# yozhijk/capsaicin

Measured on AMD Instinct MI355X. Metric: Mrays/sec (primary+secondary), cornell_box 1080p 64spp, higher is better.
Workload: dtype f32; 1 GPU; cornell_box.obj 1920x1080 64spp depth=8 (reference shading: Lambert + directional light + sky), tile-sharded over 1 GPU(s); triangles=32, bvh_depth=8, parallelism=tiles1, exchange=none

## Files before the change

### capsaicin_amd/capi.py

```python
import ctypes as C
import os
import subprocess

import numpy as np

_PKG = os.path.dirname(os.path.abspath(__file__))
_ROOT = os.path.dirname(_PKG)
LIB_PATH = os.path.join(_PKG, "libcapsaicin_hip.so")
if os.environ.get("CAP_LIB_VARIANT"):
    LIB_PATH = os.path.join(_PKG, "variants", "libcapsaicin_hip_%s.so" % os.environ["CAP_LIB_VARIANT"])

RENDER_AOV = 1
RENDER_EXT_MATERIALS = 2
RENDER_STAGE_TIMERS = 4
RENDER_GBUFFER_FEEDBACK = 8
RENDER_LOWRES_INDIRECT = 16

BUF_GBUFFER_GEO, BUF_DIRECT, BUF_ALBEDO, BUF_NORMAL_DEPTH, BUF_INDIRECT, BUF_COMBINED, BUF_ACCUM_SUM, BUF_ACCUM_MEAN, BUF_INDIRECT_LOWRES = range(9)


class CapError(RuntimeError):
    pass


# ... 472 lines not shown
        t = np.ascontiguousarray(rgba8, np.uint8)
        _check(lib().cap_texture_upload(self.ctx, index, _p(t), t.shape[1], t.shape[0]), "cap_texture_upload")

    def upload_bluenoise(self, rgba8):
        t = np.ascontiguousarray(rgba8, np.uint8)
        assert t.size == 256 * 256 * 4
        _check(lib().cap_bluenoise_upload(self.ctx, _p(t)), "cap_bluenoise_upload")

    def upload_materials(self, materials):
        m = np.ascontiguousarray(materials, np.float32).reshape(-1, 12)
        _check(lib().cap_materials_upload(self.ctx, _p(m), m.shape[0]), "cap_materials_upload")

    BVH_BUILD_AUTO, BVH_BUILD_LBVH, BVH_BUILD_SAH, BVH_BUILD_PLOC, BVH_BUILD_SAH_DEVICE = 0, 1, 2, 3, 4

    def set_bvh_build(self, mode):
        _check(lib().cap_set_bvh_build(self.ctx, mode), "cap_set_bvh_build")

    def build_bvh(self):
        _check(lib().cap_bvh_build(self.ctx), "cap_bvh_build")
        return self.bvh_info()

    def update_vertices(self, positions=None, normals=None, texcoords=None):
        ptrs, flags, keep = vertex_update_args(self._vertex_count, positions, normals, texcoords)
        if flags:
            import torch
            dev = torch.device("cuda", self.device)
            for a in keep:
                if a.device != dev:
                    raise CapError("update_vertices: tensors must be on %s, got %s" % (dev, a.device))
            torch.cuda.current_stream(dev).synchronize()
        _check(lib().cap_scene_update_vertices(self.ctx, ptrs[0], ptrs[1], ptrs[2], flags), "cap_scene_update_vertices")

    def refit_bvh(self):
        info = RefitInfo()
        _check(lib().cap_bvh_refit(self.ctx, C.byref(info)), "cap_bvh_refit")
        return info

    def bvh_info(self):
        bi = BvhInfo()
        _check(lib().cap_bvh_info(self.ctx, C.byref(bi)), "cap_bvh_info")
        return bi

    def bvh_readback(self):
        bi = self.bvh_info()
        nodes = np.zeros((bi.node_count, 16), np.float32)
        leaves = np.zeros(bi.triangle_count, np.uint32)
        _check(lib().cap_bvh_readback(self.ctx, _p(nodes), _p(leaves)), "cap_bvh_readback")
        return nodes, leaves

    def bvh_wide_readback(self):
        info = np.zeros(3, np.uint32)
        _check(lib().cap_bvh_wide_readback(self.ctx, None, None, _p(info)), "cap_bvh_wide_readback")
        nodes = np.zeros((int(info[0]), 20), np.uint32)
        src = np.zeros(max(1, self.bvh_info().triangle_count), np.uint32)
        _check(lib().cap_bvh_wide_readback(self.ctx, _p(nodes), _p(src), _p(info)), "cap_bvh_wide_readback")
        return nodes, src[:self.bvh_info().triangle_count], int(info[1]), int(info[2])

    def bvh_wide_info(self):
        info = np.zeros(3, np.uint32)
        _check(lib().cap_bvh_wide_readback(self.ctx, None, None, _p(info)), "cap_bvh_wide_readback")
        return int(info[0]), int(info[1]), int(info[2])

    def set_camera(self, cam):
        _check(lib().cap_camera_set(self.ctx, C.byref(cam)), "cap_camera_set")

    def set_prev_camera(self, cam):
        _check(lib().cap_prev_camera_set(self.ctx, C.byref(cam)), "cap_prev_camera_set")

    def set_resolution(self, width, height):
        _check(lib().cap_set_resolution(self.ctx, width, height), "cap_set_resolution")
        self.width, self.height = width, height

    def set_shard(self, index, count):
        _check(lib().cap_set_shard(self.ctx, index, count), "cap_set_shard")

    def set_traversal(self, mode):
        _check(lib().cap_set_traversal(self.ctx, mode), "cap_set_traversal")

    DEBUG_QUEUE_CAPACITY_DIV, DEBUG_WIDE_DEPTH_LIMIT, DEBUG_WIDE_IN_USE, DEBUG_FAIL_LANE1, DEBUG_LANES_USED = 1, 2, 3, 4, 5
    DEBUG_QUEUE_CANARY_FILL, DEBUG_QUEUE_CANARY_BEHIND, DEBUG_QUEUE_CANARY_USED, DEBUG_SELFTEST_DIV, DEBUG_NEE_PAIRS = 6, 7, 8, 9, 10
    DEBUG_SELFTEST_SHADE_UNARY, DEBUG_SELFTEST_SHADE_DIV2, DEBUG_SHADE_TAME = 11, 12, 13
    DEBUG_CAMERA_CULL = 14
    DEBUG_MARK_FORM = 15

    def debug_set(self, key, value):
        _check(lib().cap_debug_set(self.ctx, key, value), "cap_debug_set")

    DEBUG_SWITCH_BASE = 64

    def debug_switch(self, name, value):
        i = lib().cap_debug_switch_index(name.encode())
        if i < 0:
            raise CapError("unknown switch %s" % name)
        self.debug_set(self.DEBUG_SWITCH_BASE + i, 0xFFFFFFFFFFFFFFFF if value is None else int(value))

    def debug_get(self, key):
        v = _u64()
        _check(lib().cap_debug_get(self.ctx, key, C.byref(v)), "cap_debug_get")
        return int(v.value)

    def set_batch_paths(self, n):
        _check(lib().cap_set_batch_paths(self.ctx, n), "cap_set_batch_paths")

    def render(self, frame_begin, n_frames, num_bounces, flags=0):
        _check(lib().cap_render(self.ctx, frame_begin, n_frames, num_bounces, flags), "cap_render")

    def accum_reset(self):
        _check(lib().cap_accum_reset(self.ctx), "cap_accum_reset")

    def accum_import(self, sum_rgba, frames):
        a = np.ascontiguousarray(sum_rgba, np.float32)
        assert a.shape == (self.height, self.width, 4)
        _check(lib().cap_accum_import(self.ctx, _p(a), int(frames)), "cap_accum_import")

    def sync(self):
        _check(lib().cap_sync(self.ctx), "cap_sync")

    def readback(self, kind):
        if kind == BUF_INDIRECT_LOWRES:
            out = np.zeros((self.height // 2, self.width // 2, 4), np.float32)
        else:
            out = np.zeros((self.height, self.width, 4), np.float32)
        _check(lib().cap_readback(self.ctx, kind, _p(out)), "cap_readback")
        return out

    def stats(self):
        s = Stats()
        _check(lib().cap_stats_get(self.ctx, C.byref(s)), "cap_stats_get")
        return s

    def stats_reset(self):
        _check(lib().cap_stats_reset(self.ctx), "cap_stats_reset")

    RAY_FLAG_ACCEPT_FIRST_HIT, RAY_FLAG_CULL_BACK_FACING, RAY_FLAG_CULL_FRONT_FACING = 0x04, 0x10, 0x20

    def set_instance_masks(self, masks):
        if masks is None:
            _check(lib().cap_scene_set_instance_masks(self.ctx, None, len(self._tri_end)), "cap_scene_set_instance_masks")
            return
        m = np.ascontiguousarray(masks, np.uint8).reshape(-1)
        _check(lib().cap_scene_set_instance_masks(self.ctx, _p(m), m.size), "cap_scene_set_instance_masks")

    def trace_options(self, cull=None, mask=None, first_hit=False):
        if cull not in (None, "back", "front"):
            raise CapError('cull must be None, "back" or "front", got %r' % (cull,))
        if cull is None and mask is None and not first_hit:
            return None
        flags = {None: 0, "back": self.RAY_FLAG_CULL_BACK_FACING, "front": self.RAY_FLAG_CULL_FRONT_FACING}[cull]
        if first_hit:
            flags |= self.RAY_FLAG_ACCEPT_FIRST_HIT
        return TraceOptions(flags, 0 if mask is None else int(mask))

    def trace_rays(self, rays, out=None, sync=True, cull=None, mask=None, first_hit=False):
        return self._query(rays, out, sync, False, self.trace_options(cull, mask, first_hit))

    def trace_occlusion(self, rays, out=None, sync=True, cull=None, mask=None):
        return self._query(rays, out, sync, True, self.trace_options(cull, mask))

    def _query(self, rays, out, sync, any_hit, options=None):
        import torch
        dev = torch.device("cuda", self.device)
        host = isinstance(rays, np.ndarray)
        if host:
            rays = torch.from_numpy(np.ascontiguousarray(rays, np.float32).reshape(-1, 8)).to(dev)
            sync = True
        if rays.dtype != torch.float32 or rays.dim() != 2 or rays.shape[1] != 8 or not rays.is_contiguous() or rays.device != dev:
# ... 466 lines not shown
```

### capsaicin_amd/csrc/cap_context.h

```cpp
#pragma once

#include <array>
#include <string>
#include <utility>
#include <vector>

#include "../../include/capsaicin_hip.h"

#include "cap_kernels.h"

namespace cap
{
int fail(int code, const char* fmt, ...);

#define HIP_TRY(expr)                                                                                         \
    do                                                                                                        \
    {                                                                                                         \
        hipError_t e_ = (expr);                                                                               \
        if (e_ != hipSuccess) return fail(CAP_ERR_HIP, "%s failed: %s (%s:%d)", #expr, hipGetErrorString(e_), \
                                          __FILE__, __LINE__);                                                \
    } while (0)

template <typename T>
struct DevBuf
// ... 69 lines not shown
    uint32_t         vertex_count = 0, index_count = 0, mesh_count = 0, tri_count = 0;
    bool             scene_ready = false;

    std::vector<DevBuf<uint8_t>> texture_data;
    std::vector<TextureDev>      texture_host;
    DevBuf<TextureDev>           textures;
    bool                         textures_dirty = true;
    DevBuf<float2>               bluenoise;
    bool                         bluenoise_ready = false;
    std::vector<CapMaterial>     materials_host;
    DevBuf<CapMaterial>          materials;
    std::vector<float>           positions_host;
    std::vector<uint32_t>        indices_host;
    std::vector<CapMeshDesc>     meshes_host;
    DevBuf<uint32_t>             light_tris;
    DevBuf<float>                light_cdf;
    DevBuf<float2>               bluenoise_ba;
    uint32_t                     light_count = 0;
    float                        light_area  = 0.0f;
    bool                         materials_ready = false;

    DevBuf<float4>   shade_tris, tris_sorted, nodes, tri_raw, tri_box;
    DevBuf<float4>   nodes8, tris8;
    DevBuf<uint32_t> wide_src;
    DevBuf<uint32_t> wide_task, wide_alloc, wide_cnt;
    uint32_t         wide8_depth = 0, wide8_top = 0, wide8_nodes = 0;
    float            wide8_ms = 0.f;
    DevBuf<uint32_t> query_work, query_defer;
    DevBuf<uint8_t>  tri_mask;
    bool             tri_mask_on = false;
    DevBuf<float4>   inst_desc, inst_rec, inst_box, inst_tlas;
    DevBuf<uint32_t> inst_keys[2], inst_vals[2], inst_hist, inst_scan, inst_misc, inst_level_off;
    uint32_t         inst_count = 0, inst_top = 0, inst_nodes = 0;
    DevBuf<float2>   inst_near;
    DevBuf<uint32_t> inst_obj;
    bool             inst_obj_on = false;
    InstObject       scene_object_host{};
    DevBuf<InstObject> scene_object;
    std::vector<CapObjectInfo> obj_info;
    std::vector<uint32_t>      obj_node_base, obj_rec_base;
    uint32_t                   obj_count = 0, obj_max_depth = 0;
    DevBuf<float4>             forest_nodes, forest_tris;
    DevBuf<InstObject>         obj_table;
    DevBuf<float4>             obj_tri_raw, obj_tri_box;
    DevBuf<uint32_t>           obj_leaf_tri, obj_misc;
    DevBuf<float4>   fan_pairs, fan_singles;
    uint32_t         fan_pair_count = 0, fan_single_count = 0;
    DevBuf<float4>   fan_pairs_nee;
    uint32_t         fan_pair_nee_count = 0;
    std::vector<float>    fan_pairs_host;
    std::vector<uint32_t> light_tris_host;
    DevBuf<uint32_t> leaf_tri, keys0, keys1, vals0, vals1, hist, parent, flags, bvh_misc;
    DevBuf<float4>   ploc_boxes;
    DevBuf<uint32_t> ploc_ints;
    DevBuf<uint32_t> sahdev_words;
    CapBvhInfo       bvh_info{};
    bool             shade_tame = false;
    bool             bvh_ready = false;
    DevBuf<float>        pn_table;
    bool                 pn_ready = false;
    CapPseudonormalsInfo pn_info{};
    bool                  bvh_stale = false;
    bool                  positions_host_stale = false;
    bool                  visits_built_known = false;
    double                refit_visits_built = 0.0;
    std::vector<uint32_t> wide_levels;
    DevBuf<float>         wide_boxes;
    DevBuf<double>        refit_sums;

    CapCameraData camera{}, prev_camera{};
    bool          camera_ready = false, prev_camera_ready = false;
    ScreenDev     screen{};
    uint64_t      max_batch_paths = 0;
    SwitchTable   sw{};
    uint32_t      debug_capacity_div = 1;
    uint32_t      debug_wide_depth_limit = 0;
    bool          debug_fail_lane = false;
    uint64_t      lane1_failed_paths = 0;
    uint32_t      lane1_failed_bounces = 0, lane1_retry_tick = 0;
    uint32_t      lanes_last_render = 0;
    uint32_t      last_class_capacity = 0;
    uint32_t      tri_ids_dense = 0;
    uint32_t      last_mark_form = 0;
    uint32_t      last_cull_camera_pairs = 0;
    uint32_t      traversal_mode  = CAP_TRAVERSAL_AUTO;
    uint32_t      bvh_build_mode  = CAP_BVH_BUILD_AUTO;

    DevBuf<float4>     aov_geo, aov_nd, accum, image_tmp;
    DevBuf<uint64_t>   shaded_counter;
    struct Lane
    {
        hipStream_t      stream = nullptr;
        DevBuf<float4>   hits, q_org[2], q_dir[2], q_thr[2], s_org, s_dir, s_con, pl_color, pl_direct, pl_albedo;
        DevBuf<uint32_t> counters;
        DevBuf<uint32_t> stack_spill;
    } lane[2];
    hipStream_t stream2 = nullptr;
    hipEvent_t  lane_ev[2] = {nullptr, nullptr}, fork_ev = nullptr, join_ev = nullptr;
    static constexpr int kFrameRing = 4;
    DevBuf<FrameConst> frames_ring[kFrameRing];
    FrameConst*        frames_pinned[kFrameRing] = {nullptr, nullptr, nullptr, nullptr};
    size_t             frames_pinned_n[kFrameRing] = {0, 0, 0, 0};
    hipEvent_t         frames_event[kFrameRing] = {nullptr, nullptr, nullptr, nullptr};
    uint32_t           frames_next = 0;
    uint32_t           last_slots = 0;
    bool               aov_valid = false;
    bool               aov_lowres = false;
    uint32_t           aov_frame  = 0;
    uint64_t           frames_accumulated = 0;

    DevBuf<float4> post_in[4];
    DevBuf<float4> post_ihist[2], post_mhist[2], post_chist[2], post_prev_nd, post_itemp, post_temp[2], post_normals;
    uint32_t       post_w = 0, post_h = 0;
    int            post_last_dst = -1;

    void*           comm = nullptr;
    uint32_t        comm_rank = 0, comm_size = 0;
    bool            comm_local = false;
    DevBuf<float>   comm_send, comm_gathered, comm_image;
    hipEvent_t      comm_event = nullptr;

    CapStats               stats{};
    std::vector<TimedSpan> spans;
    std::vector<std::array<hipEvent_t, 6>> post_marks;
    std::vector<hipEvent_t> event_pool;
    std::vector<uint32_t*> pinned_pool;
    std::vector<std::pair<uint32_t*, uint32_t>> pending;
    uint64_t*              pinned_shaded = nullptr;
};

namespace cap
{
struct AovPlanes
{
    const float4 *color, *direct, *albedo;
};

int        sync_and_collect(CapContext* c);
hipEvent_t get_event(CapContext* c);
CameraDev  camera_dev(const CapCameraData& cd);
BvhDev     bvh_dev(const CapContext* c, const CapContext::Lane& lane);
AovPlanes  aov_planes(const CapContext* c);
int        trace_launch(const CapContext* c, const char* fmt, ...);
void       launch_texture_footprints(hipStream_t stream, const uint32_t* src, uint4* dst, uint32_t width, uint32_t height);
bool pair_ids_dense(const float* pairs, uint32_t pair_count, uint32_t single_count, uint32_t tri_count);
int  upload_fan_records(CapContext* c);
int  update_nee_pairs(CapContext* c);
int  ensure_positions_host(CapContext* c);
int  upload_light_table(CapContext* c);
int query_state(CapContext* c, const char* what);
}
```

### capsaicin_amd/csrc/cap_kernels.h

```cpp
#pragma once

#include "cap_device.h"

#include <cstdio>
#include <vector>

namespace cap
{
enum CapSwitch : uint32_t
{
    SW_NO_WIDE8 = 0,
    SW_LANE1_PRIORITY,
    SW_PLOC_RADIUS,
    SW_SAHDEV_LEAF,
    SW_WIDE_HOST_COLLAPSE,
    SW_TRACE_LAUNCHES,
    SW_NO_TWO_LANES,
    SW_LANE_SPLIT_MIN,
    SW_BLOCKS_PER_CU,
    SW_NO_CAMERA_CULL,
    SW_NO_ALBEDO_IN_W,
    SW_NO_INLINE_NEE,
    SW_NO_INLINE_PROBE,
    SW_NO_WAVE_RING,
    SW_ANY_REFILL,
    SW_PRIMARY_WIDE,
    SW_NO_PACKET,
    SW_NO_ANY_PROBE,
    SW_ANY_PROBE,
    SW_ANY_BLOCKS,
    SW_NO_PRIMARY_FUSE,
    SW_W8_REFILL,
    SW_W8_GRID,
    SW_AUTO_SAH_TRIANGLES,
    SW_NO_NEE_PAIR_CULL,
    SW_RAYGEN_KERNEL,
    SW_NO_PLANE_CODE,
    SW_COUNT
};
struct SwitchTable
{
    int64_t v[SW_COUNT];
    bool    on(CapSwitch k) const { return v[k] > 0; }
    int64_t get(CapSwitch k, int64_t dflt) const { return v[k] >= 0 ? v[k] : dflt; }
};

struct LaunchCfg
{
    hipStream_t stream;
    uint32_t    grid_blocks;
    uint32_t    stack_entries;
    uint32_t    cu_count = 0;
    uint32_t    any_no_probe = 0;
    const SwitchTable* sw = nullptr;
    bool    sw_on(CapSwitch k) const { return sw && sw->on(k); }
    int64_t sw_get(CapSwitch k, int64_t dflt) const { return sw ? sw->get(k, dflt) : dflt; }
};

template <auto K>
uint32_t resident_grid(const LaunchCfg& cfg, uint32_t want)
{
    static int per_cu = -1;
    if (per_cu < 0)
    {
        int n = 0;
        per_cu = (hipOccupancyMaxActiveBlocksPerMultiprocessor(&n, K, (int)kBlock, 0) == hipSuccess && n > 0) ? n : 0;
        if (cfg.sw_on(SW_TRACE_LAUNCHES)) fprintf(stderr, "[cap] resident workgroups per CU: %d\n", per_cu);
    }
    if (!cfg.cu_count || !per_cu) return want;
    const uint32_t cap = cfg.cu_count * (uint32_t)per_cu;
    return want < cap ? want : cap;
}
inline uint32_t queue_grid(const LaunchCfg& cfg, uint32_t max_count)
{
    uint32_t g = (max_count + kBlock - 1) / kBlock;
    if (g > cfg.grid_blocks) g = cfg.grid_blocks;
    return g ? g : 1;
}

void launch_trace_primary(const LaunchCfg& cfg, const BvhDev& bvh, const CameraDev& cam, const ScreenDev& screen,
                          const FrameConst* frames, uint32_t n_slots, float4* hits, uint32_t* work);
void launch_raygen_identity(const LaunchCfg& cfg, const CameraDev& cam, const ScreenDev& screen, const FrameConst* frames, uint32_t n_slots,
                            const RayQueue& q);
void launch_trace_closest(const LaunchCfg& cfg, const BvhDev& bvh, const RayQueue& q, uint32_t max_count, float4* hits);
void launch_trace_closest8(const LaunchCfg& cfg, const BvhDev& bvh, const RayQueue& q, uint32_t max_count, float4* hits, uint32_t* work);
void launch_trace_closest8_camera(const LaunchCfg& cfg, const BvhDev& bvh, const RayQueue& q, uint32_t max_count, float4* hits, uint32_t* work,
                                  const CameraDev& cam, const ScreenDev& screen, const FrameConst* frames, uint32_t n_slots);
void launch_trace_any(const LaunchCfg& cfg, const BvhDev& bvh, const ShadowQueue& q, uint32_t max_count, float4* target,
                      uint32_t pixels_padded, uint32_t n_slots, uint64_t* guard, uint32_t* work, bool mostly_unoccluded,
                      const FrameConst* frames, float4* code_plane = nullptr);

void launch_trace_any8_refill(const LaunchCfg& cfg, const BvhDev& bvh, const ShadowQueue& q, uint32_t max_count, float4* target, uint32_t pixels_padded,
                              uint32_t n_slots, uint64_t* guard, uint32_t* work, const FrameConst* frames);

struct QueryArgs
{
    const float4* rays;
    uint32_t      n;
    void*         out;
    uint32_t*     work;
    uint32_t*     defer;
    float         safe;
};
constexpr float kQuerySafeScale = 4.0f;
bool query8_stack_matches();
struct RayFilter;
void launch_query8(const LaunchCfg& cfg, const BvhDev& bvh, const QueryArgs& q, bool any, const RayFilter* f = nullptr, bool first_hit = false);
void launch_query_binary(const LaunchCfg& cfg, const BvhDev& bvh, const QueryArgs& q, bool any, bool deferred);
struct MultiArgs
{
    QueryArgs q;
    uint32_t  k;
    uint32_t* counts;
    uint32_t  resume;
};
constexpr uint32_t kMultiMaxK = 16;
uint32_t multi_bucket(uint32_t k);
void     launch_query8_multi(const LaunchCfg& cfg, const BvhDev& bvh, const MultiArgs& m, const RayFilter* f = nullptr);
void     launch_query_binary_multi(const LaunchCfg& cfg, const BvhDev& bvh, const MultiArgs& m, bool deferred, const RayFilter* f = nullptr);

// ... 19 lines not shown
    const float* normals;
    float*       signed_out;
};
void launch_signed_distance(const LaunchCfg& cfg, const BvhDev& bvh, const ClosestArgs& a, const SignedArgs& s, const RayFilter* f, uint32_t depth);
struct ClosestMultiArgs
{
    ClosestArgs a;
    uint32_t    k;
    uint32_t*   counts;
    uint32_t    resume;
};
void launch_closest_points_multi(const LaunchCfg& cfg, const BvhDev& bvh, const ClosestMultiArgs& m, const RayFilter* f, uint32_t depth);
struct TlasDev;
struct ClosestInstArgs
{
    ClosestArgs     a;
    uint32_t*       inst_out;
    const float4*   descs;
    const float2*   near;
    const uint32_t* xw_max;
};
void launch_closest_instances(const LaunchCfg& cfg, const BvhDev& bvh, const ClosestInstArgs& a, const TlasDev& tl, const RayFilter& f, uint32_t depth);
struct ClosestInstMultiArgs
{
    ClosestInstArgs ia;
    uint32_t        k;
    uint32_t*       counts;
    uint32_t        resume;
};
void launch_closest_instances_multi(const LaunchCfg& cfg, const BvhDev& bvh, const ClosestInstMultiArgs& m, const TlasDev& tl, const RayFilter& f,
                                    uint32_t depth);

struct InstObject
{
    double   blo[3], bhi[3];
    int32_t  root;
    uint32_t reserved;
};
struct InstanceBuildArgs
{
    const float*      descs;
    uint32_t          n;
    const InstObject* objects;
    uint32_t          n_objects;
    const uint32_t*   object_index;
    float4*      rec;
    float4*      box;
    float4*      tlas;
    float2*      near;
    uint32_t*    keys[2];
    uint32_t*    vals[2];
    uint32_t*    hist;
    uint32_t*    scan;
    uint32_t*    misc;
};
constexpr uint32_t kTlasMaxLevels = 25;
uint32_t tlas_layout(uint32_t n, uint32_t level_off[kTlasMaxLevels], uint32_t* total);
void     launch_instances_build(hipStream_t stream, const InstanceBuildArgs& a);
struct TlasDev
{
    const float4*   rec;
    const float4*   tlas;
    const uint32_t* level_off;
    uint32_t        top;
};
void launch_query_instances(const LaunchCfg& cfg, const BvhDev& bvh, const QueryArgs& q, const TlasDev& tl, const RayFilter& f, int mode, uint32_t* inst_out,
                            uint32_t depth);
void launch_query_instances_multi(const LaunchCfg& cfg, const BvhDev& bvh, const MultiArgs& m, const TlasDev& tl, const RayFilter& f, uint32_t* inst_out,
                                  uint32_t depth);
struct ForestRelocArgs
{
    float4*  nodes;
    float4*  tris;
    uint32_t n_tris, node_base, rec_base, first_triangle;
};
void launch_forest_relocate(hipStream_t stream, const ForestRelocArgs& a);

struct ShadeArgs
{
    SceneDev          scene;
    CameraDev         cam;
    ScreenDev         screen;
    const FrameConst* frames;
    const float4*     hits;
    RayQueue          in;
    RayQueue          out;
    ShadowQueue       shadow;
    Planes            planes;
    uint32_t          n_slots;
    uint32_t          bounce;
    uint32_t          num_bounces;
    uint32_t          max_count;
    uint32_t          aov_slot;
    uint64_t*         shaded_counter;
    uint32_t*         work;
    FeedbackDev       fb;
    uint32_t          albedo_in_w;
    uint32_t          inline_nee;
    uint32_t          inline_probe;
    uint32_t          wave_ring;
    uint32_t          cull_camera_pairs;
    uint32_t          code_in_color;
};
constexpr float kCodePadding = 0.f, kCodeSky = 1.f, kCodeKd = 2.f, kCodeBlack = 3.f;
constexpr float kCodeLit = 4.f;
constexpr float kCameraCullPad = 2.0f;
void launch_shade(const LaunchCfg& cfg, const ShadeArgs& args, bool ext, bool feedback = false);
bool launch_primary_shade(const LaunchCfg& cfg, const BvhDev& bvh, const ShadeArgs& args, float4* hits, bool ext);
uint32_t launch_trace_shade(const LaunchCfg& cfg, const BvhDev& bvh, const ShadeArgs& args, bool ext, bool feedback = false);
bool trace_shade_has_code_form(const BvhDev& bvh, const SceneDev& scene);

void launch_resolve(const LaunchCfg& cfg, const Planes& planes, uint32_t n_slots, uint32_t pixels_padded, float4* accum,
                    bool albedo_in_w = false, float kd_untextured = 0.0f, bool code_in_color = false);
void launch_untile(const LaunchCfg& cfg, const ScreenDev& screen, const float4* src, const float4* albedo, const float4* direct,
                   int plane_kind, float4* image);
void launch_tile(const LaunchCfg& cfg, const ScreenDev& screen, const float4* image, float4* dst);
void launch_untile4(const LaunchCfg& cfg, const ScreenDev& screen, const float4* s0, const float4* s1, const float4* s2, const float4* s3,
                    float4* d0, float4* d1, float4* d2, float4* d3);
void launch_tiles_mean(const LaunchCfg& cfg, const float4* accum, uint32_t pixels_padded, float4* dst);
void launch_assemble(const LaunchCfg& cfg, const ScreenDev& screen, const float4* gathered, uint32_t shard_count, float4* image,
                     size_t shard_stride = 0);
void launch_geo_aov(const LaunchCfg& cfg, const SceneDev& scene, const float4* hits_slot, uint32_t pixels_padded, float4* aov_geo);

struct BvhBuildArgs
{
    const float*    positions;
    const float*    normals;
    const float*    texcoords;
    const uint32_t* indices;
    const uint4*    tri_ids;
    const uint4*    mesh_offsets;
    uint32_t        tri_count;
    float4*         shade_tris;
    float4*         tris_sorted;
    float4*         nodes;
    uint32_t*       leaf_tri;
    float4*         tri_raw;
    float4*         tri_box;
    uint32_t*       keys[2];
    uint32_t*       vals[2];
    uint32_t*       hist;
    uint32_t*       parent;
    uint32_t*       flags;
    uint32_t*       bounds;
    uint32_t*       max_depth;
};
size_t bvh_radix_blocks(uint32_t n);
void   launch_bvh_build(hipStream_t stream, const BvhBuildArgs& a);
int    launch_bvh_sort(hipStream_t stream, const BvhBuildArgs& a);
size_t bvh_radix_scan_words(uint32_t n);
int    launch_radix_sort_pairs(hipStream_t stream, uint32_t* const keys[2], uint32_t* const vals[2], uint32_t n, uint32_t* hist, uint32_t* scan);
size_t bvh_scan_scratch_words(uint32_t total);
void   launch_exclusive_scan_u32(hipStream_t stream, uint32_t* v, uint32_t total, uint32_t* scratch);
struct PlocScratch
{
    float4*   boxes;
    uint32_t* ints;
};
int    launch_bvh_build_ploc(hipStream_t stream, const BvhBuildArgs& a, const PlocScratch& s, uint32_t radius);
size_t bvh_sah_device_scratch_words(uint32_t n);
int    launch_bvh_build_sah_device(hipStream_t stream, const BvhBuildArgs& a, const PlocScratch& s, uint32_t* scratch, uint32_t radius, uint32_t leaf);
void launch_bvh_setup(hipStream_t stream, const BvhBuildArgs& a);
void launch_bvh_finish_host(hipStream_t stream, const BvhBuildArgs& a);

void     launch_gather_wide(hipStream_t stream, const uint32_t* tri_src, const float4* tris_sorted, uint32_t n, float4* tris8);
struct WideCollapseArgs
{
    const float4*   bnodes;
    const uint32_t* count;
    uint32_t        n_tris, capacity;
    double          pad;
    uint32_t *      task, *alloc, *nodes8, *tri_src;
    uint32_t*       cnt;
    uint32_t        begin, end;
};
int      launch_wide_collapse(hipStream_t stream, WideCollapseArgs a, uint32_t* node_count, uint32_t* depth, uint32_t* top_nodes,
                          std::vector<uint32_t>* level_begin = nullptr);
struct PseudonormalArgs
{
    const float*    positions;
    const uint32_t* indices;
    const uint4*    tri_ids;
    const uint4*    mesh_offsets;
    uint32_t        tri_count;
    float*          table;
    uint32_t *      kx, *ky, *kz;
    uint32_t*       keys[2];
    uint32_t*       vals[2];
    uint32_t*       weld;
    uint32_t*       flag;
    uint32_t*       hist;
    uint32_t*       scan;
    double*         nf;
// ... 55 lines not shown
```

### capsaicin_amd/csrc/cap_shade.h

```cpp
#pragma once

#include "cap_exhaustive.h"
#include "cap_kernels.h"
#include "cap_reproject.h"
#include "cap_unscaled.h"

namespace cap
{
__device__ __forceinline__ void bluenoise4x4(const float2* tex, uint32_t x, uint32_t y, uint32_t count, float& s0, float& s1)
{
    const uint32_t px = (count % 16u) % 4u, py = (count % 16u) / 4u;
    const uint32_t sx = (x * 4u + px) % 256u, sy = (y * 4u + py) % 256u;
    const float2   t  = tex[sy * 256u + sx];
    const float    k  = 0.61803398875f * (float)(count / 16u);
    const float    a = t.x + k, b = t.y + k;
    s0 = a - floorf(a);
    s1 = b - floorf(b);
}

__device__ __forceinline__ v3 ortho_vector(v3 n)
{
    const bool  zn = fabsf(n.z) > 0.0f;
    const float a = zn ? n.z : n.y, b = zn ? n.y : n.x;
    const float k = sqrtf(fmaf(a, a, b * b));
    const float q1 = a / k, q2 = b / k;
    return zn ? mk3(0.0f, -q1, q2) : mk3(q1, -q2, 0.0f);
}

__device__ __forceinline__ v3 map_to_hemisphere(float r1, float r2, v3 n)
{
    v3       u = ortho_vector(n);
    const v3 v = cross3(u, n);
    u          = cross3(n, v);
    float sin_psi, cos_psi;
    sincos_c((2.0f * kPi) * r1, sin_psi, cos_psi);
    const float cos_theta = sqrtf(1.0f - r2);
    const float sin_theta = sqrtf(1.0f - cos_theta * cos_theta);
    const float a = sin_theta * cos_psi, b = sin_theta * sin_psi;
    return normalize3(mk3(fmaf(n.x, cos_theta, fmaf(v.x, b, u.x * a)), fmaf(n.y, cos_theta, fmaf(v.y, b, u.y * a)),
                          fmaf(n.z, cos_theta, fmaf(v.z, b, u.z * a))));
}

constexpr float kNormLo = 0.125f, kNormHi = 4.0f;
__device__ __forceinline__ v3 normalize3_tame(v3 v)
{
    return v * div_unscaled(1.0f, sqrt_pos(dot3(v, v)));
}
__device__ __forceinline__ bool ortho_in_range(float a, float b, float g)
{
    constexpr uint32_t kG0 = (127u - 78u) << 23, kG1 = (127u + 80u) << 23, kX0 = (127u - 80u) << 23;
    const uint32_t     xa = (f2u(a) & 0x7fffffffu) - 1u, xb = (f2u(b) & 0x7fffffffu) - 1u;
    return (f2u(g) - kG0 < kG1 - kG0) & ((xa < xb ? xa : xb) >= kX0 - 1u);
}
__device__ __forceinline__ v3 map_to_hemisphere_tame(float r1, float r2, v3 n)
{
    const bool  zn = fabsf(n.z) > 0.0f;
    const float a = zn ? n.z : n.y, b = zn ? n.y : n.x;
    const float g = fmaf(a, a, b * b);
#if defined(CAP_SHADE_ORTHO_PLAIN)
    const bool fast = false;
#else
    const bool  fast = __ballot(!ortho_in_range(a, b, g)) == 0ull;
#endif
    float       q1, q2;
    if (fast)
        div2_unscaled(a, b, sqrt_pos(g), q1, q2);
    else
    {
        const float k = sqrtf(g);
        q1 = a / k, q2 = b / k;
    }
    v3       u = zn ? mk3(0.0f, -q1, q2) : mk3(q1, -q2, 0.0f);
    const v3 v = cross3(u, n);
    u          = cross3(n, v);
    float sin_psi, cos_psi;
    sincos_c((2.0f * kPi) * r1, sin_psi, cos_psi);
    const float cos_theta = sqrt_pos(1.0f - r2);
    const float sin_theta = sqrt_unscaled(1.0f - cos_theta * cos_theta);
    const float ca = sin_theta * cos_psi, cb = sin_theta * sin_psi;
    const v3    d = mk3(fmaf(n.x, cos_theta, fmaf(v.x, cb, u.x * ca)), fmaf(n.y, cos_theta, fmaf(v.y, cb, u.y * ca)),
                        fmaf(n.z, cos_theta, fmaf(v.z, cb, u.z * ca)));
    return fast ? normalize3_tame(d) : normalize3(d);
}

__device__ __forceinline__ void oct_encode(v3 n, float& ox, float& oy)
{
    const float s = fabsf(n.x) + fabsf(n.y) + fabsf(n.z);
    n             = mk3(n.x / s, n.y / s, n.z / s);
    ox = n.x, oy = n.y;
    if (!(n.z >= 0.0f))
    {
        ox = (1.0f - fabsf(n.y)) * (n.x >= 0.0f ? 1.0f : -1.0f);
        oy = (1.0f - fabsf(n.x)) * (n.y >= 0.0f ? 1.0f : -1.0f);
    }
    ox = ox * 0.5f + 0.5f;
    oy = oy * 0.5f + 0.5f;
}

__device__ __forceinline__ uint32_t wrap_texel(float f, uint32_t n)
{
    const float m = f - floorf(f / (float)n) * (float)n;
    int         i = (int)m;
    if (i < 0) i = 0;
    if ((uint32_t)i >= n) i = 0;
    return (uint32_t)i;
}

__device__ __forceinline__ v3 sample_texture(const TextureDev& tex, float u, float v)
{
    const float    fx = fmaf(u, (float)tex.width, -0.5f), fy = fmaf(v, (float)tex.height, -0.5f);
    const float    x0f = floorf(fx), y0f = floorf(fy);
    const float    wx = fx - x0f, wy = fy - y0f;
    const uint32_t x0 = wrap_texel(x0f, tex.width), y0 = wrap_texel(y0f, tex.height);
    const uint4  fq   = reinterpret_cast<const uint4*>(tex.quads)[y0 * tex.width + x0];
    auto         rgba = [](uint32_t wd) { return make_uchar4((uint8_t)wd, (uint8_t)(wd >> 8), (uint8_t)(wd >> 16), (uint8_t)(wd >> 24)); };
    const uchar4 c00 = rgba(fq.x), c10 = rgba(fq.y), c01 = rgba(fq.z), c11 = rgba(fq.w);
    auto unorm8 = [](uint8_t b) {
        const float r = 1.0f / 255.0f, fb = (float)b, q = fb * r;
        return fmaf(fmaf(-q, 255.0f, fb), r, q);
    };
    auto           lerp2 = [&](uint8_t a00, uint8_t a10, uint8_t a01, uint8_t a11) {
        const float f00 = unorm8(a00), f10 = unorm8(a10), f01 = unorm8(a01), f11 = unorm8(a11);
        const float top = fmaf(f10 - f00, wx, f00);
        const float bot = fmaf(f11 - f01, wx, f01);
        return fmaf(bot - top, wy, top);
    };
    return mk3(lerp2(c00.x, c10.x, c01.x, c11.x), lerp2(c00.y, c10.y, c01.y, c11.y), lerp2(c00.z, c10.z, c01.z, c11.z));
}

__device__ __forceinline__ uint32_t wave_append(bool emit, uint32_t* counter)
{
    const unsigned long long mask = __ballot(emit);
    if (mask == 0ull) return 0;
    const uint32_t lane   = threadIdx.x & 63u;
    const uint32_t leader = (uint32_t)__ffsll((long long)mask) - 1u;
    uint32_t       base   = 0;
    if (lane == leader) base = atomicAdd(counter, (uint32_t)__popcll(mask));
    base = __shfl(base, (int)leader);
    return base + (uint32_t)__popcll(mask & ((1ull << lane) - 1ull));
}

struct ShadePre
{
    bool  valid;
    v3    L, I;
    float r1, r2;
    float r3, r4, r5, r6;
    float r1n, r2n;
    bool  indirect_on;
};

__device__ __forceinline__ void stage_frames(const ShadeArgs& a, FrameConst* lds_frames)
{
    const uint32_t  words = a.n_slots * (uint32_t)(sizeof(FrameConst) / 4);
    const uint32_t* src   = reinterpret_cast<const uint32_t*>(a.frames);
    uint32_t*       dst   = reinterpret_cast<uint32_t*>(lds_frames);
    for (uint32_t i = threadIdx.x; i < words; i += kBlock) dst[i] = src[i];
    __syncthreads();
}

#if defined(CAP_CHUNK_PLAIN)
constexpr bool kChunkLean = false;
#else
constexpr bool kChunkLean = true;
#endif

#pragma clang diagnostic push
#pragma clang diagnostic ignored "-Wuninitialized"
__device__ __forceinline__ float unread_f()
{
    float x;
    return x;
}
#pragma clang diagnostic pop
__device__ __forceinline__ v3 unread3() { return mk3(unread_f(), unread_f(), unread_f()); }

struct SlotSample
{
    uint32_t off;
    float    k;
};
__device__ __forceinline__ uint32_t bluenoise_offset(uint32_t count) { return (((count % 16u) / 4u) << 8) | ((count % 16u) % 4u); }
__device__ __forceinline__ float    bluenoise_shift(uint32_t count) { return 0.61803398875f * (float)(count / 16u); }
__device__ __forceinline__ uint32_t bluenoise_base(uint32_t x, uint32_t y) { return ((y & 63u) << 10) | ((x & 63u) << 2); }
__device__ __forceinline__ void     bluenoise_at(const float2* tex, uint32_t base, uint32_t off, float k, float& s0, float& s1)
{
    const float2 t = tex[base | off];
    const float  a = t.x + k, b = t.y + k;
    s0 = a - floorf(a);
    s1 = b - floorf(b);
}
template <bool FIRST>
__device__ __forceinline__ void stage_frames_samples(const ShadeArgs& a, FrameConst* lds_frames, SlotSample* lds_first)
{
    constexpr uint32_t kWords = (uint32_t)(sizeof(FrameConst) / 4);
    static_assert(kWords == 12 && offsetof(FrameConst, frame_count) == 8 && offsetof(FrameConst, pad1) == 28 && offsetof(FrameConst, pad2) == 44, "FrameConst layout");
    const uint32_t  words = (a.n_slots < kMaxFrameSlots ? a.n_slots : kMaxFrameSlots) * kWords;
    const uint32_t* src   = reinterpret_cast<const uint32_t*>(a.frames);
    uint32_t*       dst   = reinterpret_cast<uint32_t*>(lds_frames);
    for (uint32_t i = threadIdx.x; i < kMaxFrameSlots * kWords; i += kBlock)
    {
        uint32_t v = 0u;
        if (i < words)
        {
            const uint32_t sl = i / kWords, w = i - sl * kWords;
            v = src[i];
            if (w == 7u || w == 11u)
            {
                const uint32_t next = src[sl * kWords + 2u] * 25u + a.bounce + 1u;
                v = w == 7u ? bluenoise_offset(next) : f2u(bluenoise_shift(next));
            }
        }
        dst[i] = v;
    }
    if (FIRST)
        for (uint32_t sl = threadIdx.x; sl < kMaxFrameSlots; sl += kBlock)
        {
            SlotSample ss = {0u, 0.0f};
            if (sl < a.n_slots)
            {
                const uint32_t count = a.frames[sl].frame_count * 25u + a.bounce;
                ss.off = bluenoise_offset(count), ss.k = bluenoise_shift(count);
            }
            lds_first[sl] = ss;
        }
    __syncthreads();
}

template <class C>
__device__ __forceinline__ ShadePre shade_prefetch(const ShadeArgs& a, const FrameConst* lds_frames, bool active, uint32_t pid,
                                                   float carried_r1 = 0.f, float carried_r2 = 0.f, const SlotSample* lds_first = nullptr)
{
    ShadePre       s;
    const uint32_t slot = pid >> kPidShift, pl = pid & kPidMask;
    if constexpr (C::LEAN)
    {
        static_assert(C::CARRY && !C::EXT, "LEAN: the reference model's fused kernels");
        const uint32_t    sl = slot < kMaxFrameSlots ? slot : 0;
        const FrameConst& fc = lds_frames[sl];
        uint32_t          base;
        s.indirect_on = true;
        if (C::FIRST)
        {
            uint32_t x = 0, y = 0;
            s.valid = active && local_pixel_to_xy(a.screen, pl, x, y);
            if (fc.lowres_sel & 4u) s.indirect_on = (x & 1u) == ((fc.lowres_sel >> 1) & 1u) && (y & 1u) == (fc.lowres_sel & 1u);
            base = bluenoise_base(x, y);
        }
        else
        {
            s.valid = active;
            const uint32_t gt = __umul24(pl >> 6, a.screen.shard_count) + a.screen.shard_index;
            const uint32_t ty = tile_div(gt, a.screen.tiles_x_mul, a.screen.tiles_x_shift);
            const uint32_t tx = gt + (ty & 7u) * ((0u - a.screen.tiles_x) & 7u);
            base = ((ty & 7u) << 13) | ((pl & 0x38u) << 7) | ((tx & 7u) << 5) | ((pl & 7u) << 2);
        }
        s.L = unread3(), s.I = unread3(), s.r1 = s.r2 = s.r1n = s.r2n = unread_f();
        s.r3 = s.r4 = s.r5 = s.r6 = 0.f;
        if (s.valid)
        {
            s.L = mk3(fc.light_dir[0], fc.light_dir[1], fc.light_dir[2]);
            s.I = mk3(fc.light_intensity[0], fc.light_intensity[1], fc.light_intensity[2]);
            if (C::FIRST)
            {
                const SlotSample ss = lds_first[sl];
                bluenoise_at(a.scene.bluenoise, base, ss.off, ss.k, s.r1, s.r2);
            }
            else
                s.r1 = carried_r1, s.r2 = carried_r2;
            if (!C::TAME || a.bounce < a.num_bounces) bluenoise_at(a.scene.bluenoise, base, f2u(fc.pad1), fc.pad2, s.r1n, s.r2n);
        }
        return s;
    }
    uint32_t       x = 0, y = 0;
    s.valid = active && local_pixel_to_xy(a.screen, pl, x, y);
    s.L = mk3(0, 0, 0), s.I = mk3(0, 0, 0), s.r1 = 0.f, s.r2 = 0.f;
    s.r3 = s.r4 = s.r5 = s.r6 = 0.f;
    s.r1n = s.r2n = 0.f;
    s.indirect_on = true;
    if (s.valid)
    {
        const FrameConst fc = lds_frames[slot < kMaxFrameSlots ? slot : 0];
        if (fc.lowres_sel & 4u) s.indirect_on = (x & 1u) == ((fc.lowres_sel >> 1) & 1u) && (y & 1u) == (fc.lowres_sel & 1u);
        s.L = mk3(fc.light_dir[0], fc.light_dir[1], fc.light_dir[2]);
        s.I = mk3(fc.light_intensity[0], fc.light_intensity[1], fc.light_intensity[2]);
        const uint32_t count = fc.frame_count * 25u + a.bounce;
        if (C::CARRY && !C::FIRST)
            s.r1 = carried_r1, s.r2 = carried_r2;
        else
            bluenoise4x4(a.scene.bluenoise, x, y, count, s.r1, s.r2);
        if (C::CARRY && (!C::TAME || a.bounce < a.num_bounces)) bluenoise4x4(a.scene.bluenoise, x, y, count + 1u, s.r1n, s.r2n);
        if (C::EXT)
        {
            bluenoise4x4(a.scene.bluenoise_ba, x, y, count, s.r3, s.r4);
            bluenoise4x4(a.scene.bluenoise, x, y, count + 7u, s.r5, s.r6);
        }
    }
    return s;
}

__device__ __forceinline__ void wave_append2(bool& emit_ext, bool& emit_shadow, uint32_t* counter_pair, uint32_t& ext_slot,
                                             uint32_t& shadow_slot, uint32_t capacity, uint64_t* guard)
{
    const unsigned long long me = __ballot(emit_ext), ms = __ballot(emit_shadow);
    ext_slot = shadow_slot = 0;
    if ((me | ms) == 0ull) return;
    const uint32_t lane   = threadIdx.x & 63u;
    const uint32_t leader = (uint32_t)__ffsll((long long)(me | ms)) - 1u;
    uint32_t       lo = 0, hi = 0;
    if (lane == leader)
    {
        const unsigned long long add = ((unsigned long long)__popcll(ms) << 32) | (unsigned long long)__popcll(me);
        const unsigned long long old = atomicAdd(reinterpret_cast<unsigned long long*>(counter_pair), add);
        lo = (uint32_t)old, hi = (uint32_t)(old >> 32);
    }
    lo = __shfl(lo, (int)leader), hi = __shfl(hi, (int)leader);
    const unsigned long long below = (1ull << lane) - 1ull;
    ext_slot    = lo + (uint32_t)__popcll(me & below);
    shadow_slot = hi + (uint32_t)__popcll(ms & below);
    if (lo + (uint32_t)__popcll(me) > capacity || hi + (uint32_t)__popcll(ms) > capacity)
    {
        if (lane == leader)
        {
            atomicAdd((unsigned long long*)guard + 4, 1ull);
            guard[3] = ((uint64_t)lo << 32) | hi;
        }
        emit_ext    = emit_ext && ext_slot < capacity;
        emit_shadow = emit_shadow && shadow_slot < capacity;
    }
}

#ifdef CAP_STAMPS
static __device__ unsigned long long g_stamps[16];
struct Stamps
{
    unsigned long long last, acc[8], t_begin;
    __device__ void    start()
    {
        for (int i = 0; i < 8; ++i) acc[i] = 0;
        last    = __builtin_amdgcn_s_memtime();
        t_begin = __builtin_amdgcn_s_memrealtime();
    }
    __device__ void mark(int i, bool wait)
    {
#ifdef CAP_STAMPS_PHASES
// ... 81 lines not shown
                    atomicAdd(c + 2, thr.z * 0.85f);
                }
            }
        }
        else if (valid)
        {
            ++n_shaded;
            const float4* tab = shade_tab + kShadeRec * (size_t)gid;
            const float4  s0 = tab[0], s1 = tab[1], s2 = tab[2], s3 = tab[3], s4 = tab[4], s5 = tab[5];
            const float   u = hit.x, v = hit.y, w = (1.0f - u) - v;
            auto          mix = [&](float c0, float c1, float c2) { return fmaf(c2, v, fmaf(c1, u, c0 * w)); };
            const v3      nm = mk3(mix(s3.x, s4.x, s5.x), mix(s3.y, s4.y, s5.y), mix(s3.z, s4.z, s5.z));
            const v3      n  = C::TAME ? normalize3_tame(nm) : normalize3(nm);
            p = mk3(mix(s0.x, s1.x, s2.x), mix(s0.y, s1.y, s2.y), mix(s0.z, s1.z, s2.z));
            v3       kd   = mk3(a.scene.kd_untextured, a.scene.kd_untextured, a.scene.kd_untextured);
            uint32_t inst = 0;
            if (a.scene.texture_count != 0 || (C::FIRST && slot == a.aov_slot))
            {
                const float4 idf   = tab[6];
                inst               = f2u(idf.x);
                const uint32_t tex = f2u(idf.z);
                if (tex != kInvalidId && tex < a.scene.texture_count)
                {
                    const float tu = mix(s0.w, s2.w, s4.w), tv = mix(s1.w, s3.w, s5.w);
                    const v3    c  = sample_texture(a.scene.textures[tex], tu, 1.0f - tv);
                    kd             = mk3(pow22_c(c.x), pow22_c(c.y), pow22_c(c.z));
                }
            }
            const bool black = kd.x < 1e-5f && kd.y < 1e-5f && kd.z < 1e-5f;
            if (C::FIRST)
            {
                if (C::CODE)
                    a.planes.color[plane_idx] = make_float4(0.f, 0.f, 0.f, black ? kCodeBlack : kCodeKd);
                else
                {
                    a.planes.color[plane_idx]  = make_float4(0.f, 0.f, 0.f, 1.f);
                    a.planes.direct[plane_idx] = make_float4(0.f, 0.f, 0.f, a.albedo_in_w ? (black ? kCodeBlack : kCodeKd) : 1.f);
                }
                if (!C::CODE && !a.albedo_in_w) a.planes.albedo[plane_idx] = black ? make_float4(0.f, 0.f, 0.f, 0.f) : make_float4(kd.x, kd.y, kd.z, 1.f);
                if (slot == a.aov_slot)
                {
                    float4 nd = make_float4(0.f, 0.f, 0.f, 0.f);
                    if (!black)
                    {
                        oct_encode(n, nd.x, nd.y);
                        nd.z = (float)inst;
                        nd.w = length3(mk3(a.cam.position[0], a.cam.position[1], a.cam.position[2]) - p);
                    }
                    a.planes.aov_normal_depth[pl] = nd;
                }
            }
            bool reused = false;
            if (C::FB && !C::FIRST && !black)
            {
                const uint32_t W = a.screen.width, H = a.screen.height;
                const f2       puv = image_plane_uv(a.fb.prev_cam, p);
                if (puv.x >= 0.0f && puv.y >= 0.0f && puv.x <= 1.0f && puv.y <= 1.0f)
                {
                    const f2    pxy        = uv_to_xy(puv, W, H);
                    const float prev_depth = ldi(Img{a.fb.prev_normal_depth, W, H}, (int)pxy.x, (int)pxy.y).w;
                    const float cur_depth =
                        length3(p - mk3(a.fb.prev_cam.position[0], a.fb.prev_cam.position[1], a.fb.prev_cam.position[2]));
                    if (!(fabsf(prev_depth - cur_depth) / cur_depth > 0.05f))
                    {
                        reused        = true;
                        const v3 hc   = sample_bilinear(Img{a.fb.color_history, W, H}, puv);
                        const float4 cur = a.planes.color[plane_idx];
                        a.planes.color[plane_idx] = make_float4(cur.x + thr.x * hc.x, cur.y + thr.y * hc.y, cur.z + thr.z * hc.z, cur.w);
                    }
                }
            }
            if (!black && !reused)
            {
                const float ndl = fmaxf(0.0f, dot3(n, pre.L));
                v3          c   = mk3(((pre.I.x * kd.x) * kInvPi) * ndl, ((pre.I.y * kd.y) * kInvPi) * ndl, ((pre.I.z * kd.z) * kInvPi) * ndl);
                if (c.x != 0.0f || c.y != 0.0f || c.z != 0.0f)
                {
                    emit_shadow = true;
                    contrib     = C::FIRST ? c : thr * c;
                }
                const bool more = a.bounce < a.num_bounces;
                if (!C::TAME || more)
                {
                    dir             = C::TAME ? map_to_hemisphere_tame(pre.r1, pre.r2, n) : map_to_hemisphere(pre.r1, pre.r2, n);
                    const float ndd = dot3(n, dir);
                    const float pdf = C::TAME ? div_unscaled(fmaxf(0.0f, ndd), kPi) : fmaxf(0.0f, ndd) / kPi;
                    if (!(pdf < 1e-5f))
                    {
                        const float fn = kInvPi * fmaxf(ndd, 0.0f);
                        const float f  = C::TAME ? div_unscaled(fn, pdf) : fn / pdf;
                        thr            = thr * f;
                        if (!C::FIRST) thr = thr * kd;
                        emit_ext = more && (!C::FIRST || pre.indirect_on);
                    }
                }
            }
        }

        if (C::PROBE)
        {
            if (probe.rows != nullptr)
            {
                const Ray    sr  = make_ray(p, pre.L, kRayEps, kRayFar);
                const uint32_t ps = valid ? slot : 0u;
                const float4   pa = probe.rows[2u * ps], pb = probe.rows[2u * ps + 1u];
                const bool   occluded = pair_occludes_pre(sr, probe.pairs, probe.k, pa, pb);
                if (emit_shadow && occluded) emit_shadow = false, ++*n_probed;
            }
        }
        uint32_t ei, si;
        STAMP(st, 2, true);
        wave_append2(emit_ext, emit_shadow, a.out.count + klass * kCounterStride, ei, si, a.out.class_capacity, a.shaded_counter);
        STAMP(st, 3, true);
        ei += klass * a.out.class_capacity;
        si += klass * a.shadow.class_capacity;
        if (C::PROBE && probe.ring_org != nullptr)
        {
            const unsigned long long ms = __ballot(emit_shadow);
            if (emit_shadow)
            {
                const uint32_t lane_ = threadIdx.x & 63u;
                const uint32_t pos   = (ring_head + *ring_n + (uint32_t)__popcll(ms & ((1ull << lane_) - 1ull))) & (kWaveRing - 1u);
                probe.ring_org[pos]  = make_float4(p.x, p.y, p.z, u2f(pid));
                probe.ring_con[pos]  = make_float4(contrib.x, contrib.y, contrib.z, 0.0f);
            }
            *ring_n += (uint32_t)__popcll(ms);
            __builtin_amdgcn_fence(__ATOMIC_RELEASE, "wavefront");
        }
        else if (emit_shadow)
        {
            a.shadow.org_tmin[si]    = make_float4(p.x, p.y, p.z, u2f(pid));
            a.shadow.contrib_pid[si] = make_float4(contrib.x, contrib.y, contrib.z, C::CODE ? kCodeKd : 0.0f);
        }
        if (emit_ext)
        {
            a.out.org_tmin[ei] = make_float4(p.x, p.y, p.z, C::CARRY ? pre.r1n : kRayEps);
            a.out.dir_tmax[ei] = make_float4(dir.x, dir.y, dir.z, C::CARRY ? pre.r2n : kRayFar);
            a.out.thr_pid[ei]  = make_float4(thr.x, thr.y, thr.z, u2f(pid));
        }
    }
}

struct ExtBsdf
{
    v3    f;
    float pdf_spec, pdf_diff;
};

__device__ __forceinline__ float lum3(v3 c) { return fmaf(c.z, 0.114f, fmaf(c.y, 0.587f, c.x * 0.299f)); }

struct ExtView
{
    float cos_o, lam_o;
};
__device__ __forceinline__ ExtView ext_view(float a2, v3 nf, v3 wo)
{
    ExtView w;
    w.cos_o = dot3(nf, wo);
    w.lam_o = w.cos_o + sqrtf(fmaf(1.0f - a2, w.cos_o * w.cos_o, a2));
    return w;
}
__device__ __forceinline__ ExtBsdf ext_bsdf(v3 kd, v3 ks, float a2, v3 nf, v3 wo, v3 wi, const ExtView& vw)
{
    const float cos_i = dot3(nf, wi);
    const v3    h     = normalize3(wo + wi);
    const float cos_h = dot3(nf, h), woh = dot3(wo, h);
    const float dd    = fmaf(cos_h * cos_h, a2 - 1.0f, 1.0f);
// ... 232 lines not shown
```

### capsaicin_amd/csrc/context.hip

```cpp
#include <algorithm>
#include <cmath>
#include <cstdarg>
#include <cstdio>
#include <cstdlib>
#include <cstring>
#include <memory>

#include "cap_context.h"
#include "cap_near.h"
#include "cap_wide.h"
#include "query_ranges.h"

namespace
{
thread_local std::string g_error;

constexpr double kPrimaryWideTrianglesPerPixel = 2.0;
constexpr uint64_t kAnyRefillTreeBytes = ~0ull;

constexpr size_t kGuardWords = 8;
}

namespace cap
{
// ... 152 lines not shown

namespace
{
struct StageTimer
{
    CapContext* c;
    TimedSpan   sp;
    bool        on;
    StageTimer(CapContext* ctx, int stage, bool enabled = true, int also = ST_NONE) : c(ctx), on(enabled)
    {
        if (!on) return;
        sp.stage = stage;
        sp.also  = also;
        sp.a     = get_event(c);
        sp.b     = get_event(c);
        (void)hipEventRecord(sp.a, c->stream);
    }
    ~StageTimer()
    {
        if (!on) return;
        (void)hipEventRecord(sp.b, c->stream);
        c->spans.push_back(sp);
    }
};

void update_screen(CapContext* c, uint32_t w, uint32_t h, uint32_t shard_index, uint32_t shard_count)
{
    ScreenDev& s  = c->screen;
    s.width       = w;
    s.height      = h;
    s.tiles_x     = (w + kTileDim - 1) / kTileDim;
    s.tiles_y     = (h + kTileDim - 1) / kTileDim;
    s.tile_count  = s.tiles_x * s.tiles_y;
    s.shard_index = shard_index;
    s.shard_count = shard_count ? shard_count : 1;
    const uint32_t max_local = (s.tile_count + s.shard_count - 1) / s.shard_count;
    s.local_tiles   = s.tile_count > s.shard_index ? (s.tile_count - s.shard_index + s.shard_count - 1) / s.shard_count : 0;
    s.pixels_padded = max_local * kTilePixels;
    tile_div_setup(s.tiles_x, s.tiles_x_mul, s.tiles_x_shift);
    c->frames_accumulated = 0;
    c->aov_valid = false;
}

FrameConst frame_const(uint32_t frame_count, bool lowres_indirect)
{
    FrameConst f{};
    halton23(frame_count, f.jitter_x, f.jitter_y);
    f.frame_count = frame_count;
    f.lowres_sel = lowres_indirect ? (4u | (((frame_count % 4u) / 2u) << 1) | ((frame_count % 4u) % 2u)) : 0u;
    const float t = 2.0f * 3.14f * (float)(frame_count % 4096) / 4096.0f;
    float       st, ct;
    sincos_c(t, st, ct);
    const v3 dir = normalize3(mk3(40.0f * st, 100.0f, 40.0f * ct));
    f.light_dir[0] = dir.x, f.light_dir[1] = dir.y, f.light_dir[2] = dir.z;
    f.light_intensity[0] = 1.0f * (2.0f * 14.0f + 0.0f);
    f.light_intensity[1] = 1.0f * (2.0f * 12.0f + 0.0f);
    f.light_intensity[2] = 1.0f * (2.0f * 10.0f + (2.0f + 2.0f * ct));
    return f;
}

SceneDev scene_dev(const CapContext* c)
{
    SceneDev s{};
    s.shade_tris    = c->shade_tris.p;
    s.tri_ids       = c->tri_ids.p;
    s.mesh_texture  = c->mesh_texture.p;
    s.textures      = c->textures.p;
    s.texture_count = (uint32_t)c->texture_host.size();
    s.bluenoise     = c->bluenoise.p;
    s.kd_untextured = pow22_c(0.75f);
    s.shade_tame    = c->shade_tame ? 1u : 0u;
    s.bluenoise_ba  = c->bluenoise_ba.p;
    s.materials     = reinterpret_cast<const MaterialDev*>(c->materials.p);
    s.material_count = c->materials_ready ? c->mesh_count : 0u;
    s.light_tris    = c->light_tris.p;
    s.light_cdf     = c->light_cdf.p;
    s.light_count   = c->light_count;
    s.light_area    = c->light_area;
    return s;
}

struct LaneSizes
{
    size_t planes, queues, rings, counters;
};

LaneSizes lane_sizes(const CapContext* c, uint32_t slots, uint32_t bounces)
{
    LaneSizes z;
    z.planes = (size_t)slots * c->screen.pixels_padded;
    z.queues = z.planes + (size_t)kQueueClasses * 64;
    z.rings = std::max(z.queues, (size_t)std::max(c->cu_count, 1) * 8 * (kBlock / 64) * 128);
    z.counters = (3 * (size_t)(bounces + 1) + 1) * kQueueClasses * kCounterStride;
    return z;
}

bool lane_grows(const CapContext::Lane& L, const LaneSizes& z) { return L.pl_color.n < z.planes || L.counters.n < z.counters; }

int ensure_lane(CapContext* c, CapContext::Lane& L, uint32_t slots, uint32_t bounces)
{
    const LaneSizes z = lane_sizes(c, slots, bounces);
    for (DevBuf<float4>* b : {&L.hits, &L.q_org[0], &L.q_org[1], &L.q_dir[0], &L.q_dir[1], &L.q_thr[0], &L.q_thr[1], &L.s_dir})
        HIP_TRY(b->ensure(z.queues));
    for (DevBuf<float4>* b : {&L.s_org, &L.s_con}) HIP_TRY(b->ensure(z.rings));
    for (DevBuf<float4>* b : {&L.pl_color, &L.pl_direct, &L.pl_albedo}) HIP_TRY(b->ensure(z.planes));
    HIP_TRY(L.counters.ensure(z.counters));
    if (c->lane[0].stack_spill.n) HIP_TRY(L.stack_spill.ensure(c->lane[0].stack_spill.n));
    return CAP_OK;
}

int ensure_frame_buffers(CapContext* c)
{
    HIP_TRY(c->aov_geo.ensure(c->screen.pixels_padded));
    HIP_TRY(c->aov_nd.ensure(c->screen.pixels_padded));
    if (!c->shaded_counter.p)
    {
        HIP_TRY(c->shaded_counter.ensure(kGuardWords));
        HIP_TRY(hipMemsetAsync(c->shaded_counter.p, 0, kGuardWords * sizeof(uint64_t), c->stream));
    }
    if (!c->accum.p || c->accum.n < c->screen.pixels_padded)
    {
        HIP_TRY(c->accum.ensure(c->screen.pixels_padded));
        HIP_TRY(hipMemsetAsync(c->accum.p, 0, sizeof(float4) * c->screen.pixels_padded, c->stream));
        c->frames_accumulated = 0;
    }
    return CAP_OK;
}

int ensure_lane_streams(CapContext* c)
{
    if (!c->stream2)
    {
        if (c->sw.v[SW_LANE1_PRIORITY] >= 0)
            HIP_TRY(hipStreamCreateWithPriority(&c->stream2, hipStreamNonBlocking, (int)c->sw.v[SW_LANE1_PRIORITY]));
        else
            HIP_TRY(hipStreamCreateWithFlags(&c->stream2, hipStreamNonBlocking));
    }
    c->lane[1].stream = c->stream2;
    for (hipEvent_t* e : {&c->lane_ev[0], &c->lane_ev[1], &c->fork_ev, &c->join_ev})
        if (!*e) HIP_TRY(hipEventCreateWithFlags(e, hipEventDisableTiming));
    return CAP_OK;
}

struct BatchPolicy
{
    uint32_t slots;
    bool     two_lanes;
    bool     lane1_failed_before;
};

BatchPolicy batch_policy(const CapContext* c, uint32_t n_frames, uint32_t num_bounces, uint32_t flags, bool tree_path)
{
    const uint32_t Ppad = c->screen.pixels_padded;
    uint64_t       budget = c->max_batch_paths ? c->max_batch_paths : (uint64_t)64 << 20;
    if (!c->max_batch_paths && (uint64_t)n_frames * Ppad > budget)
    {
        const uint64_t big       = (uint64_t)128 << 20;
        const uint64_t big_slots = std::max<uint64_t>(1, std::min<uint64_t>(big / std::max(1u, Ppad), kMaxFrameSlots));
        bool           room      = c->lane[0].pl_color.n >= big_slots * Ppad && (!tree_path || c->lane[1].pl_color.n >= big_slots * Ppad);
        if (!room)
        {
            size_t free_b = 0, total_b = 0;
            room = hipMemGetInfo(&free_b, &total_b) == hipSuccess && free_b > 3u * big_slots * Ppad * 256u;
        }
        if (room) budget = big;
    }
    uint32_t       slots  = (uint32_t)std::max<uint64_t>(1, std::min<uint64_t>(budget / std::max(1u, Ppad), kMaxFrameSlots));
    slots                 = std::min(slots, n_frames);
    const bool no_two_lanes = c->sw.on(SW_NO_TWO_LANES);
    bool two_lanes = !no_two_lanes && tree_path && c->bvh_info.stack_entries != 0 && !(flags & CAP_RENDER_GBUFFER_FEEDBACK) &&
                     !(flags & CAP_RENDER_LOWRES_INDIRECT) && n_frames >= 2;
    if (two_lanes && slots >= n_frames)
    {
        const uint64_t split_min = (uint64_t)c->sw.get(SW_LANE_SPLIT_MIN, (int64_t)4 << 20);
        if ((uint64_t)n_frames * Ppad >= split_min)
            slots = (n_frames + 1) / 2;
        else
            two_lanes = false;
    }
    if ((flags & CAP_RENDER_STAGE_TIMERS) || c->sw.on(SW_TRACE_LAUNCHES)) two_lanes = false;
    const bool failed_before =
        two_lanes && c->lane1_failed_paths && (uint64_t)slots * Ppad >= c->lane1_failed_paths && num_bounces >= c->lane1_failed_bounces;
    return BatchPolicy{slots, two_lanes, failed_before};
}
}

__global__ __launch_bounds__(256) void k_texture_footprints(const uint32_t* src, uint4* dst, uint32_t width, uint32_t height)
{
    const size_t i = (size_t)blockIdx.x * 256 + threadIdx.x;
    if (i >= (size_t)width * height) return;
    const uint32_t y = (uint32_t)(i / width), x = (uint32_t)(i - (size_t)y * width);
    const uint32_t x1 = x + 1 == width ? 0 : x + 1, y1 = y + 1 == height ? 0 : y + 1;
    dst[i] = make_uint4(src[(size_t)y * width + x], src[(size_t)y * width + x1], src[(size_t)y1 * width + x], src[(size_t)y1 * width + x1]);
}

void cap::launch_texture_footprints(hipStream_t stream, const uint32_t* src, uint4* dst, uint32_t width, uint32_t height)
{
    const size_t texels = (size_t)width * height;
    hipLaunchKernelGGL(k_texture_footprints, dim3((unsigned)((texels + 255) / 256)), dim3(256), 0, stream, src, dst, width, height);
}

extern "C" {

const char* cap_last_error(void) { return g_error.c_str(); }
void cap_set_error_(const char* msg) { g_error = msg ? msg : ""; }

int cap_device_count(void)
{
    int n = 0;
    if (hipGetDeviceCount(&n) != hipSuccess) return 0;
    return n;
}

static const char* const kSwitchNames[SW_COUNT] = {
    "CAP_NO_WIDE8", "CAP_LANE1_PRIORITY", "CAP_PLOC_RADIUS", "CAP_SAHDEV_LEAF", "CAP_WIDE_HOST_COLLAPSE", "CAP_TRACE_LAUNCHES", "CAP_NO_TWO_LANES",
    "CAP_LANE_SPLIT_MIN", "CAP_BLOCKS_PER_CU", "CAP_NO_CAMERA_CULL", "CAP_NO_ALBEDO_IN_W", "CAP_NO_INLINE_NEE", "CAP_NO_INLINE_PROBE", "CAP_NO_WAVE_RING",
    "CAP_ANY_REFILL", "CAP_PRIMARY_WIDE", "CAP_NO_PACKET", "CAP_NO_ANY_PROBE", "CAP_ANY_PROBE", "CAP_ANY_BLOCKS", "CAP_NO_PRIMARY_FUSE", "CAP_W8_REFILL",
    "CAP_W8_GRID", "CAP_AUTO_SAH_TRIANGLES", "CAP_NO_NEE_PAIR_CULL", "CAP_RAYGEN_KERNEL", "CAP_NO_PLANE_CODE"};

static void switches_from_environment(SwitchTable& t)
{
    for (uint32_t k = 0; k < SW_COUNT; ++k)
    {
        const char* e = getenv(kSwitchNames[k]);
        t.v[k]        = -1;
        if (!e) continue;
        char*           end = nullptr;
        const long long v   = strtoll(e, &end, 10);
        t.v[k]              = (end != e && v >= 0) ? v : 1;
    }
    if (getenv("CAP_BVH_BINARY") && t.v[SW_NO_WIDE8] < 0) t.v[SW_NO_WIDE8] = 1;
}

int cap_debug_switch_index(const char* name)
{
    for (uint32_t k = 0; name && k < SW_COUNT; ++k)
        if (strcmp(name, kSwitchNames[k]) == 0) return (int)k;
    return -1;
}

extern "C" int cap_debug_tile_divmod(uint32_t tiles_x, const uint32_t* n, uint64_t count, uint32_t* quotient, uint32_t* remainder)
{
    if (!tiles_x || !n || !quotient || !remainder) return CAP_ERR_INVALID_ARG;
    uint32_t mul, shift;
    tile_div_setup(tiles_x, mul, shift);
    for (uint64_t k = 0; k < count; ++k)
    {
        quotient[k]  = tile_div(n[k], mul, shift);
        remainder[k] = n[k] - quotient[k] * tiles_x;
    }
    return CAP_OK;
}

int cap_debug_pair_ids_dense(const float* pair_records, uint32_t pair_count, uint32_t single_count, uint32_t tri_count)
{
    if (!pair_records && pair_count) return 0;
    return pair_ids_dense(pair_records, pair_count, single_count, tri_count) ? 1 : 0;
}

int cap_debug_query_ranges(uint64_t n, uint32_t count, const uint64_t* base, const uint64_t* stride, const uint32_t* align)
{
    static const char* const names[4] = {"range 0", "range 1", "range 2", "range 3"};
    if (count > 4 || (count && (!base || !stride || !align))) return fail(CAP_ERR_INVALID_ARG, "cap_debug_query_ranges: at most 4 ranges, no NULL array");
    QueryRange r[4];
    for (uint32_t i = 0; i < count; ++i)
    {
        if (!align[i] || (align[i] & (align[i] - 1u))) return fail(CAP_ERR_INVALID_ARG, "cap_debug_query_ranges: align[%u] is not a power of two", i);
        r[i] = QueryRange{names[i], (uintptr_t)base[i], stride[i], align[i], stride[i] != 0};
    }
    char msg[256];
    return query_ranges_ok("cap_debug_query_ranges", n, r, count, msg, sizeof(msg)) ? CAP_OK : fail(CAP_ERR_INVALID_ARG, "%s", msg);
}

int cap_debug_closest_instance_bound(const float* transform, const float* box_lo, const float* box_hi, const float* point, float best_dist2,
                                     float* world_to_object, float* g, float* xw, float* slack, uint32_t* skip)
{
    if (!transform || !box_lo || !box_hi || !point) return fail(CAP_ERR_INVALID_ARG, "cap_debug_closest_instance_bound: NULL input");
    double m[12], w[12], wd[12], A[12], nA, kappa, blo[3], bhi[3];
    float  wf[12];
    bool   live = true;
    for (int k = 0; k < 12; ++k) m[k] = (double)transform[k], live = live && finite_d(m[k]);
    for (int k = 0; k < 3; ++k) blo[k] = (double)box_lo[k], bhi[k] = (double)box_hi[k];
    live = instance_inverse(m, live, w, wf, wd, A, nA, kappa, (float)CAP_INSTANCE_MAX_CONDITION);
    const float gi = live ? near_sigma_min_bound(w) : 0.0f, xi = live ? near_world_extent(m, blo, bhi) : 0.0f;
    const float pmax = fmaxf(fabsf(point[0]), fmaxf(fabsf(point[1]), fabsf(point[2])));
    const float sl   = near_slack(pmax, xi);
    float       ox, oy, oz;
    near_to_object(wf, point[0], point[1], point[2], ox, oy, oz);
    const float bd2 = box_dist2(ox, oy, oz, box_lo[0], box_lo[1], box_lo[2], box_hi[0], box_hi[1], box_hi[2]);
    if (world_to_object)
        for (int k = 0; k < 12; ++k) world_to_object[k] = wf[k];
    if (g) *g = gi;
    if (xw) *xw = xi;
    if (slack) *slack = sl;
    if (skip) *skip = live && near_skip(bd2, near_bound2_object(sqrtf(best_dist2), sl, gi)) ? 1u : 0u;
    return CAP_OK;
}

int cap_ctx_create(int device_id, void* hip_stream, CapContext** out_ctx)
{
    if (!out_ctx) return fail(CAP_ERR_INVALID_ARG, "cap_ctx_create: out_ctx is NULL");
// ... 145 lines not shown
    if (!c) return fail(CAP_ERR_INVALID_ARG, "cap_debug_set: ctx is NULL");
    switch (key)
    {
    case CAP_DEBUG_QUEUE_CAPACITY_DIV:
        if (value < 1 || value > 1024) return fail(CAP_ERR_INVALID_ARG, "cap_debug_set: capacity divisor %llu not in 1..1024", (unsigned long long)value);
        c->debug_capacity_div = (uint32_t)value;
        return CAP_OK;
    case CAP_DEBUG_WIDE_DEPTH_LIMIT:
        c->debug_wide_depth_limit = (uint32_t)value;
        return CAP_OK;
    case CAP_DEBUG_QUEUE_CANARY_FILL:
        if (!c->lane[0].q_org[0].p) return fail(CAP_ERR_STATE, "cap_debug_set: the queues are allocated by the first cap_render");
        HIP_TRY(hipSetDevice(c->device));
        for (int k = 0; k < 2; ++k)
            for (DevBuf<float4>* b : {&c->lane[0].q_org[k], &c->lane[0].q_dir[k], &c->lane[0].q_thr[k]})
                HIP_TRY(hipMemsetD32Async((hipDeviceptr_t)b->p, (int)kCanaryWord, b->n * 4, c->stream));
        return CAP_OK;
    case CAP_DEBUG_FAIL_LANE1:
        c->debug_fail_lane = value != 0;
        if (!value) c->lane1_failed_paths = 0;
        return CAP_OK;
    default:
        if (key >= CAP_DEBUG_SWITCH_BASE && key < CAP_DEBUG_SWITCH_BASE + SW_COUNT)
        {
            c->sw.v[key - CAP_DEBUG_SWITCH_BASE] = value == ~0ull ? -1 : (int64_t)value;
            return CAP_OK;
        }
        return fail(CAP_ERR_INVALID_ARG, "cap_debug_set: unknown key %u", key);
    }
}

int cap_debug_get(CapContext* c, uint32_t key, uint64_t* value)
{
    if (!c || !value) return fail(CAP_ERR_INVALID_ARG, "cap_debug_get: NULL argument");
    switch (key)
    {
    case CAP_DEBUG_QUEUE_CAPACITY_DIV: *value = c->debug_capacity_div; return CAP_OK;
    case CAP_DEBUG_WIDE_DEPTH_LIMIT: *value = c->debug_wide_depth_limit; return CAP_OK;
    case CAP_DEBUG_FAIL_LANE1: *value = c->debug_fail_lane ? 1u : 0u; return CAP_OK;
    case CAP_DEBUG_LANES_USED: *value = c->lanes_last_render; return CAP_OK;
    case CAP_DEBUG_SELFTEST_DIV:
    {
        HIP_TRY(hipSetDevice(c->device));
        DevBuf<unsigned long long> d;
        unsigned long long         h[3] = {0, 0, 0};
        HIP_TRY(d.ensure(3));
        HIP_TRY(hipMemsetAsync(d.p, 0, sizeof(h), c->stream));
        launch_div_selftest(c->stream, d.p);
        HIP_TRY(hipGetLastError());
        HIP_TRY(hipMemcpyAsync(h, d.p, sizeof(h), hipMemcpyDeviceToHost, c->stream));
        HIP_TRY(hipStreamSynchronize(c->stream));
        const unsigned long long expected = (0x7f7fffffull - 0x00800000ull + 1ull) + (1ull << 30);
        if (h[2] != expected) return fail(CAP_ERR_HIP, "cap_debug_get: the division self-test compared %llu of %llu cases", h[2], expected);
        *value = h[0] + h[1];
        return CAP_OK;
    }
    case CAP_DEBUG_SELFTEST_SHADE_UNARY:
    case CAP_DEBUG_SELFTEST_SHADE_DIV2:
    {
        HIP_TRY(hipSetDevice(c->device));
        DevBuf<unsigned long long> d;
        unsigned long long         h[2] = {0, 0};
        HIP_TRY(d.ensure(2));
        HIP_TRY(hipMemsetAsync(d.p, 0, sizeof(h), c->stream));
        launch_shade_forms_selftest(c->stream, d.p, key == CAP_DEBUG_SELFTEST_SHADE_DIV2 ? 1u : 0u);
        HIP_TRY(hipGetLastError());
        HIP_TRY(hipMemcpyAsync(h, d.p, sizeof(h), hipMemcpyDeviceToHost, c->stream));
        HIP_TRY(hipStreamSynchronize(c->stream));
        const unsigned long long floats_sqrt = 0x7f7fffffull - ((127ull - 96ull) << 23) + 1ull;
        const unsigned long long least = key == CAP_DEBUG_SELFTEST_SHADE_DIV2 ? (1ull << 30) : 2ull * floats_sqrt + 3ull + (5ull << 23) + 1ull + 0x40000001ull + (8ull << 23);
        if (h[1] < least) return fail(CAP_ERR_HIP, "cap_debug_get: the shading self-test compared %llu of at least %llu cases", h[1], least);
        *value = h[0];
        return CAP_OK;
    }
    case CAP_DEBUG_SHADE_TAME:
        if (!c->bvh_ready || c->bvh_stale) return fail(CAP_ERR_STATE, "cap_debug_get: BVH not built or stale");
        *value = c->shade_tame ? 1u : 0u;
        return CAP_OK;
    case CAP_DEBUG_CAMERA_CULL: *value = c->last_cull_camera_pairs; return CAP_OK;
    case CAP_DEBUG_MARK_FORM:
        if (!c->bvh_ready) return fail(CAP_ERR_STATE, "cap_debug_get: BVH not built");
        *value = ((uint64_t)c->last_mark_form << 8) | c->tri_ids_dense;
        return CAP_OK;
    case CAP_DEBUG_NEE_PAIRS:
        if (!c->bvh_ready) return fail(CAP_ERR_STATE, "cap_debug_get: BVH not built");
        *value = ((uint64_t)(c->fan_pairs_nee.p ? c->fan_pair_nee_count : c->fan_pair_count) << 32) | c->fan_pair_count;
        return CAP_OK;
    case CAP_DEBUG_QUEUE_CANARY_BEHIND: return canary_count(c, true, value);
    case CAP_DEBUG_QUEUE_CANARY_USED: return canary_count(c, false, value);
    case CAP_DEBUG_WIDE_IN_USE:
        if (!c->bvh_ready) return fail(CAP_ERR_STATE, "cap_debug_get: BVH not built");
        *value = bvh_dev(c, c->lane[0]).wide8_ok;
        return CAP_OK;
    default:
        if (key >= CAP_DEBUG_SWITCH_BASE && key < CAP_DEBUG_SWITCH_BASE + SW_COUNT)
        {
            *value = (uint64_t)c->sw.v[key - CAP_DEBUG_SWITCH_BASE];
            return CAP_OK;
        }
        return fail(CAP_ERR_INVALID_ARG, "cap_debug_get: unknown key %u", key);
    }
}

int cap_set_bvh_build(CapContext* c, uint32_t mode)
{
    if (!c) return fail(CAP_ERR_INVALID_ARG, "cap_set_bvh_build: ctx is NULL");
    if (mode > CAP_BVH_BUILD_SAH_DEVICE) return fail(CAP_ERR_INVALID_ARG, "cap_set_bvh_build: unknown mode %u", mode);
    c->bvh_build_mode = mode;
    return CAP_OK;
}

int cap_set_traversal(CapContext* c, uint32_t mode)
{
    if (!c) return fail(CAP_ERR_INVALID_ARG, "cap_set_traversal: ctx is NULL");
    if (mode > CAP_TRAVERSAL_EXHAUSTIVE) return fail(CAP_ERR_INVALID_ARG, "cap_set_traversal: unknown mode %u", mode);
    c->traversal_mode = mode;
    return CAP_OK;
}

int cap_accum_reset(CapContext* c)
{
    if (!c) return fail(CAP_ERR_INVALID_ARG, "cap_accum_reset: ctx is NULL");
    HIP_TRY(hipSetDevice(c->device));
    if (c->accum.p) HIP_TRY(hipMemsetAsync(c->accum.p, 0, sizeof(float4) * c->accum.n, c->stream));
    c->frames_accumulated = 0;
    return CAP_OK;
}

int cap_accum_import(CapContext* c, const float* sum_rgba, uint64_t frames)
{
    if (!c || !sum_rgba) return fail(CAP_ERR_INVALID_ARG, "cap_accum_import: NULL argument");
    if (!c->screen.width) return fail(CAP_ERR_STATE, "cap_accum_import: resolution not set");
    HIP_TRY(hipSetDevice(c->device));
    if (sync_and_collect(c) != CAP_OK) return CAP_ERR_HIP;
    const size_t npix = (size_t)c->screen.width * c->screen.height;
    HIP_TRY(c->image_tmp.ensure(npix));
    HIP_TRY(c->accum.ensure(c->screen.pixels_padded));
    HIP_TRY(hipMemcpyAsync(c->image_tmp.p, sum_rgba, sizeof(float4) * npix, hipMemcpyHostToDevice, c->stream));
    LaunchCfg cfg{c->stream, (uint32_t)c->cu_count * 8u, 32};
    launch_tile(cfg, c->screen, c->image_tmp.p, c->accum.p);
    HIP_TRY(hipGetLastError());
    HIP_TRY(hipStreamSynchronize(c->stream));
    c->frames_accumulated = frames;
    return CAP_OK;
}

int cap_sync(CapContext* c)
{
    if (!c) return fail(CAP_ERR_INVALID_ARG, "cap_sync: ctx is NULL");
    HIP_TRY(hipSetDevice(c->device));
    return sync_and_collect(c);
}

int cap_render(CapContext* c, uint32_t frame_begin, uint32_t n_frames, uint32_t num_bounces, uint32_t flags)
{
    if (!c) return fail(CAP_ERR_INVALID_ARG, "cap_render: ctx is NULL");
    if (!c->bvh_ready) return fail(CAP_ERR_STATE, "cap_render: call cap_bvh_build first");
    if (c->bvh_stale) return fail(CAP_ERR_STATE, "cap_render: vertices changed; call cap_bvh_refit or cap_bvh_build");
    if (!c->camera_ready || !c->bluenoise_ready || !c->screen.width) return fail(CAP_ERR_STATE, "cap_render: camera, blue noise and resolution must be set");
    const bool ext = (flags & CAP_RENDER_EXT_MATERIALS) != 0;
    if (ext && !c->materials_ready) return fail(CAP_ERR_STATE, "cap_render: CAP_RENDER_EXT_MATERIALS needs cap_materials_upload (one material per mesh)");
    static_assert(sizeof(MaterialDev) == sizeof(CapMaterial), "material layouts must match");
    if (num_bounces > 255) return fail(CAP_ERR_INVALID_ARG, "cap_render: num_bounces %u exceeds 255", num_bounces);
    if (!n_frames) return CAP_OK;
    HIP_TRY(hipSetDevice(c->device));
    c->last_mark_form   = 0;
    const bool feedback = (flags & CAP_RENDER_GBUFFER_FEEDBACK) != 0;
    if (feedback)
    {
        if (ext) return fail(CAP_ERR_UNSUPPORTED, "cap_render: CAP_RENDER_GBUFFER_FEEDBACK is defined for the reference shading model only");
        if (n_frames != 1) return fail(CAP_ERR_INVALID_ARG, "cap_render: CAP_RENDER_GBUFFER_FEEDBACK renders one frame per call (n_frames is %u)", n_frames);
        if (!c->prev_camera_ready) return fail(CAP_ERR_STATE, "cap_render: CAP_RENDER_GBUFFER_FEEDBACK needs cap_prev_camera_set");
        if (c->post_w != c->screen.width || c->post_h != c->screen.height)
            if (int e = cap_post_reset(c)) return e;
    }

    const bool lowres = (flags & CAP_RENDER_LOWRES_INDIRECT) != 0;
    if (lowres)
    {
        if (ext) return fail(CAP_ERR_UNSUPPORTED, "cap_render: CAP_RENDER_LOWRES_INDIRECT is defined for the reference shading model only");
        if (n_frames != 1) return fail(CAP_ERR_INVALID_ARG, "cap_render: CAP_RENDER_LOWRES_INDIRECT renders one frame per call (n_frames is %u)", n_frames);
        if ((c->screen.width | c->screen.height) & 1u) return fail(CAP_ERR_INVALID_ARG, "cap_render: CAP_RENDER_LOWRES_INDIRECT needs even width and height (%ux%u)", c->screen.width, c->screen.height);
    }

    if (c->traversal_mode == CAP_TRAVERSAL_EXHAUSTIVE && c->tri_count > 4096)
        return fail(CAP_ERR_UNSUPPORTED, "cap_render: exhaustive traversal refused for %u triangles", c->tri_count);
    const bool     tree_path     = c->traversal_mode == CAP_TRAVERSAL_EXHAUSTIVE ? false
                                                                                 : !(c->traversal_mode == CAP_TRAVERSAL_AUTO && c->tri_count <= kExhaustiveMax);
    const uint32_t stack_entries = tree_path ? c->bvh_info.stack_entries : 0u;
    const bool     fused         = stack_entries == 0;

    const uint32_t    Ppad      = c->screen.pixels_padded;
    const BatchPolicy policy    = batch_policy(c, n_frames, num_bounces, flags, tree_path);
    const uint32_t    slots     = policy.slots;
    bool              two_lanes = policy.two_lanes;
    if (c->spans.size() > 2048 || c->pending.size() > 64 || c->post_marks.size() > 256)
        if (sync_and_collect(c) != CAP_OK) return CAP_ERR_HIP;
    const LaneSizes need = lane_sizes(c, slots, num_bounces);
    if (lane_grows(c->lane[0], need) || !c->accum.p || c->accum.n < Ppad) HIP_TRY(hipStreamSynchronize(c->stream));
    if (ensure_lane(c, c->lane[0], slots, num_bounces) != CAP_OK || ensure_frame_buffers(c) != CAP_OK) return CAP_ERR_HIP;
    if (policy.lane1_failed_before)
    {
        size_t free_b = 0, total_b = 0;
        const bool room = hipMemGetInfo(&free_b, &total_b) == hipSuccess && free_b > (size_t)slots * Ppad * 256u;
        if (!room && (++c->lane1_retry_tick % 32u) != 0u)
        {
            two_lanes = false;
            ++c->stats.lane1_dropped;
        }
    }
    if (two_lanes)
    {
        if (lane_grows(c->lane[1], need))
        {
            HIP_TRY(hipStreamSynchronize(c->stream));
            if (c->stream2) HIP_TRY(hipStreamSynchronize(c->stream2));
        }
        if (c->debug_fail_lane || ensure_lane(c, c->lane[1], slots, num_bounces) != CAP_OK || ensure_lane_streams(c) != CAP_OK)
        {
            (void)hipGetLastError();
            c->lane[1] = CapContext::Lane{};
            c->lane1_failed_paths = (uint64_t)slots * Ppad, c->lane1_failed_bounces = num_bounces;
            ++c->stats.lane1_dropped;
            two_lanes = false;
        }
    }
    c->lanes_last_render = two_lanes ? 2u : 1u;
    const uint32_t ring = c->frames_next;
    c->frames_next      = (c->frames_next + 1) % CapContext::kFrameRing;
    if (!c->frames_event[ring]) HIP_TRY(hipEventCreateWithFlags(&c->frames_event[ring], hipEventDisableTiming));
    HIP_TRY(hipEventSynchronize(c->frames_event[ring]));
    if (c->frames_ring[ring].n < n_frames)
    {
        HIP_TRY(c->frames_ring[ring].ensure(n_frames));
    }
    if (c->frames_pinned_n[ring] < n_frames)
    {
        if (c->frames_pinned[ring]) HIP_TRY(hipHostFree(c->frames_pinned[ring]));
        c->frames_pinned[ring] = nullptr;
        HIP_TRY(hipHostMalloc((void**)&c->frames_pinned[ring], sizeof(FrameConst) * n_frames, hipHostMallocDefault));
        c->frames_pinned_n[ring] = n_frames;
    }
    for (uint32_t f = 0; f < n_frames; ++f) c->frames_pinned[ring][f] = frame_const(frame_begin + f, lowres);
    HIP_TRY(hipMemcpyAsync(c->frames_ring[ring].p, c->frames_pinned[ring], sizeof(FrameConst) * n_frames, hipMemcpyHostToDevice, c->stream));
    const bool st = (flags & CAP_RENDER_STAGE_TIMERS) != 0;
    if (c->textures_dirty)
    {
        HIP_TRY(hipStreamSynchronize(c->stream));
        HIP_TRY(c->textures.ensure(std::max<size_t>(1, c->texture_host.size())));
        if (!c->texture_host.empty())
            HIP_TRY(hipMemcpy(c->textures.p, c->texture_host.data(), sizeof(TextureDev) * c->texture_host.size(), hipMemcpyHostToDevice));
        c->textures_dirty = false;
    }

    uint32_t blocks_per_cu = fused ? 6u : (stack_entries <= 32 ? 5u : 2u);
    if (c->sw.v[SW_BLOCKS_PER_CU] >= 0) blocks_per_cu = (uint32_t)std::max<int64_t>(1, c->sw.v[SW_BLOCKS_PER_CU]);
    const SceneDev  scene = scene_dev(c);
    const CameraDev cam   = camera_dev(c->camera);
    const uint32_t  D     = num_bounces;
    std::unique_ptr<StageTimer> total(new StageTimer(c, ST_COUNT));

    const uint32_t n_batches = (n_frames + slots - 1) / slots;
    struct LaneJoin
    {
        CapContext* c;
        bool        armed = false;
        ~LaneJoin()
        {
            if (!armed) return;
            if (hipEventRecord(c->join_ev, c->stream2) != hipSuccess || hipStreamWaitEvent(c->stream, c->join_ev, 0) != hipSuccess)
                (void)hipStreamSynchronize(c->stream2);
        }
    } lane_join{c};
    if (two_lanes)
    {
        HIP_TRY(hipEventRecord(c->fork_ev, c->stream));
        HIP_TRY(hipStreamWaitEvent(c->stream2, c->fork_ev, 0));
        lane_join.armed = true;
    }
    hipEvent_t last_resolve = nullptr;
    uint32_t   batch        = 0;

    for (uint32_t done = 0; done < n_frames; done += slots, ++batch)
    {
        const uint32_t    lane = two_lanes ? ((n_batches - 1u - batch) & 1u) : 0u;
        CapContext::Lane& L    = c->lane[lane];
        const BvhDev      bvh  = bvh_dev(c, L);
        LaunchCfg         cfg{L.stream, (uint32_t)c->cu_count * blocks_per_cu, stack_entries, (uint32_t)c->cu_count};
        cfg.sw = &c->sw;
        const uint32_t ns = std::min(slots, n_frames - done);
        const FrameConst* frames = c->frames_ring[ring].p + done;
        const size_t   per_queue     = (size_t)kQueueClasses * kCounterStride;
        const size_t   counter_words = (size_t)(D + 1) * per_queue;
        HIP_TRY(hipMemsetAsync(L.counters.p, 0, sizeof(uint32_t) * 3 * counter_words, L.stream));
        uint32_t*      ext_count = L.counters.p;
        uint32_t*      sh_count  = L.counters.p + 1;
        uint32_t*      work_shade = L.counters.p + counter_words;
        uint32_t*      work_any   = L.counters.p + 2 * counter_words;
        const uint32_t total_chunks   = ns * (Ppad >> 6);
        uint32_t       class_capacity = ((total_chunks + kQueueClasses - 1) / kQueueClasses) * 64u;
        if (c->debug_capacity_div > 1) class_capacity = std::max(64u, (class_capacity / c->debug_capacity_div) & ~63u);
        c->last_class_capacity = class_capacity;
        const bool     last_batch = done + ns >= n_frames;
        const uint32_t aov_slot   = ((flags & CAP_RENDER_AOV) && last_batch) ? ns - 1 : ~0u;
        const uint32_t max_count  = ns * Ppad;

        ShadeArgs sa{};
        sa.scene = scene, sa.cam = cam, sa.screen = c->screen, sa.frames = frames, sa.hits = L.hits.p;
        sa.planes = Planes{L.pl_color.p, L.pl_direct.p, L.pl_albedo.p, c->aov_geo.p, c->aov_nd.p};
        sa.n_slots = ns, sa.num_bounces = D, sa.max_count = max_count, sa.aov_slot = aov_slot, sa.shaded_counter = c->shaded_counter.p;
        {
            const bool no_cull = c->sw.on(SW_NO_CAMERA_CULL);
            auto dotf = [](const float* x, const float* y) { return x[0] * y[0] + x[1] * y[1] + x[2] * y[2]; };
            const CapCameraData& cd = c->camera;
            const float skew = std::max({std::fabs(dotf(cd.right, cd.up)), std::fabs(dotf(cd.right, cd.forward)), std::fabs(dotf(cd.up, cd.forward)),
                                         std::fabs(dotf(cd.right, cd.right) - 1.f), std::fabs(dotf(cd.up, cd.up) - 1.f),
                                         std::fabs(dotf(cd.forward, cd.forward) - 1.f)});
            const double f = cd.focal_length, sx = cd.sensor_size[0], sy = cd.sensor_size[1];
            const double shift_x = (double)skew * c->screen.width * (f / sx + 1.0 + sy / (2.0 * sx) + (sx + sy) / (4.0 * f));
            const double shift_y = (double)skew * c->screen.height * (f / sy + 1.0 + sx / (2.0 * sy) + (sx + sy) / (4.0 * f));
            const bool   ortho   = skew < 1e-4f && shift_x <= 0.125 * (double)kCameraCullPad && shift_y <= 0.125 * (double)kCameraCullPad;
            sa.cull_camera_pairs = (ortho && !no_cull) ? 1u : 0u;
            c->last_cull_camera_pairs = sa.cull_camera_pairs;
        }
        const bool no_albedo_w = c->sw.on(SW_NO_ALBEDO_IN_W);
        sa.albedo_in_w = (!no_albedo_w && !feedback && !lowres && !(flags & CAP_RENDER_AOV) && (ext || scene.texture_count == 0)) ? 1u : 0u;
        const bool no_plane_code = c->sw.on(SW_NO_PLANE_CODE);
        sa.code_in_color = (sa.albedo_in_w && fused && !ext && !no_plane_code && trace_shade_has_code_form(bvh, scene)) ? 1u : 0u;
        if (feedback)
            sa.fb = FeedbackDev{camera_dev(c->prev_camera), c->post_prev_nd.p, c->post_chist[(frame_begin + 1) % 2].p};
        const bool no_inline_nee = c->sw.on(SW_NO_INLINE_NEE);
        sa.inline_nee = (ext && fused && !no_inline_nee) ? 1u : 0u;
        const bool no_inline_probe = c->sw.on(SW_NO_INLINE_PROBE);
        sa.inline_probe = (!ext && !feedback && fused && !no_inline_probe && c->tri_count <= kExhaustiveMax && bvh.fan_pair_count >= 1 &&
                           bvh.fan_pair_count <= kExhaustiveMax / 2)
                              ? 1u
                              : 0u;
        const bool no_wave_ring = c->sw.on(SW_NO_WAVE_RING);
        sa.wave_ring = (sa.inline_probe && !no_wave_ring && (size_t)cfg.grid_blocks * (kBlock / 64) * 128 <= std::min(L.s_org.n, L.s_con.n)) ? 1u : 0u;
        LaunchCfg cfg_any    = cfg;
        cfg_any.any_no_probe = sa.inline_probe;
        bool primary_shaded = false;
        bool any_refill = false;
        if (!fused && !ext && bvh.wide8_ok && c->tri_count > kExhaustiveMax)
        {
            const int force = (int)c->sw.v[SW_ANY_REFILL];
            const uint64_t tree_bytes = (uint64_t)c->wide8_nodes * kWideNodeStride * 4u + (uint64_t)c->tri_count * 64u;
            any_refill = force >= 0 ? force != 0 : tree_bytes >= kAnyRefillTreeBytes;
        }
        bool primary_wide = false;
        if (!fused && bvh.wide8_ok && c->tri_count > kExhaustiveMax)
        {
            const int force = (int)c->sw.v[SW_PRIMARY_WIDE];
            bool inside = true;
            for (int k = 0; k < 3; ++k)
                inside = inside && c->camera.position[k] >= c->bvh_info.bounds_lo[k] && c->camera.position[k] <= c->bvh_info.bounds_hi[k];
            const double per_pixel = (double)c->tri_count / std::max(1.0, (double)c->screen.width * c->screen.height);
            primary_wide = inside && (force >= 0 ? force != 0 : per_pixel >= kPrimaryWideTrianglesPerPixel);
        }
        for (uint32_t b = 0; b <= D; ++b)
        {
            const int pi = (int)(b & 1u), po = pi ^ 1;
            sa.bounce    = b;
            sa.in        = RayQueue{L.q_org[pi].p, L.q_dir[pi].p, L.q_thr[pi].p, b ? ext_count + (b - 1) * per_queue : nullptr, class_capacity,
                                    pi ? L.s_dir.p : L.s_org.p};
            sa.out       = RayQueue{L.q_org[po].p, L.q_dir[po].p, L.q_thr[po].p, ext_count + b * per_queue, class_capacity,
                                    po ? L.s_dir.p : L.s_org.p};
            sa.shadow    = ShadowQueue{L.s_org.p, L.s_dir.p, L.s_con.p, sh_count + b * per_queue, class_capacity};
            sa.work      = work_shade + b * per_queue;
            if (fused)
            {
                StageTimer t(c, b == 0 ? ST_PRIMARY : ST_CLOSEST, st);
                const uint32_t form = launch_trace_shade(cfg, bvh, sa, ext, feedback);
                if (b) ++c->stats.launches_trace_closest, c->last_mark_form = form;
                if (trace_launch(c, "trace_shade bounce %u batch %u", b, batch)) return fail(CAP_ERR_HIP, "trace_shade failed");
            }
            else
            {
                if (b == 0)
                {
                    {
                        StageTimer t(c, ST_PRIMARY, st);
                        if (primary_wide)
                        {
                            const uint32_t id_cap = (((max_count + kQueueClasses - 1) / kQueueClasses) + 63u) & ~63u;
                            const RayQueue idq{L.q_org[0].p, L.q_dir[0].p, nullptr, L.counters.p + 3 * counter_words, id_cap, nullptr};
                            if (c->sw.on(SW_RAYGEN_KERNEL) || bvh.tri_count == 0)
                            {
                                launch_raygen_identity(cfg, cam, c->screen, frames, ns, idq);
                                launch_trace_closest8(cfg, bvh, idq, max_count, L.hits.p, sa.work);
                            }
                            else
                                launch_trace_closest8_camera(cfg, bvh, idq, max_count, L.hits.p, sa.work, cam, c->screen, frames, ns);
                        }
                        else
                        {
                            primary_shaded = launch_primary_shade(cfg, bvh, sa, L.hits.p, ext);
                            if (!primary_shaded) launch_trace_primary(cfg, bvh, cam, c->screen, frames, ns, L.hits.p, sa.work);
                        }
                    }
                    if (aov_slot != ~0u) launch_geo_aov(cfg, scene, L.hits.p + (size_t)aov_slot * Ppad, Ppad, c->aov_geo.p);
                }
                if (b != 0 || !primary_shaded)
                {
                    StageTimer t(c, ST_SHADE, st, b == 0 ? ST_DIRECT : ST_NONE);
                    launch_shade(cfg, sa, ext, feedback);
                    ++c->stats.launches_shade;
                }
            }
            if (!sa.inline_nee && !(fused && sa.wave_ring && b != 0))
            {
                StageTimer t(c, ST_ANY, st, b == 0 ? ST_DIRECT : ST_NONE);
                if (any_refill)
                    launch_trace_any8_refill(cfg_any, bvh, sa.shadow, max_count, b == 0 ? L.pl_direct.p : L.pl_color.p, Ppad, ns, c->shaded_counter.p,
                                             work_any + b * per_queue, frames);
                else
                    launch_trace_any(cfg_any, bvh, sa.shadow, max_count, b == 0 ? L.pl_direct.p : L.pl_color.p, Ppad, ns, c->shaded_counter.p,
                                     work_any + b * per_queue,  ext, frames,
                                     (b == 0 && sa.code_in_color) ? L.pl_color.p : nullptr);
                ++c->stats.launches_trace_any;
                if (trace_launch(c, "trace_any bounce %u batch %u", b, batch)) return fail(CAP_ERR_HIP, "trace_any failed");
            }
            if (!fused && b < D)
            {
                StageTimer t(c, ST_CLOSEST, st);
                if (bvh.wide8_ok)
                    launch_trace_closest8(cfg, bvh, sa.out, max_count, L.hits.p, work_shade + (b + 1) * per_queue);
                else
                    launch_trace_closest(cfg, bvh, sa.out, max_count, L.hits.p);
                ++c->stats.launches_trace_closest;
            }
        }
        if (!lowres)
        {
            StageTimer t(c, ST_RESOLVE, st);
            if (two_lanes && last_resolve) HIP_TRY(hipStreamWaitEvent(L.stream, last_resolve, 0));
            launch_resolve(cfg, sa.planes, ns, Ppad, c->accum.p, sa.albedo_in_w != 0u, scene.kd_untextured, sa.code_in_color != 0u);
            if (two_lanes)
            {
                HIP_TRY(hipEventRecord(c->lane_ev[lane], L.stream));
                last_resolve = c->lane_ev[lane];
            }
        }
        uint32_t* pinned = nullptr;
        if (!c->pinned_pool.empty())
        {
// ... 139 lines not shown
```

### capsaicin_amd/csrc/kernels.hip

```cpp
#include "cap_exhaustive.h"
#include "cap_kernels.h"
#include "cap_reproject.h"
#include "cap_shade.h"
#include "cap_trace.h"
#include "cap_unscaled.h"
#include "cap_wide_trace.h"

#include <cassert>

namespace cap
{
template <int STACK>
__device__ __forceinline__ void traverse_closest(const BvhDev& bvh, const Ray& r, uint32_t* stack, float& best_t, float& best_u,
                                                 float& best_v, uint32_t& best_gid)
{
    best_t = r.tmax, best_u = 0.0f, best_v = 0.0f, best_gid = kInvalidId;
    if (bvh.tri_count == 0) return;
    int node = bvh.root;
    int sp   = 0;
    while (true)
    {
        if (node >= 0)
        {
            const float4 q0 = bvh.nodes[4 * node + 0], q1 = bvh.nodes[4 * node + 1], q2 = bvh.nodes[4 * node + 2],
// ... 807 lines not shown
    }
    uint32_t       gx     = (chunks + 3) / 4;
    if (gx > cfg.grid_blocks) gx = cfg.grid_blocks;
    if (gx == 0) gx = 1;
    const dim3 grid(gx, n_slots);
    BvhDev     b = bvh;
    b.wide8_ok   = 0;
    if (cfg.stack_entries == 0)
        hipLaunchKernelGGL(k_trace_primary<0>, grid, dim3(kBlock), 0, cfg.stream, b, cam, screen, frames, hits);
    else if (cfg.stack_entries <= 32)
        hipLaunchKernelGGL(k_trace_primary<32>, grid, dim3(kBlock), 0, cfg.stream, b, cam, screen, frames, hits);
    else
        hipLaunchKernelGGL(k_trace_primary<64>, grid, dim3(kBlock), 0, cfg.stream, b, cam, screen, frames, hits);
}

void launch_trace_closest(const LaunchCfg& cfg, const BvhDev& bvh, const RayQueue& q, uint32_t max_count, float4* hits)
{
    dim3 grid(queue_grid(cfg, max_count));
    if (cfg.stack_entries == 0)
        hipLaunchKernelGGL(k_trace_closest<0>, grid, dim3(kBlock), 0, cfg.stream, bvh, q, hits);
    else if (cfg.stack_entries <= 32)
    {
        grid.x = resident_grid<k_trace_closest_refill<32>>(cfg, grid.x);
        hipLaunchKernelGGL(k_trace_closest_refill<32>, grid, dim3(kBlock), 0, cfg.stream, bvh, q, hits);
    }
    else
    {
        grid.x = resident_grid<k_trace_closest_refill<64>>(cfg, grid.x);
        hipLaunchKernelGGL(k_trace_closest_refill<64>, grid, dim3(kBlock), 0, cfg.stream, bvh, q, hits);
    }
}

void launch_trace_any(const LaunchCfg& cfg, const BvhDev& bvh, const ShadowQueue& q, uint32_t max_count, float4* target,
                      uint32_t pixels_padded, uint32_t n_slots, uint64_t* guard, uint32_t* work, bool mostly_unoccluded,
                      const FrameConst* frames, float4* code_plane)
{
    assert(!code_plane || (cfg.stack_entries == 0 && !mostly_unoccluded));
    dim3         grid(queue_grid(cfg, max_count));
    const BvhDev bw = for_grid(bvh, grid.x);
    const uint32_t pre = (cfg.stack_entries == 0 && !mostly_unoccluded) ? pre_table_bytes(n_slots, bvh.fan_pair_count) : 0u;
    const bool     no_probe = cfg.sw_on(SW_NO_ANY_PROBE);
    const uint32_t probe    = (uint32_t)cfg.sw_get(SW_ANY_PROBE, CAP_ANY_PROBE);
    if (pre != 0u && work && !no_probe && !cfg.any_no_probe && bvh.fan_pair_count <= kExhaustiveMax / 2)
    {
        const uint32_t per_cu = (uint32_t)cfg.sw_get(SW_ANY_BLOCKS, 6);
        uint32_t g = (max_count + kBlock - 1) / kBlock;
        const uint32_t cap = cfg.cu_count ? cfg.cu_count * per_cu : cfg.grid_blocks;
        g = g > cap ? cap : (g ? g : 1u);
        grid = dim3(g);
        const auto kernel = code_plane ? k_trace_any_small<true> : k_trace_any_small<false>;
        hipLaunchKernelGGL(kernel, grid, dim3(kBlock), pre, cfg.stream, bw, q, target, pixels_padded, n_slots, guard, work, frames, probe, code_plane);
        return;
    }
#define CAP_LAUNCH_ANY(S, R, ...) \
    hipLaunchKernelGGL((k_trace_any<S, R, ##__VA_ARGS__>), grid, dim3(kBlock), pre, cfg.stream, bw, q, target, pixels_padded, n_slots, guard, work, frames, pre, code_plane)
    if (cfg.stack_entries == 0)
    {
        if (mostly_unoccluded)
            CAP_LAUNCH_ANY(0, true);
        else if (code_plane)
            CAP_LAUNCH_ANY(0, false, true);
        else
            CAP_LAUNCH_ANY(0, false);
    }
    else if (bw.wide8_ok)
    {
        if (mostly_unoccluded) CAP_LAUNCH_ANY((int)kWideLdsEntries, true); else CAP_LAUNCH_ANY((int)kWideLdsEntries, false);
    }
    else if (cfg.stack_entries <= 32)
    {
        if (mostly_unoccluded) CAP_LAUNCH_ANY(32, true); else CAP_LAUNCH_ANY(32, false);
    }
    else
    {
        if (mostly_unoccluded) CAP_LAUNCH_ANY(64, true); else CAP_LAUNCH_ANY(64, false);
    }
#undef CAP_LAUNCH_ANY
}

template <bool FIRST_, bool EXT_, bool FB_ = false>
struct ShadeStageCfg
{
    static constexpr bool FIRST = FIRST_, EXT = EXT_, FB = FB_;
    static constexpr bool CARRY = false, SKY_RMW = true, PROBE = false, TAME = false, LEAN = false, CODE = false;
};

template <bool FIRST, bool EXT, bool FB = false>
__global__ __launch_bounds__(kBlock) void k_shade(ShadeArgs a)
{
    using C = ShadeStageCfg<FIRST, EXT, FB>;
    const uint32_t Ppad = a.screen.pixels_padded;
    const uint32_t chunks   = FIRST ? (Ppad >> 6) : (a.in.class_capacity >> 6) * kQueueClasses;
    uint32_t       n_shaded = 0;
    __shared__ FrameConst lds_frames[kMaxFrameSlots];
    stage_frames(a, lds_frames);
    Stamps st;
    st.start();
    for (uint32_t chunk = wave_global_id(); chunk < chunks; chunk += wave_total())
    {
        uint32_t i, klass;
        bool     active;
        if (FIRST)
        {
            i      = chunk * 64 + (threadIdx.x & 63u);
            active = true;
            klass  = chunk_class(blockIdx.y * (Ppad >> 6) + chunk);
        }
        else
            active = queue_chunk(a.in.count, a.in.class_capacity, chunk, threadIdx.x & 63u, i, klass);
        uint32_t pid = 0;
        float4   hit = make_float4(0.f, 0.f, u2f(kInvalidId), 0.f);
        v3       thr = mk3(1.0f, 1.0f, 1.0f);
        if (active)
        {
            if (FIRST)
            {
                pid = (blockIdx.y << kPidShift) | i;
                hit = a.hits[(size_t)blockIdx.y * Ppad + i];
            }
            else
            {
                const float4 tp = a.in.thr_pid[i];
                thr = mk3(tp.x, tp.y, tp.z), pid = f2u(tp.w);
                hit = a.hits[i];
            }
        }
        const ShadePre pre = shade_prefetch<C>(a, lds_frames, active, pid);
        if constexpr (EXT)
        {
            v3 d = mk3(0.f, 0.f, 1.f);
            if (active)
            {
                if (FIRST)
                {
                    uint32_t x, y;
                    if (local_pixel_to_xy(a.screen, i, x, y)) d = primary_dir(a.cam, a.screen, a.frames[blockIdx.y], x, y);
                }
                else
                {
                    const float4 dq = a.in.dir_tmax[i];
                    d               = mk3(dq.x, dq.y, dq.z);
                }
            }
            shade_vertex_ext<FIRST>(a, a.scene.shade_tris, pre, klass, pid, hit, thr, d, n_shaded);
        }
        else
            shade_vertex<C>(a, a.scene.shade_tris, pre, klass, pid, hit, thr, n_shaded, st);
    }
    flush_stats(a.out.count + (size_t)(wave_global_id() % kQueueClasses) * kCounterStride, n_shaded);
}

#ifndef CAP_PS_BLOCKS
#define CAP_PS_BLOCKS 8
#endif
template <bool EXT>
__global__ __launch_bounds__(kBlock, CAP_PS_BLOCKS) void k_primary_shade(BvhDev bvh, ShadeArgs a, float4* hits_out)
{
    using C = ShadeStageCfg<true, EXT>;
    __shared__ uint32_t   lds_wstack[(kBlock / 64) * kPacketStack];
    __shared__ FrameConst lds_frames[kMaxFrameSlots];
    stage_frames(a, lds_frames);
    uint32_t*      wstack   = lds_wstack + (threadIdx.x >> 6) * kPacketStack;
    const uint32_t Ppad     = a.screen.pixels_padded;
    const uint32_t cps      = Ppad >> 6;
    const uint32_t chunks   = cps * a.n_slots;
    const uint32_t my_class = wave_global_id() % kQueueClasses;
    uint32_t       n_shaded = 0;
// ... 118 lines not shown
```

### capsaicin_amd/csrc/small_scene.hip

```cpp
#include "cap_shade.h"

#include <cassert>

namespace cap
{
#ifndef CAP_TS_FIRST
#define CAP_TS_FIRST 5
#endif
#ifndef CAP_TS_EXT
#define CAP_TS_EXT 6
#endif
#ifndef CAP_TS_NEXT
#define CAP_TS_NEXT 6
#endif
#ifdef CAP_STAMPS
__device__ unsigned long long g_wave_times[2 * 16384];
#endif
template <bool FIRST_, bool EXT_, bool FB_, bool LDS_, bool TAME_, bool CODE_ = false>
struct TraceShadeCfg
{
    static_assert(!TAME_ || (!EXT_ && !FB_ && LDS_), "TAME: reference model, scene in LDS");
    static_assert(!CODE_ || (FIRST_ && TAME_), "CODE: bounce 0 of the reference model, scene in LDS, tame records");
    static constexpr bool FIRST = FIRST_, EXT = EXT_, FB = FB_, LDS = LDS_, TAME = TAME_, CODE = CODE_;
    static constexpr bool CARRY = !EXT, SKY_RMW = false;
    static constexpr bool PROBE = !EXT && !FB && LDS;
    static constexpr bool LEAN = PROBE && TAME && kChunkLean;
    static constexpr bool ORG  = FIRST && LDS;
    static constexpr bool XT   = EXT && LDS;
    static constexpr int  kBlocksPerCu = FB ? 4 : (EXT ? (FIRST ? 5 : CAP_TS_EXT) : (FIRST ? CAP_TS_FIRST : CAP_TS_NEXT));
};

__device__ __forceinline__ void stage_scene_records(const BvhDev& bvh, const ShadeArgs& a, float4* lds_shade, float4* lds_rec)
{
    const uint32_t n = bvh.tri_count <= kExhaustiveMax ? bvh.tri_count : kExhaustiveMax;
    for (uint32_t k = threadIdx.x; k < kShadeRec * n; k += kBlock) lds_shade[k] = a.scene.shade_tris[k];
    for (uint32_t k = threadIdx.x; k < 4 * n; k += kBlock) lds_rec[k] = bvh.tris_by_id[k];
}
__device__ __forceinline__ void stage_ext_tables(const ShadeArgs& a, float* lds_mat, float* lds_lcdf, float4* lds_lrec)
{
    const float* ms = reinterpret_cast<const float*>(a.scene.materials);
    for (uint32_t k = threadIdx.x; k < 12u * a.scene.material_count; k += kBlock) lds_mat[k] = ms[k];
    for (uint32_t k = threadIdx.x; k < a.scene.light_count; k += kBlock)
    {
        lds_lcdf[k] = a.scene.light_cdf[k];
        const float4* lt = a.scene.shade_tris + kShadeRec * (size_t)a.scene.light_tris[k];
        const float4  l0 = lt[0], l1 = lt[1], l2 = lt[2];
        const v3      q0 = mk3(l0.x, l0.y, l0.z), q1 = mk3(l1.x, l1.y, l1.z), q2 = mk3(l2.x, l2.y, l2.z);
        const v3      nl = normalize3(cross3(q1 - q0, q2 - q0));
        const MaterialDev lm = a.scene.materials[f2u(lt[6].x)];
        lds_lrec[4 * k]     = make_float4(q0.x, q0.y, q0.z, lm.ke[0]);
        lds_lrec[4 * k + 1] = make_float4(q1.x, q1.y, q1.z, lm.ke[1]);
        lds_lrec[4 * k + 2] = make_float4(q2.x, q2.y, q2.z, lm.ke[2]);
        lds_lrec[4 * k + 3] = make_float4(nl.x, nl.y, nl.z, 0.f);
    }
}
__device__ __forceinline__ void stage_camera_pairs(const BvhDev& bvh, const ShadeArgs& a, float4* lds_org, float4* lds_bounds)
{
    const v3     o  = mk3(a.cam.position[0], a.cam.position[1], a.cam.position[2]);
    const float* fp = reinterpret_cast<const float*>(bvh.fan_pairs);
    for (uint32_t k = threadIdx.x; k < bvh.fan_pair_count && 2 * k + 1 < kExhaustiveMax; k += kBlock)
    {
        const float* rec  = fp + 20 * (size_t)k;
        const v3     tvec = o - mk3(rec[0], rec[1], rec[2]);
        lds_org[2 * k]     = make_float4(tvec.x, tvec.y, tvec.z, dot3(tvec, mk3(rec[12], rec[13], rec[14])));
        lds_org[2 * k + 1] = make_float4(dot3(tvec, mk3(rec[15], rec[16], rec[17])), 0.f, 0.f, 0.f);
        const v3 R = mk3(a.cam.right[0], a.cam.right[1], a.cam.right[2]), U = mk3(a.cam.up[0], a.cam.up[1], a.cam.up[2]),
                 F = mk3(a.cam.forward[0], a.cam.forward[1], a.cam.forward[2]);
        float x0 = 3.0e38f, y0 = 3.0e38f, x1 = -3.0e38f, y1 = -3.0e38f;
        bool  behind = false;
        for (int e = 0; e < 4; ++e)
        {
            const v3    d = e == 0 ? tvec * -1.0f : (mk3(rec[3 * e], rec[3 * e + 1], rec[3 * e + 2]) - tvec);
            const float z = dot3(d, F);
            behind |= !(z > 1e-4f);
            const float px = ((a.cam.focal_length * dot3(d, R) / z) / a.cam.sensor_x + 0.5f) * (float)a.screen.width;
            const float py = ((a.cam.focal_length * dot3(d, U) / z) / a.cam.sensor_y + 0.5f) * (float)a.screen.height;
            x0 = fminf(x0, px), x1 = fmaxf(x1, px), y0 = fminf(y0, py), y1 = fmaxf(y1, py);
        }
        const bool usable = a.cull_camera_pairs != 0u && !behind && x0 == x0 && y0 == y0 && x1 == x1 && y1 == y1;
        lds_bounds[k] = usable ? make_float4(x0 - kCameraCullPad, y0 - kCameraCullPad, x1 + kCameraCullPad, y1 + kCameraCullPad) : make_float4(-3.0e38f, -3.0e38f, 3.0e38f, 3.0e38f);
    }
}
__device__ __forceinline__ void stage_probe_rows(const BvhDev& bvh, const ShadeArgs& a, float* lds_pscore, uint32_t& probe_k, float4* lds_probe)
{
    const uint32_t np = bvh.fan_pair_count;
    const float*   fp = reinterpret_cast<const float*>(bvh.fan_pairs);
    if (threadIdx.x < np)
    {
        const float* rec = fp + 20 * (size_t)threadIdx.x;
        const v3     L   = mk3(a.frames[0].light_dir[0], a.frames[0].light_dir[1], a.frames[0].light_dir[2]);
        const v3     v0  = mk3(rec[0], rec[1], rec[2]);
        float        sc  = dot3(v0, L);
        for (int e = 0; e < 3; ++e) sc += dot3(v0 + mk3(rec[3 + 3 * e], rec[4 + 3 * e], rec[5 + 3 * e]), L);
        lds_pscore[threadIdx.x] = sc;
    }
    __syncthreads();
    if (threadIdx.x < np)
    {
        const float sc   = lds_pscore[threadIdx.x];
        uint32_t    rank = 0;
        for (uint32_t j = 0; j < np; ++j)
        {
            const float o = lds_pscore[j];
            rank += (o > sc || (o == sc && j < threadIdx.x)) ? 1u : 0u;
        }
        if (rank == 0) probe_k = threadIdx.x;
    }
    __syncthreads();
    const float* rec = fp + 20 * (size_t)probe_k;
    for (uint32_t sl = threadIdx.x; sl < a.n_slots && sl < kMaxFrameSlots; sl += kBlock)
    {
        const v3 d = mk3(a.frames[sl].light_dir[0], a.frames[sl].light_dir[1], a.frames[sl].light_dir[2]);
        lds_probe[2 * sl]     = tri_pre(d, mk3(rec[12], rec[13], rec[14]), kRayEps, kRayFar);
        lds_probe[2 * sl + 1] = tri_pre(d, mk3(rec[15], rec[16], rec[17]), kRayEps, kRayFar);
    }
}

template <bool FIRST, bool EXT, bool FB = false, bool LDS = false, bool TAME = false, bool CODE = false>
__global__ __launch_bounds__(kBlock, (TraceShadeCfg<FIRST, EXT, FB, LDS, TAME, CODE>::kBlocksPerCu)) void k_trace_shade(BvhDev bvh, ShadeArgs a)
{
    using C = TraceShadeCfg<FIRST, EXT, FB, LDS, TAME, CODE>;
    const uint32_t Ppad     = a.screen.pixels_padded;
    const uint32_t cps      = Ppad >> 6;
    const uint32_t chunks   = FIRST ? cps * a.n_slots : (a.in.class_capacity >> 6) * kQueueClasses;
    uint32_t       n_shaded = 0, n_probed = 0;
    __shared__ FrameConst lds_frames[kMaxFrameSlots];
    __shared__ float4     lds_shade[LDS ? kShadeRec * kExhaustiveMax : 1];
    __shared__ float4     lds_rec[LDS ? 4 * kExhaustiveMax : 1];
    __shared__ float4     lds_probe[C::PROBE ? 2 * kMaxFrameSlots : 1];
    __shared__ float      lds_pscore[C::PROBE ? kExhaustiveMax / 2 : 1];
    __shared__ SlotSample lds_first[(C::LEAN && FIRST) ? kMaxFrameSlots : 1];
    __shared__ uint32_t   lds_probe_k;
    __shared__ float4     lds_ring[(C::PROBE && !FIRST) ? (kBlock / 64) * kWaveRing : 1];
    __shared__ float4     lds_org[C::ORG ? kExhaustiveMax : 1];
    __shared__ float4     lds_bounds[C::ORG ? kExhaustiveMax / 2 : 1];
    __shared__ float      lds_mat[C::XT ? 12 * kExhaustiveMax : 1];
    __shared__ float      lds_lcdf[C::XT ? kExtLightsMax : 1];
    __shared__ float4     lds_lrec[C::XT ? 4 * kExtLightsMax : 1];
    const bool            ext_tabs = C::XT && a.scene.material_count <= kExhaustiveMax && a.scene.light_count <= kExtLightsMax;
    if (LDS)
    {
        stage_scene_records(bvh, a, lds_shade, lds_rec);
        if (C::XT && ext_tabs) stage_ext_tables(a, lds_mat, lds_lcdf, lds_lrec);
        if (C::ORG) stage_camera_pairs(bvh, a, lds_org, lds_bounds);
    }
    if (C::PROBE && a.inline_probe) stage_probe_rows(bvh, a, lds_pscore, lds_probe_k, lds_probe);
    if constexpr (C::LEAN)
        stage_frames_samples<FIRST>(a, lds_frames, lds_first);
    else
        stage_frames(a, lds_frames);
    ProbeArgs probe;
    if (C::PROBE && a.inline_probe) probe.rows = lds_probe, probe.pairs = bvh.fan_pairs, probe.k = lds_probe_k;
    uint32_t ring_head = 0, ring_n = 0;
    if (C::PROBE && !FIRST && a.inline_probe && a.wave_ring)
    {
        probe.ring_org = lds_ring + (threadIdx.x >> 6) * kWaveRing;
        probe.ring_con = a.shadow.contrib_pid + (size_t)wave_global_id() * kWaveRing;
    }
    auto trace_ring = [&](uint32_t count) {
        wave_handoff();
        const uint32_t lane_ = threadIdx.x & 63u;
        const bool     on    = lane_ < count;
        const uint32_t pos   = (ring_head + lane_) & (kWaveRing - 1u);
        float4         o     = make_float4(0.f, 0.f, 0.f, 0.f);
        if (on) o = probe.ring_org[pos];
        const uint32_t spid = f2u(o.w);
        const bool     good = on && (spid >> kPidShift) < a.n_slots && (spid & kPidMask) < Ppad;
        const FrameConst& fc = lds_frames[good ? (spid >> kPidShift) : 0u];
        const Ray  sr = make_ray(mk3(o.x, o.y, o.z), mk3(fc.light_dir[0], fc.light_dir[1], fc.light_dir[2]), kRayEps, good ? kRayFar : kRayEps);
        float4* const target = a.bounce == 0 ? a.planes.direct : a.planes.color;
        const size_t  idx    = good ? (size_t)(spid >> kPidShift) * Ppad + (spid & kPidMask) : 0;
        float4        c = make_float4(0.f, 0.f, 0.f, 0.f), cur = c;
        if (good) c = probe.ring_con[pos], cur = target[idx];
        const bool occluded = exhaustive_any<false>(bvh, sr);
        if (good && !occluded) target[idx] = make_float4(cur.x + c.x, cur.y + c.y, cur.z + c.z, cur.w);
        ring_head = (ring_head + count) & (kWaveRing - 1u);
        ring_n -= count;
    };
    const float4* shade_tab = LDS ? lds_shade : a.scene.shade_tris;
    const float4* rec_tab   = LDS ? lds_rec : bvh.tris_by_id;
    ExtTables     xtabs;
    if (C::XT && ext_tabs) xtabs.materials = reinterpret_cast<const MaterialDev*>(lds_mat), xtabs.light_cdf = lds_lcdf, xtabs.light_rec = lds_lrec;
    Stamps st;
    st.start();
    const uint32_t my_class = wave_global_id() % kQueueClasses;
    const uint32_t lane     = threadIdx.x & 63u;
    uint32_t       n_class  = 0;
    if (!FIRST)
    {
        n_class = a.in.count[my_class * kCounterStride];
        n_class = n_class < a.in.class_capacity ? n_class : a.in.class_capacity;
    }
    uint32_t grab = grab_issue(a.work, my_class);
    while (true)
    {
        const uint32_t j = grab_value(grab);
        uint32_t       i, pid = 0, slot = 0;
        const uint32_t klass = my_class;
        bool           active;
        v3             thr = mk3(1.0f, 1.0f, 1.0f);
        Ray            r   = make_ray(mk3(0.f, 0.f, 0.f), mk3(0.f, 0.f, 1.f), 0.0f, 0.0f);
        float          carried_r1 = 0.f, carried_r2 = 0.f;
        if (FIRST)
        {
            const uint32_t chunk = class_chunk(j, my_class);
            if (chunk >= chunks) break;
            grab   = grab_issue(a.work, my_class);
            slot   = chunk / cps;
            i      = (chunk - slot * cps) * 64 + lane;
            active = true;
            pid    = (slot << kPidShift) | i;
            uint32_t x, y;
            if (local_pixel_to_xy(a.screen, i, x, y))
                r = make_ray(mk3(a.cam.position[0], a.cam.position[1], a.cam.position[2]),
                             primary_dir(a.cam, a.screen, lds_frames[slot], x, y), 0.0f, kPrimaryFar);
        }
        else
        {
            if (j * 64u >= n_class) break;
            active = j * 64u + lane < n_class;
            if constexpr (C::LEAN)
            {
                const uint32_t local = j * 64u + lane;
                i                    = my_class * a.in.class_capacity + (local < n_class ? local : n_class - 1u);
                const float4 o = a.in.org_tmin[i], d = a.in.dir_tmax[i], tp = a.in.thr_pid[i];
                grab = grab_issue(a.work, my_class);
                r    = make_ray(mk3(o.x, o.y, o.z), mk3(d.x, d.y, d.z), kRayEps, kRayFar);
                thr  = mk3(tp.x, tp.y, tp.z), pid = f2u(tp.w);
                carried_r1 = o.w, carried_r2 = d.w;
            }
            else
            {
                i      = my_class * a.in.class_capacity + j * 64u + lane;
                float4 o = make_float4(0.f, 0.f, 0.f, 0.f), d = make_float4(0.f, 0.f, 1.f, 0.f), tp = make_float4(1.f, 1.f, 1.f, 0.f);
                if (active) o = a.in.org_tmin[i], d = a.in.dir_tmax[i], tp = a.in.thr_pid[i];
                grab = grab_issue(a.work, my_class);
                if (active)
                {
                    r   = make_ray(mk3(o.x, o.y, o.z), mk3(d.x, d.y, d.z), kRayEps, kRayFar);
                    thr = mk3(tp.x, tp.y, tp.z), pid = f2u(tp.w);
                    carried_r1 = o.w, carried_r2 = d.w;
                }
            }
        }
        float    t, u, v;
        uint32_t gid;
        STAMP(st, 0, true);
        uint32_t pair_mask = ~0u;
        if (C::ORG)
        {
            uint32_t tx = 0, ty = 0;
            (void)local_pixel_to_xy(a.screen, i & ~63u, tx, ty);
            const float4 b    = lds_bounds[lane < kExhaustiveMax / 2 ? lane : 0u];
            const bool   over = lane < bvh.fan_pair_count && b.x < (float)(tx + 8u) && b.z >= (float)tx && b.y < (float)(ty + 8u) && b.w >= (float)ty;
            pair_mask         = (uint32_t)__ballot(over);
        }
        __builtin_amdgcn_s_setprio(0);
#if !defined(CAP_CLOSEST_V1)
        if constexpr (LDS && !C::ORG)
        {
            if (bvh.tri_count > 32u)
                exhaustive_closest_marked<true>(bvh, rec_tab, r, active, t, u, v, gid);
            else
                exhaustive_closest_marked<false>(bvh, rec_tab, r, active, t, u, v, gid);
        }
        else
#endif
            exhaustive_closest<C::ORG, !LDS>(bvh, rec_tab, r, t, u, v, gid, lds_org, pair_mask);
        __builtin_amdgcn_s_setprio(3);
        STAMP(st, 1, true);
        const ShadePre pre = shade_prefetch<C>(a, lds_frames, active, pid, carried_r1, carried_r2, lds_first);
        if (FIRST && slot == a.aov_slot)
        {
            float4 g = make_float4(0.f, 0.f, u2f(kInvalidId), u2f(kInvalidId));
            if (gid != kInvalidId)
            {
                const uint4 id = a.scene.tri_ids[gid];
                g              = make_float4(u, v, u2f(id.x), u2f(id.y));
            }
            a.planes.aov_geo[i] = g;
        }
        if constexpr (EXT)
        {
            if (a.inline_nee)
            {
                v3 acc = mk3(0.f, 0.f, 0.f);
                if (!FIRST && active)
                {
                    const float4 q = a.in.acc[i];
                    acc            = mk3(q.x, q.y, q.z);
                }
                shade_vertex_ext<FIRST, true>(a, shade_tab, pre, klass, pid, make_float4(u, v, u2f(gid), t), thr, r.d, n_shaded, &bvh, acc, xtabs);
            }
            else
                shade_vertex_ext<FIRST>(a, shade_tab, pre, klass, pid, make_float4(u, v, u2f(gid), t), thr, r.d, n_shaded, nullptr, mk3(0.f, 0.f, 0.f), xtabs);
        }
        else
        {
            shade_vertex<C>(a, shade_tab, pre, klass, pid, make_float4(u, v, u2f(gid), t), thr, n_shaded, st, probe, &n_probed, ring_head, &ring_n);
            if (C::PROBE && ring_n >= 64u) trace_ring(64u);
        }
        STAMP(st, 4, false);
    }
    if (!FIRST && !EXT && !FB) st.flush();
#ifdef CAP_STAMPS
    if (!FIRST && !EXT && !FB && (threadIdx.x & 63u) == 0 && wave_global_id() < 16384)
    {
        g_wave_times[2 * wave_global_id() + 0] = st.t_begin;
        g_wave_times[2 * wave_global_id() + 1] = __builtin_amdgcn_s_memrealtime();
    }
#endif
    if (C::PROBE && ring_n != 0u) trace_ring(ring_n);
    flush_stats(a.out.count + (size_t)my_class * kCounterStride, n_shaded, n_probed);
}

#ifdef CAP_STAMPS
extern "C" int cap_debug_stamps(unsigned long long* out, int reset)
{
    if (reset == 2) return (int)hipMemcpyFromSymbol(out, HIP_SYMBOL(g_wave_times), 2 * 16384 * sizeof(unsigned long long));
    hipError_t e = hipMemcpyFromSymbol(out, HIP_SYMBOL(g_stamps), 8 * sizeof(unsigned long long));
    if (e == hipSuccess && reset)
    {
        unsigned long long z[16] = {};
        e = hipMemcpyToSymbol(HIP_SYMBOL(g_stamps), z, sizeof(z));
    }
    return (int)e;
}
#endif

__device__ __forceinline__ uint32_t selftest_hash32(uint32_t x)
{
    x ^= x >> 16, x *= 0x7feb352du, x ^= x >> 15, x *= 0x846ca68bu, x ^= x >> 16;
    return x;
}
__global__ __launch_bounds__(kBlock) void k_shade_forms_selftest(unsigned long long* out, uint32_t which)
{
    const uint32_t     tid = blockIdx.x * kBlock + threadIdx.x, total = gridDim.x * kBlock;
    unsigned long long bad = 0, n = 0;
    auto               differ = [](float x, float y) { return f2u(x) != f2u(y) ? 1u : 0u; };
    if (which == 0)
    {
        for (uint64_t b = ((127ull - 96ull) << 23) + tid; b <= 0x7f7fffffull; b += total)
        {
            const float x = u2f((uint32_t)b), s = sqrtf(x);
            bad += differ(sqrt_pos(x), s) + differ(sqrt_unscaled(x), s), n += 2;
        }
        if (tid < 3)
        {
            const float x = tid == 0 ? 0.0f : (tid == 1 ? -0.0f : __builtin_inff());
            bad += differ(sqrt_unscaled(x), sqrtf(x)), ++n;
        }
        for (uint64_t b = (uint64_t)f2u(kNormLo) + tid; b <= f2u(kNormHi); b += total)
        {
            const float x = u2f((uint32_t)b);
            bad += differ(div_unscaled(1.0f, sqrt_pos(x)), 1.0f / sqrtf(x)), ++n;
        }
        for (uint64_t b = tid; b <= f2u(2.0f); b += total)
        {
            const float x = u2f((uint32_t)b), pdf = x / kPi, fast = div_unscaled(x, kPi);
            if (b == 0 || b >= ((127ull - 80ull) << 23))
                bad += differ(fast, pdf);
            else
                bad += (fast < 1e-5f && fast > -1e-5f) ? 0u : 1u;
            ++n;
            if (!(pdf < 1e-5f)) bad += differ(div_unscaled(kInvPi * fmaxf(x, 0.0f), pdf), (kInvPi * fmaxf(x, 0.0f)) / pdf), ++n;
        }
    }
    else
    {
        for (uint64_t i = tid; i < (1ull << 31); i += total)
        {
            const uint32_t h0 = selftest_hash32((uint32_t)i), h1 = selftest_hash32((uint32_t)i ^ 0x9e3779b9u), h2 = selftest_hash32(h0 + h1);
            const uint32_t e1 = 82u + h2 % 90u, d = (h2 >> 8) % 96u, e0 = e1 > d ? e1 - d : 1u;
            float          p = u2f((e1 << 23) | (h0 & 0x007fffffu) | ((h2 << 3) & 0x80000000u));
            float          q = u2f((e0 << 23) | (h1 & 0x007fffffu) | ((h2 << 2) & 0x80000000u));
            if ((h2 >> 24 & 7u) == 0u) q = (h2 & 0x08000000u) ? 0.0f : -0.0f;
            const bool  sw = (h2 >> 27 & 1u) != 0u;
            const float a = sw ? q : p, b = sw ? p : q, g = fmaf(a, a, b * b);
            if (!ortho_in_range(a, b, g)) continue;
            const float k = sqrtf(g), kf = sqrt_pos(g);
            float       qa, qb;
            div2_unscaled(a, b, kf, qa, qb);
            bad += differ(kf, k) + differ(qa, a / k) + differ(qb, b / k), ++n;
        }
    }
    if (bad) atomicAdd(&out[0], bad);
    atomicAdd(&out[1], n);
}

void launch_shade_forms_selftest(hipStream_t stream, unsigned long long* out_device, uint32_t which)
{
    hipLaunchKernelGGL(k_shade_forms_selftest, dim3(4096), dim3(kBlock), 0, stream, out_device, which);
}

enum : uint32_t { TS_FIRST = 1, TS_EXT = 2, TS_FB = 4, TS_LDS = 8, TS_TAME = 16, TS_CODE = 32 };
struct TraceShadeKernel
{
    uint32_t is;
    void (*kernel)(BvhDev, ShadeArgs);
};
template <uint32_t IS>
constexpr TraceShadeKernel trace_shade_kernel()
{
    return {IS, k_trace_shade<(IS & TS_FIRST) != 0, (IS & TS_EXT) != 0, (IS & TS_FB) != 0, (IS & TS_LDS) != 0, (IS & TS_TAME) != 0, (IS & TS_CODE) != 0>};
}
constexpr TraceShadeKernel kTraceShadeKernels[13] = {
    trace_shade_kernel<TS_FIRST | TS_LDS | TS_TAME | TS_CODE>(),
    trace_shade_kernel<TS_FIRST | TS_EXT | TS_LDS>(), trace_shade_kernel<TS_FIRST | TS_EXT>(),
    trace_shade_kernel<TS_FIRST | TS_LDS | TS_TAME>(), trace_shade_kernel<TS_FIRST | TS_LDS>(), trace_shade_kernel<TS_FIRST>(),
    trace_shade_kernel<TS_EXT | TS_LDS>(), trace_shade_kernel<TS_EXT>(),
    trace_shade_kernel<TS_FB | TS_LDS>(), trace_shade_kernel<TS_FB>(),
    trace_shade_kernel<TS_LDS | TS_TAME>(), trace_shade_kernel<TS_LDS>(), trace_shade_kernel<0>(),
};

static bool tame_kernels(const BvhDev& bvh, const SceneDev& scene)
{
#if defined(CAP_SHADE_IEEE)
    return false;
#else
    return bvh.tri_count <= kExhaustiveMax && scene.shade_tame != 0;
#endif
}
bool trace_shade_has_code_form(const BvhDev& bvh, const SceneDev& scene) { return tame_kernels(bvh, scene); }

uint32_t launch_trace_shade(const LaunchCfg& cfg, const BvhDev& bvh, const ShadeArgs& args, bool ext, bool feedback)
{
    const bool first = args.bounce == 0;
    const bool fb    = feedback && !ext && !first;
    const bool lds   = bvh.tri_count <= kExhaustiveMax;
    const bool tame  = !ext && !fb && tame_kernels(bvh, args.scene);
    const bool code  = first && args.code_in_color != 0u;
    assert(!code || tame);
    const uint32_t is = (first ? TS_FIRST : 0u) | (ext ? TS_EXT : 0u) | (fb ? TS_FB : 0u) | (lds ? TS_LDS : 0u) | (tame ? TS_TAME : 0u) | (code ? TS_CODE : 0u);
    const uint32_t gx = queue_grid(cfg, first ? args.screen.pixels_padded * args.n_slots : args.max_count);
    const TraceShadeKernel* k = kTraceShadeKernels;
    while (k->is != is && k + 1 < kTraceShadeKernels + 13) ++k;
    assert(k->is == is);
    hipLaunchKernelGGL(k->kernel, dim3(gx), dim3(kBlock), 0, cfg.stream, bvh, args);
#if defined(CAP_CLOSEST_V1)
    return 0u;
#else
    if (!lds || first) return 0u;
    return (kMarkCarry && bvh.tri_ids_dense) ? (bvh.tri_count > 32u ? 3u : 2u) : 1u;
#endif
}
}
```

### include/capsaicin_hip.h

```cpp
#ifndef CAPSAICIN_HIP_H
#define CAPSAICIN_HIP_H

#include <stddef.h>
#include <stdint.h>

#ifdef __cplusplus
extern "C" {
#endif

typedef struct CapContext CapContext;

typedef enum CapStatus
{
    CAP_OK                = 0,
    CAP_ERR_INVALID_ARG   = 1,
    CAP_ERR_HIP           = 2,
    CAP_ERR_STATE         = 3,
    CAP_ERR_UNSUPPORTED   = 4,
    CAP_ERR_IO            = 5
} CapStatus;

typedef struct CapCameraData
{
    float position[3];
// ... 74 lines not shown
    double   ms_post;
    uint64_t post_frames;
    double   ms_direct;
    double   ms_post_pass[5];
    uint64_t shadow_entries;
    uint64_t shadow_entries_bounce0;
    uint64_t guard_append;
    uint64_t lane1_dropped;
} CapStats;

typedef struct CapBvhInfo
{
    uint32_t triangle_count;
    uint32_t node_count;
    uint32_t max_depth;
    uint32_t stack_entries;
    float    bounds_lo[3];
    float    bounds_hi[3];
    double   build_ms;
} CapBvhInfo;

const char* cap_last_error(void);
int cap_device_count(void);

int  cap_ctx_create(int device_id, void* hip_stream, CapContext** out_ctx);
void cap_ctx_destroy(CapContext* ctx);

int cap_scene_upload(CapContext* ctx, const float* positions, const float* normals, const float* texcoords,
                     const uint32_t* indices, const CapMeshDesc* meshes, uint32_t vertex_count, uint32_t index_count,
                     uint32_t mesh_count);
int cap_texture_upload(CapContext* ctx, uint32_t index, const uint8_t* rgba8, uint32_t width, uint32_t height);
int cap_bluenoise_upload(CapContext* ctx, const uint8_t* rgba8_256x256);
int cap_materials_upload(CapContext* ctx, const CapMaterial* materials, uint32_t mesh_count);

int cap_bvh_build(CapContext* ctx);
typedef enum CapBvhBuild
{
    CAP_BVH_BUILD_AUTO = 0,
    CAP_BVH_BUILD_LBVH = 1,
    CAP_BVH_BUILD_SAH  = 2,
    CAP_BVH_BUILD_PLOC = 3,
    CAP_BVH_BUILD_SAH_DEVICE = 4
} CapBvhBuild;
int cap_set_bvh_build(CapContext* ctx, uint32_t mode);
int cap_bvh_info(CapContext* ctx, CapBvhInfo* out);
int cap_bvh_readback(CapContext* ctx, float* nodes, uint32_t* leaf_triangles);
int cap_bvh_wide_readback(CapContext* ctx, uint32_t* nodes, uint32_t* tri_src, uint32_t* info);

enum
{
    CAP_VERTICES_DEVICE = 1u << 0
};
int cap_scene_update_vertices(CapContext* ctx, const float* positions, const float* normals, const float* texcoords, uint32_t flags);
typedef struct CapRefitInfo
{
    double ms;
    double expected_node_visits;
    double expected_node_visits_built;
} CapRefitInfo;
int cap_bvh_refit(CapContext* ctx, CapRefitInfo* out);

int cap_camera_set(CapContext* ctx, const CapCameraData* camera);
int cap_prev_camera_set(CapContext* ctx, const CapCameraData* camera);
int cap_set_resolution(CapContext* ctx, uint32_t width, uint32_t height);
int cap_set_shard(CapContext* ctx, uint32_t shard_index, uint32_t shard_count);
int cap_set_batch_paths(CapContext* ctx, uint64_t max_paths);
enum
{
    CAP_DEBUG_QUEUE_CAPACITY_DIV = 1,
    CAP_DEBUG_WIDE_DEPTH_LIMIT   = 2,
    CAP_DEBUG_WIDE_IN_USE        = 3,
    CAP_DEBUG_FAIL_LANE1         = 4,
    CAP_DEBUG_LANES_USED         = 5,
    CAP_DEBUG_QUEUE_CANARY_FILL   = 6,
    CAP_DEBUG_QUEUE_CANARY_BEHIND = 7,
    CAP_DEBUG_QUEUE_CANARY_USED   = 8,
    CAP_DEBUG_SELFTEST_DIV        = 9,
    CAP_DEBUG_NEE_PAIRS           = 10,
    CAP_DEBUG_SELFTEST_SHADE_UNARY = 11,
    CAP_DEBUG_SELFTEST_SHADE_DIV2  = 12,
    CAP_DEBUG_SHADE_TAME           = 13,
    CAP_DEBUG_CAMERA_CULL          = 14,
    CAP_DEBUG_MARK_FORM            = 15,
    CAP_DEBUG_SWITCH_BASE         = 64
};
int cap_debug_set(CapContext* ctx, uint32_t key, uint64_t value);
int cap_debug_get(CapContext* ctx, uint32_t key, uint64_t* value);
int cap_debug_switch_index(const char* name);
int cap_debug_pair_ids_dense(const float* pair_records, uint32_t pair_count, uint32_t single_count, uint32_t tri_count);
int cap_debug_query_ranges(uint64_t n, uint32_t count, const uint64_t* base, const uint64_t* stride, const uint32_t* align);
int cap_debug_closest_instance_bound(const float* transform, const float* box_lo, const float* box_hi, const float* point, float best_dist2,
                                     float* world_to_object, float* g, float* xw, float* slack, uint32_t* skip);
typedef enum CapTraversal
{
    CAP_TRAVERSAL_AUTO       = 0,
    CAP_TRAVERSAL_STACK      = 1,
    CAP_TRAVERSAL_EXHAUSTIVE = 2
} CapTraversal;
int cap_set_traversal(CapContext* ctx, uint32_t mode);

int cap_render(CapContext* ctx, uint32_t frame_begin, uint32_t n_frames, uint32_t num_bounces, uint32_t flags);
int cap_accum_reset(CapContext* ctx);
int cap_accum_import(CapContext* ctx, const float* sum_rgba, uint64_t frames);
int cap_sync(CapContext* ctx);

int cap_readback(CapContext* ctx, CapBufferKind kind, float* dst);

int cap_stats_get(CapContext* ctx, CapStats* out);
int cap_stats_reset(CapContext* ctx);

typedef struct CapRayDesc
{
    float origin[3];
    float tmin;
    float direction[3];
    float tmax;
} CapRayDesc;
typedef struct CapHit
{
    float    t;
    float    u;
    float    v;
    uint32_t triangle;
} CapHit;
int cap_trace_rays(CapContext* ctx, const CapRayDesc* device_rays, uint64_t n, CapHit* device_hits, uint32_t flags);
int cap_trace_occlusion(CapContext* ctx, const CapRayDesc* device_rays, uint64_t n, uint32_t* device_occluded, uint32_t flags);

#define CAP_MULTI_MAX_K 16
enum
{
    CAP_MULTI_CONTINUE = 1u << 0
};
int cap_trace_rays_multi(CapContext* ctx, const CapRayDesc* device_rays, uint64_t n, uint32_t k, CapHit* device_hits, uint32_t* device_counts,
                         uint32_t flags);

enum
{
    CAP_RAY_FLAG_ACCEPT_FIRST_HIT  = 0x04,
    CAP_RAY_FLAG_CULL_BACK_FACING  = 0x10,
    CAP_RAY_FLAG_CULL_FRONT_FACING = 0x20
};
typedef struct CapTraceOptions
{
    uint32_t ray_flags;
    uint32_t instance_mask;
    uint32_t reserved[2];
} CapTraceOptions;
int cap_scene_set_instance_masks(CapContext* ctx, const uint8_t* masks, uint32_t mesh_count);
int cap_trace_rays_ex(CapContext* ctx, const CapRayDesc* device_rays, uint64_t n, CapHit* device_hits, const CapTraceOptions* options);
int cap_trace_occlusion_ex(CapContext* ctx, const CapRayDesc* device_rays, uint64_t n, uint32_t* device_occluded,
                           const CapTraceOptions* options);
int cap_trace_rays_multi_ex(CapContext* ctx, const CapRayDesc* device_rays, uint64_t n, uint32_t k, CapHit* device_hits,
                            uint32_t* device_counts, uint32_t multi_flags, const CapTraceOptions* options);

typedef struct CapPointDesc
{
    float point[3];
    float radius;
} CapPointDesc;
typedef struct CapClosest
{
    float    point[3];
    float    dist2;
    float    u, v;
    uint32_t triangle;
    uint32_t feature;
// ... 149 lines not shown
```

Before: 56320 Mrays/s.

## Precompute per-slot bluenoise hemisphere sample terms into a table before bounces

Adds a pre-pass kernel that computes, for every slot, bounce and 64x64 bluenoise cell, the hemisphere sampling terms (sin/cos products and cos_theta). The fused lean trace-shade kernels then read these terms from the table instead of carrying r1/r2 in the ray queue and recomputing sincos and square roots per ray. The aim is to cut transcendental ALU work and the bluenoise staging in the shading path. The cost is an extra launch per batch, a table buffer, and a global memory gather per shaded ray. A switch controls it, a self-test verifies the table, and it is on by default.

```diff
diff --git a/capsaicin_amd/capi.py b/capsaicin_amd/capi.py
--- a/capsaicin_amd/capi.py
+++ b/capsaicin_amd/capi.py
@@ -578,6 +578,8 @@
     DEBUG_SELFTEST_SHADE_UNARY, DEBUG_SELFTEST_SHADE_DIV2, DEBUG_SHADE_TAME = 11, 12, 13
     DEBUG_CAMERA_CULL = 14
     DEBUG_MARK_FORM = 15
+    DEBUG_SAMPLE_TABLE = 16
+    DEBUG_SELFTEST_SAMPLE_TABLE = 17
 
     def debug_set(self, key, value):
         _check(lib().cap_debug_set(self.ctx, key, value), "cap_debug_set")
diff --git a/capsaicin_amd/csrc/cap_context.h b/capsaicin_amd/csrc/cap_context.h
--- a/capsaicin_amd/csrc/cap_context.h
+++ b/capsaicin_amd/csrc/cap_context.h
@@ -175,6 +175,12 @@
     uint32_t      last_class_capacity = 0;
     uint32_t      tri_ids_dense = 0;
     uint32_t      last_mark_form = 0;
+    uint32_t      last_sample_table = 0;
+    struct LastTerms
+    {
+        const FrameConst* frames = nullptr;
+        uint32_t          n_slots = 0, num_bounces = 0, lane = 0;
+    } last_terms;
     uint32_t      last_cull_camera_pairs = 0;
     uint32_t      traversal_mode  = CAP_TRAVERSAL_AUTO;
     uint32_t      bvh_build_mode  = CAP_BVH_BUILD_AUTO;
@@ -185,6 +191,7 @@
     {
         hipStream_t      stream = nullptr;
         DevBuf<float4>   hits, q_org[2], q_dir[2], q_thr[2], s_org, s_dir, s_con, pl_color, pl_direct, pl_albedo;
+        DevBuf<float4>   terms;
         DevBuf<uint32_t> counters;
         DevBuf<uint32_t> stack_spill;
     } lane[2];
diff --git a/capsaicin_amd/csrc/cap_kernels.h b/capsaicin_amd/csrc/cap_kernels.h
--- a/capsaicin_amd/csrc/cap_kernels.h
+++ b/capsaicin_amd/csrc/cap_kernels.h
@@ -36,6 +36,7 @@
     SW_NO_NEE_PAIR_CULL,
     SW_RAYGEN_KERNEL,
     SW_NO_PLANE_CODE,
+    SW_SAMPLE_TABLE,
     SW_COUNT
 };
 struct SwitchTable
@@ -221,7 +222,11 @@
     CameraDev         cam;
     ScreenDev         screen;
     const FrameConst* frames;
-    const float4*     hits;
+    union
+    {
+        const float4* hits;
+        const float4* sample_terms;
+    };
     RayQueue          in;
     RayQueue          out;
     ShadowQueue       shadow;
@@ -248,6 +253,10 @@
 bool launch_primary_shade(const LaunchCfg& cfg, const BvhDev& bvh, const ShadeArgs& args, float4* hits, bool ext);
 uint32_t launch_trace_shade(const LaunchCfg& cfg, const BvhDev& bvh, const ShadeArgs& args, bool ext, bool feedback = false);
 bool trace_shade_has_code_form(const BvhDev& bvh, const SceneDev& scene);
+bool trace_shade_has_table_form(const BvhDev& bvh, const SceneDev& scene);
+void launch_sample_terms(hipStream_t stream, const float2* bluenoise, const FrameConst* frames, uint32_t n_slots, uint32_t num_bounces, float4* table);
+void launch_sample_terms_selftest(hipStream_t stream, const float2* bluenoise, const FrameConst* frames, uint32_t n_slots, uint32_t num_bounces,
+                                  const float4* table, unsigned long long* out_device);
 
 void launch_resolve(const LaunchCfg& cfg, const Planes& planes, uint32_t n_slots, uint32_t pixels_padded, float4* accum,
                     bool albedo_in_w = false, float kd_untextured = 0.0f, bool code_in_color = false);
diff --git a/capsaicin_amd/csrc/cap_shade.h b/capsaicin_amd/csrc/cap_shade.h
--- a/capsaicin_amd/csrc/cap_shade.h
+++ b/capsaicin_amd/csrc/cap_shade.h
@@ -52,7 +52,20 @@
     const uint32_t     xa = (f2u(a) & 0x7fffffffu) - 1u, xb = (f2u(b) & 0x7fffffffu) - 1u;
     return (f2u(g) - kG0 < kG1 - kG0) & ((xa < xb ? xa : xb) >= kX0 - 1u);
 }
-__device__ __forceinline__ v3 map_to_hemisphere_tame(float r1, float r2, v3 n)
+struct HemiTerms
+{
+    float ca, cb, cos_theta;
+};
+__device__ __forceinline__ HemiTerms hemisphere_terms(float r1, float r2)
+{
+    float sin_psi, cos_psi;
+    sincos_c((2.0f * kPi) * r1, sin_psi, cos_psi);
+    const float cos_theta = sqrt_pos(1.0f - r2);
+    const float sin_theta = sqrt_unscaled(1.0f - cos_theta * cos_theta);
+    return HemiTerms{sin_theta * cos_psi, sin_theta * sin_psi, cos_theta};
+}
+template <class Terms>
+__device__ __forceinline__ v3 hemisphere_dir_tame(v3 n, Terms terms)
 {
     const bool  zn = fabsf(n.z) > 0.0f;
     const float a = zn ? n.z : n.y, b = zn ? n.y : n.x;
@@ -73,14 +86,15 @@
     v3       u = zn ? mk3(0.0f, -q1, q2) : mk3(q1, -q2, 0.0f);
     const v3 v = cross3(u, n);
     u          = cross3(n, v);
-    float sin_psi, cos_psi;
-    sincos_c((2.0f * kPi) * r1, sin_psi, cos_psi);
-    const float cos_theta = sqrt_pos(1.0f - r2);
-    const float sin_theta = sqrt_unscaled(1.0f - cos_theta * cos_theta);
-    const float ca = sin_theta * cos_psi, cb = sin_theta * sin_psi;
+    const HemiTerms h = terms();
+    const float     cos_theta = h.cos_theta, ca = h.ca, cb = h.cb;
     const v3    d = mk3(fmaf(n.x, cos_theta, fmaf(v.x, cb, u.x * ca)), fmaf(n.y, cos_theta, fmaf(v.y, cb, u.y * ca)),
                         fmaf(n.z, cos_theta, fmaf(v.z, cb, u.z * ca)));
     return fast ? normalize3_tame(d) : normalize3(d);
+}
+__device__ __forceinline__ v3 map_to_hemisphere_tame(float r1, float r2, v3 n)
+{
+    return hemisphere_dir_tame(n, [=] { return hemisphere_terms(r1, r2); });
 }
 
 __device__ __forceinline__ void oct_encode(v3 n, float& ox, float& oy)
@@ -190,7 +204,7 @@
     s0 = a - floorf(a);
     s1 = b - floorf(b);
 }
-template <bool FIRST>
+template <bool FIRST, bool TAB = false>
 __device__ __forceinline__ void stage_frames_samples(const ShadeArgs& a, FrameConst* lds_frames, SlotSample* lds_first)
 {
     constexpr uint32_t kWords = (uint32_t)(sizeof(FrameConst) / 4);
@@ -205,7 +219,7 @@
         {
             const uint32_t sl = i / kWords, w = i - sl * kWords;
             v = src[i];
-            if (w == 7u || w == 11u)
+            if (!TAB && (w == 7u || w == 11u))
             {
                 const uint32_t next = src[sl * kWords + 2u] * 25u + a.bounce + 1u;
                 v = w == 7u ? bluenoise_offset(next) : f2u(bluenoise_shift(next));
@@ -213,7 +227,7 @@
         }
         dst[i] = v;
     }
-    if (FIRST)
+    if (FIRST && !TAB)
         for (uint32_t sl = threadIdx.x; sl < kMaxFrameSlots; sl += kBlock)
         {
             SlotSample ss = {0u, 0.0f};
@@ -235,7 +249,7 @@
     const uint32_t slot = pid >> kPidShift, pl = pid & kPidMask;
     if constexpr (C::LEAN)
     {
-        static_assert(C::CARRY && !C::EXT, "LEAN: the reference model's fused kernels");
+        static_assert((C::CARRY != C::TAB) && !C::EXT, "LEAN: the reference model's fused kernels, the sample carried or from the table");
         const uint32_t    sl = slot < kMaxFrameSlots ? slot : 0;
         const FrameConst& fc = lds_frames[sl];
         uint32_t          base;
@@ -245,7 +259,7 @@
             uint32_t x = 0, y = 0;
             s.valid = active && local_pixel_to_xy(a.screen, pl, x, y);
             if (fc.lowres_sel & 4u) s.indirect_on = (x & 1u) == ((fc.lowres_sel >> 1) & 1u) && (y & 1u) == (fc.lowres_sel & 1u);
-            base = bluenoise_base(x, y);
+            base = C::TAB ? ((y & 63u) << 6) | (x & 63u) : bluenoise_base(x, y);
         }
         else
         {
@@ -253,7 +267,8 @@
             const uint32_t gt = __umul24(pl >> 6, a.screen.shard_count) + a.screen.shard_index;
             const uint32_t ty = tile_div(gt, a.screen.tiles_x_mul, a.screen.tiles_x_shift);
             const uint32_t tx = gt + (ty & 7u) * ((0u - a.screen.tiles_x) & 7u);
-            base = ((ty & 7u) << 13) | ((pl & 0x38u) << 7) | ((tx & 7u) << 5) | ((pl & 7u) << 2);
+            base = C::TAB ? ((ty & 7u) << 9) | ((pl & 0x38u) << 3) | ((tx & 7u) << 3) | (pl & 7u)
+                          : ((ty & 7u) << 13) | ((pl & 0x38u) << 7) | ((tx & 7u) << 5) | ((pl & 7u) << 2);
         }
         s.L = unread3(), s.I = unread3(), s.r1 = s.r2 = s.r1n = s.r2n = unread_f();
         s.r3 = s.r4 = s.r5 = s.r6 = 0.f;
@@ -261,6 +276,15 @@
         {
             s.L = mk3(fc.light_dir[0], fc.light_dir[1], fc.light_dir[2]);
             s.I = mk3(fc.light_intensity[0], fc.light_intensity[1], fc.light_intensity[2]);
+            if constexpr (C::TAB)
+            {
+                if (a.bounce < a.num_bounces)
+                {
+                    const float4 q = a.sample_terms[((slot < a.n_slots ? slot : 0u) << 12) | base];
+                    s.r1 = q.x, s.r2 = q.y, s.r1n = q.z;
+                }
+                return s;
+            }
             if (C::FIRST)
             {
                 const SlotSample ss = lds_first[sl];
@@ -508,7 +532,10 @@
                 const bool more = a.bounce < a.num_bounces;
                 if (!C::TAME || more)
                 {
-                    dir             = C::TAME ? map_to_hemisphere_tame(pre.r1, pre.r2, n) : map_to_hemisphere(pre.r1, pre.r2, n);
+                    if constexpr (C::TAB)
+                        dir = hemisphere_dir_tame(n, [&] { return HemiTerms{pre.r1, pre.r2, pre.r1n}; });
+                    else
+                        dir = C::TAME ? map_to_hemisphere_tame(pre.r1, pre.r2, n) : map_to_hemisphere(pre.r1, pre.r2, n);
                     const float ndd = dot3(n, dir);
                     const float pdf = C::TAME ? div_unscaled(fmaxf(0.0f, ndd), kPi) : fmaxf(0.0f, ndd) / kPi;
                     if (!(pdf < 1e-5f))
diff --git a/capsaicin_amd/csrc/context.hip b/capsaicin_amd/csrc/context.hip
--- a/capsaicin_amd/csrc/context.hip
+++ b/capsaicin_amd/csrc/context.hip
@@ -258,29 +258,31 @@
 
 struct LaneSizes
 {
-    size_t planes, queues, rings, counters;
+    size_t planes, queues, rings, counters, terms;
 };
 
-LaneSizes lane_sizes(const CapContext* c, uint32_t slots, uint32_t bounces)
+LaneSizes lane_sizes(const CapContext* c, uint32_t slots, uint32_t bounces, bool sample_table)
 {
     LaneSizes z;
     z.planes = (size_t)slots * c->screen.pixels_padded;
     z.queues = z.planes + (size_t)kQueueClasses * 64;
     z.rings = std::max(z.queues, (size_t)std::max(c->cu_count, 1) * 8 * (kBlock / 64) * 128);
     z.counters = (3 * (size_t)(bounces + 1) + 1) * kQueueClasses * kCounterStride;
+    z.terms = sample_table ? (size_t)slots * bounces * 4096 : 0;
     return z;
 }
 
-bool lane_grows(const CapContext::Lane& L, const LaneSizes& z) { return L.pl_color.n < z.planes || L.counters.n < z.counters; }
-
-int ensure_lane(CapContext* c, CapContext::Lane& L, uint32_t slots, uint32_t bounces)
-{
-    const LaneSizes z = lane_sizes(c, slots, bounces);
+bool lane_grows(const CapContext::Lane& L, const LaneSizes& z) { return L.pl_color.n < z.planes || L.counters.n < z.counters || L.terms.n < z.terms; }
+
+int ensure_lane(CapContext* c, CapContext::Lane& L, uint32_t slots, uint32_t bounces, bool sample_table)
+{
+    const LaneSizes z = lane_sizes(c, slots, bounces, sample_table);
     for (DevBuf<float4>* b : {&L.hits, &L.q_org[0], &L.q_org[1], &L.q_dir[0], &L.q_dir[1], &L.q_thr[0], &L.q_thr[1], &L.s_dir})
         HIP_TRY(b->ensure(z.queues));
     for (DevBuf<float4>* b : {&L.s_org, &L.s_con}) HIP_TRY(b->ensure(z.rings));
     for (DevBuf<float4>* b : {&L.pl_color, &L.pl_direct, &L.pl_albedo}) HIP_TRY(b->ensure(z.planes));
     HIP_TRY(L.counters.ensure(z.counters));
+    if (z.terms) HIP_TRY(L.terms.ensure(z.terms));
     if (c->lane[0].stack_spill.n) HIP_TRY(L.stack_spill.ensure(c->lane[0].stack_spill.n));
     return CAP_OK;
 }
@@ -392,7 +394,7 @@
     "CAP_NO_WIDE8", "CAP_LANE1_PRIORITY", "CAP_PLOC_RADIUS", "CAP_SAHDEV_LEAF", "CAP_WIDE_HOST_COLLAPSE", "CAP_TRACE_LAUNCHES", "CAP_NO_TWO_LANES",
     "CAP_LANE_SPLIT_MIN", "CAP_BLOCKS_PER_CU", "CAP_NO_CAMERA_CULL", "CAP_NO_ALBEDO_IN_W", "CAP_NO_INLINE_NEE", "CAP_NO_INLINE_PROBE", "CAP_NO_WAVE_RING",
     "CAP_ANY_REFILL", "CAP_PRIMARY_WIDE", "CAP_NO_PACKET", "CAP_NO_ANY_PROBE", "CAP_ANY_PROBE", "CAP_ANY_BLOCKS", "CAP_NO_PRIMARY_FUSE", "CAP_W8_REFILL",
-    "CAP_W8_GRID", "CAP_AUTO_SAH_TRIANGLES", "CAP_NO_NEE_PAIR_CULL", "CAP_RAYGEN_KERNEL", "CAP_NO_PLANE_CODE"};
+    "CAP_W8_GRID", "CAP_AUTO_SAH_TRIANGLES", "CAP_NO_NEE_PAIR_CULL", "CAP_RAYGEN_KERNEL", "CAP_NO_PLANE_CODE", "CAP_SAMPLE_TABLE"};
 
 static void switches_from_environment(SwitchTable& t)
 {
@@ -704,6 +706,26 @@
         if (!c->bvh_ready) return fail(CAP_ERR_STATE, "cap_debug_get: BVH not built");
         *value = ((uint64_t)c->last_mark_form << 8) | c->tri_ids_dense;
         return CAP_OK;
+    case CAP_DEBUG_SAMPLE_TABLE: *value = c->last_sample_table; return CAP_OK;
+    case CAP_DEBUG_SELFTEST_SAMPLE_TABLE:
+    {
+        const CapContext::LastTerms& lt = c->last_terms;
+        if (!c->last_sample_table || !lt.frames) return fail(CAP_ERR_STATE, "cap_debug_get: the last cap_render built no sample table");
+        HIP_TRY(hipSetDevice(c->device));
+        if (sync_and_collect(c) != CAP_OK) return CAP_ERR_HIP;
+        DevBuf<unsigned long long> d;
+        unsigned long long         h[2] = {0, 0};
+        HIP_TRY(d.ensure(2));
+        HIP_TRY(hipMemsetAsync(d.p, 0, sizeof(h), c->stream));
+        launch_sample_terms_selftest(c->stream, c->bluenoise.p, lt.frames, lt.n_slots, lt.num_bounces, c->lane[lt.lane].terms.p, d.p);
+        HIP_TRY(hipGetLastError());
+        HIP_TRY(hipMemcpyAsync(h, d.p, sizeof(h), hipMemcpyDeviceToHost, c->stream));
+        HIP_TRY(hipStreamSynchronize(c->stream));
+        const unsigned long long expected = (unsigned long long)lt.n_slots * lt.num_bounces * 4096ull;
+        if (h[1] != expected) return fail(CAP_ERR_HIP, "cap_debug_get: the sample table self-test compared %llu of %llu entries", h[1], expected);
+        *value = (h[0] << 32) | (expected >> 12);
+        return CAP_OK;
+    }
     case CAP_DEBUG_NEE_PAIRS:
         if (!c->bvh_ready) return fail(CAP_ERR_STATE, "cap_debug_get: BVH not built");
         *value = ((uint64_t)(c->fan_pairs_nee.p ? c->fan_pair_nee_count : c->fan_pair_count) << 32) | c->fan_pair_count;
@@ -787,6 +809,8 @@
     if (!n_frames) return CAP_OK;
     HIP_TRY(hipSetDevice(c->device));
     c->last_mark_form   = 0;
+    c->last_sample_table = 0;
+    c->last_terms        = CapContext::LastTerms{};
     const bool feedback = (flags & CAP_RENDER_GBUFFER_FEEDBACK) != 0;
     if (feedback)
     {
@@ -818,9 +842,12 @@
     bool              two_lanes = policy.two_lanes;
     if (c->spans.size() > 2048 || c->pending.size() > 64 || c->post_marks.size() > 256)
         if (sync_and_collect(c) != CAP_OK) return CAP_ERR_HIP;
-    const LaneSizes need = lane_sizes(c, slots, num_bounces);
+    const bool sample_table = fused && !ext && !feedback && num_bounces >= 1 && c->sw.get(SW_SAMPLE_TABLE, 1) != 0 &&
+                              trace_shade_has_table_form(bvh_dev(c, c->lane[0]), scene_dev(c));
+    c->last_sample_table = sample_table ? 1u : 0u;
+    const LaneSizes need = lane_sizes(c, slots, num_bounces, sample_table);
     if (lane_grows(c->lane[0], need) || !c->accum.p || c->accum.n < Ppad) HIP_TRY(hipStreamSynchronize(c->stream));
-    if (ensure_lane(c, c->lane[0], slots, num_bounces) != CAP_OK || ensure_frame_buffers(c) != CAP_OK) return CAP_ERR_HIP;
+    if (ensure_lane(c, c->lane[0], slots, num_bounces, sample_table) != CAP_OK || ensure_frame_buffers(c) != CAP_OK) return CAP_ERR_HIP;
     if (policy.lane1_failed_before)
     {
         size_t free_b = 0, total_b = 0;
@@ -838,7 +865,7 @@
             HIP_TRY(hipStreamSynchronize(c->stream));
             if (c->stream2) HIP_TRY(hipStreamSynchronize(c->stream2));
         }
-        if (c->debug_fail_lane || ensure_lane(c, c->lane[1], slots, num_bounces) != CAP_OK || ensure_lane_streams(c) != CAP_OK)
+        if (c->debug_fail_lane || ensure_lane(c, c->lane[1], slots, num_bounces, sample_table) != CAP_OK || ensure_lane_streams(c) != CAP_OK)
         {
             (void)hipGetLastError();
             c->lane[1] = CapContext::Lane{};
@@ -928,7 +955,8 @@
         const uint32_t max_count  = ns * Ppad;
 
         ShadeArgs sa{};
-        sa.scene = scene, sa.cam = cam, sa.screen = c->screen, sa.frames = frames, sa.hits = L.hits.p;
+        sa.scene = scene, sa.cam = cam, sa.screen = c->screen, sa.frames = frames;
+        if (!fused) sa.hits = L.hits.p;
         sa.planes = Planes{L.pl_color.p, L.pl_direct.p, L.pl_albedo.p, c->aov_geo.p, c->aov_nd.p};
         sa.n_slots = ns, sa.num_bounces = D, sa.max_count = max_count, sa.aov_slot = aov_slot, sa.shaded_counter = c->shaded_counter.p;
         {
@@ -980,10 +1008,17 @@
             const double per_pixel = (double)c->tri_count / std::max(1.0, (double)c->screen.width * c->screen.height);
             primary_wide = inside && (force >= 0 ? force != 0 : per_pixel >= kPrimaryWideTrianglesPerPixel);
         }
+        if (sample_table)
+        {
+            launch_sample_terms(L.stream, scene.bluenoise, frames, ns, D, L.terms.p);
+            c->last_terms = CapContext::LastTerms{frames, ns, D, lane};
+            if (trace_launch(c, "sample_terms batch %u", batch)) return fail(CAP_ERR_HIP, "sample_terms failed");
+        }
         for (uint32_t b = 0; b <= D; ++b)
         {
             const int pi = (int)(b & 1u), po = pi ^ 1;
             sa.bounce    = b;
+            if (fused) sa.sample_terms = sample_table ? L.terms.p + (size_t)(b < D ? b : 0u) * ns * 4096 : nullptr;
             sa.in        = RayQueue{L.q_org[pi].p, L.q_dir[pi].p, L.q_thr[pi].p, b ? ext_count + (b - 1) * per_queue : nullptr, class_capacity,
                                     pi ? L.s_dir.p : L.s_org.p};
             sa.out       = RayQueue{L.q_org[po].p, L.q_dir[po].p, L.q_thr[po].p, ext_count + b * per_queue, class_capacity,
diff --git a/capsaicin_amd/csrc/kernels.hip b/capsaicin_amd/csrc/kernels.hip
--- a/capsaicin_amd/csrc/kernels.hip
+++ b/capsaicin_amd/csrc/kernels.hip
@@ -913,7 +913,7 @@
 struct ShadeStageCfg
 {
     static constexpr bool FIRST = FIRST_, EXT = EXT_, FB = FB_;
-    static constexpr bool CARRY = false, SKY_RMW = true, PROBE = false, TAME = false, LEAN = false, CODE = false;
+    static constexpr bool CARRY = false, SKY_RMW = true, PROBE = false, TAME = false, LEAN = false, CODE = false, TAB = false;
 };
 
 template <bool FIRST, bool EXT, bool FB = false>
diff --git a/capsaicin_amd/csrc/small_scene.hip b/capsaicin_amd/csrc/small_scene.hip
--- a/capsaicin_amd/csrc/small_scene.hip
+++ b/capsaicin_amd/csrc/small_scene.hip
@@ -16,13 +16,14 @@
 #ifdef CAP_STAMPS
 __device__ unsigned long long g_wave_times[2 * 16384];
 #endif
-template <bool FIRST_, bool EXT_, bool FB_, bool LDS_, bool TAME_, bool CODE_ = false>
+template <bool FIRST_, bool EXT_, bool FB_, bool LDS_, bool TAME_, bool CODE_ = false, bool TAB_ = false>
 struct TraceShadeCfg
 {
     static_assert(!TAME_ || (!EXT_ && !FB_ && LDS_), "TAME: reference model, scene in LDS");
     static_assert(!CODE_ || (FIRST_ && TAME_), "CODE: bounce 0 of the reference model, scene in LDS, tame records");
-    static constexpr bool FIRST = FIRST_, EXT = EXT_, FB = FB_, LDS = LDS_, TAME = TAME_, CODE = CODE_;
-    static constexpr bool CARRY = !EXT, SKY_RMW = false;
+    static_assert(!TAB_ || (TAME_ && kChunkLean), "TAB: the lean kernels (reference model, scene in LDS, tame records)");
+    static constexpr bool FIRST = FIRST_, EXT = EXT_, FB = FB_, LDS = LDS_, TAME = TAME_, CODE = CODE_, TAB = TAB_;
+    static constexpr bool CARRY = !EXT && !TAB, SKY_RMW = false;
     static constexpr bool PROBE = !EXT && !FB && LDS;
     static constexpr bool LEAN = PROBE && TAME && kChunkLean;
     static constexpr bool ORG  = FIRST && LDS;
@@ -119,199 +120,16 @@
 template <bool FIRST, bool EXT, bool FB = false, bool LDS = false, bool TAME = false, bool CODE = false>
 __global__ __launch_bounds__(kBlock, (TraceShadeCfg<FIRST, EXT, FB, LDS, TAME, CODE>::kBlocksPerCu)) void k_trace_shade(BvhDev bvh, ShadeArgs a)
 {
-    using C = TraceShadeCfg<FIRST, EXT, FB, LDS, TAME, CODE>;
-    const uint32_t Ppad     = a.screen.pixels_padded;
-    const uint32_t cps      = Ppad >> 6;
-    const uint32_t chunks   = FIRST ? cps * a.n_slots : (a.in.class_capacity >> 6) * kQueueClasses;
-    uint32_t       n_shaded = 0, n_probed = 0;
-    __shared__ FrameConst lds_frames[kMaxFrameSlots];
-    __shared__ float4     lds_shade[LDS ? kShadeRec * kExhaustiveMax : 1];
-    __shared__ float4     lds_rec[LDS ? 4 * kExhaustiveMax : 1];
-    __shared__ float4     lds_probe[C::PROBE ? 2 * kMaxFrameSlots : 1];
-    __shared__ float      lds_pscore[C::PROBE ? kExhaustiveMax / 2 : 1];
-    __shared__ SlotSample lds_first[(C::LEAN && FIRST) ? kMaxFrameSlots : 1];
-    __shared__ uint32_t   lds_probe_k;
-    __shared__ float4     lds_ring[(C::PROBE && !FIRST) ? (kBlock / 64) * kWaveRing : 1];
-    __shared__ float4     lds_org[C::ORG ? kExhaustiveMax : 1];
-    __shared__ float4     lds_bounds[C::ORG ? kExhaustiveMax / 2 : 1];
-    __shared__ float      lds_mat[C::XT ? 12 * kExhaustiveMax : 1];
-    __shared__ float      lds_lcdf[C::XT ? kExtLightsMax : 1];
-    __shared__ float4     lds_lrec[C::XT ? 4 * kExtLightsMax : 1];
-    const bool            ext_tabs = C::XT && a.scene.material_count <= kExhaustiveMax && a.scene.light_count <= kExtLightsMax;
-    if (LDS)
-    {
-        stage_scene_records(bvh, a, lds_shade, lds_rec);
-        if (C::XT && ext_tabs) stage_ext_tables(a, lds_mat, lds_lcdf, lds_lrec);
-        if (C::ORG) stage_camera_pairs(bvh, a, lds_org, lds_bounds);
-    }
-    if (C::PROBE && a.inline_probe) stage_probe_rows(bvh, a, lds_pscore, lds_probe_k, lds_probe);
-    if constexpr (C::LEAN)
-        stage_frames_samples<FIRST>(a, lds_frames, lds_first);
-    else
-        stage_frames(a, lds_frames);
-    ProbeArgs probe;
-    if (C::PROBE && a.inline_probe) probe.rows = lds_probe, probe.pairs = bvh.fan_pairs, probe.k = lds_probe_k;
-    uint32_t ring_head = 0, ring_n = 0;
-    if (C::PROBE && !FIRST && a.inline_probe && a.wave_ring)
-    {
-        probe.ring_org = lds_ring + (threadIdx.x >> 6) * kWaveRing;
-        probe.ring_con = a.shadow.contrib_pid + (size_t)wave_global_id() * kWaveRing;
-    }
-    auto trace_ring = [&](uint32_t count) {
-        wave_handoff();
-        const uint32_t lane_ = threadIdx.x & 63u;
-        const bool     on    = lane_ < count;
-        const uint32_t pos   = (ring_head + lane_) & (kWaveRing - 1u);
-        float4         o     = make_float4(0.f, 0.f, 0.f, 0.f);
-        if (on) o = probe.ring_org[pos];
-        const uint32_t spid = f2u(o.w);
-        const bool     good = on && (spid >> kPidShift) < a.n_slots && (spid & kPidMask) < Ppad;
-        const FrameConst& fc = lds_frames[good ? (spid >> kPidShift) : 0u];
-        const Ray  sr = make_ray(mk3(o.x, o.y, o.z), mk3(fc.light_dir[0], fc.light_dir[1], fc.light_dir[2]), kRayEps, good ? kRayFar : kRayEps);
-        float4* const target = a.bounce == 0 ? a.planes.direct : a.planes.color;
-        const size_t  idx    = good ? (size_t)(spid >> kPidShift) * Ppad + (spid & kPidMask) : 0;
-        float4        c = make_float4(0.f, 0.f, 0.f, 0.f), cur = c;
-        if (good) c = probe.ring_con[pos], cur = target[idx];
-        const bool occluded = exhaustive_any<false>(bvh, sr);
-        if (good && !occluded) target[idx] = make_float4(cur.x + c.x, cur.y + c.y, cur.z + c.z, cur.w);
-        ring_head = (ring_head + count) & (kWaveRing - 1u);
-        ring_n -= count;
-    };
-    const float4* shade_tab = LDS ? lds_shade : a.scene.shade_tris;
-    const float4* rec_tab   = LDS ? lds_rec : bvh.tris_by_id;
-    ExtTables     xtabs;
-    if (C::XT && ext_tabs) xtabs.materials = reinterpret_cast<const MaterialDev*>(lds_mat), xtabs.light_cdf = lds_lcdf, xtabs.light_rec = lds_lrec;
-    Stamps st;
-    st.start();
-    const uint32_t my_class = wave_global_id() % kQueueClasses;
-    const uint32_t lane     = threadIdx.x & 63u;
-    uint32_t       n_class  = 0;
-    if (!FIRST)
-    {
-        n_class = a.in.count[my_class * kCounterStride];
-        n_class = n_class < a.in.class_capacity ? n_class : a.in.class_capacity;
-    }
-    uint32_t grab = grab_issue(a.work, my_class);
-    while (true)
-    {
-        const uint32_t j = grab_value(grab);
-        uint32_t       i, pid = 0, slot = 0;
-        const uint32_t klass = my_class;
-        bool           active;
-        v3             thr = mk3(1.0f, 1.0f, 1.0f);
-        Ray            r   = make_ray(mk3(0.f, 0.f, 0.f), mk3(0.f, 0.f, 1.f), 0.0f, 0.0f);
-        float          carried_r1 = 0.f, carried_r2 = 0.f;
-        if (FIRST)
-        {
-            const uint32_t chunk = class_chunk(j, my_class);
-            if (chunk >= chunks) break;
-            grab   = grab_issue(a.work, my_class);
-            slot   = chunk / cps;
-            i      = (chunk - slot * cps) * 64 + lane;
-            active = true;
-            pid    = (slot << kPidShift) | i;
-            uint32_t x, y;
-            if (local_pixel_to_xy(a.screen, i, x, y))
-                r = make_ray(mk3(a.cam.position[0], a.cam.position[1], a.cam.position[2]),
-                             primary_dir(a.cam, a.screen, lds_frames[slot], x, y), 0.0f, kPrimaryFar);
-        }
-        else
-        {
-            if (j * 64u >= n_class) break;
-            active = j * 64u + lane < n_class;
-            if constexpr (C::LEAN)
-            {
-                const uint32_t local = j * 64u + lane;
-                i                    = my_class * a.in.class_capacity + (local < n_class ? local : n_class - 1u);
-                const float4 o = a.in.org_tmin[i], d = a.in.dir_tmax[i], tp = a.in.thr_pid[i];
-                grab = grab_issue(a.work, my_class);
-                r    = make_ray(mk3(o.x, o.y, o.z), mk3(d.x, d.y, d.z), kRayEps, kRayFar);
-                thr  = mk3(tp.x, tp.y, tp.z), pid = f2u(tp.w);
-                carried_r1 = o.w, carried_r2 = d.w;
-            }
-            else
-            {
-                i      = my_class * a.in.class_capacity + j * 64u + lane;
-                float4 o = make_float4(0.f, 0.f, 0.f, 0.f), d = make_float4(0.f, 0.f, 1.f, 0.f), tp = make_float4(1.f, 1.f, 1.f, 0.f);
-                if (active) o = a.in.org_tmin[i], d = a.in.dir_tmax[i], tp = a.in.thr_pid[i];
-                grab = grab_issue(a.work, my_class);
-                if (active)
-                {
-                    r   = make_ray(mk3(o.x, o.y, o.z), mk3(d.x, d.y, d.z), kRayEps, kRayFar);
-                    thr = mk3(tp.x, tp.y, tp.z), pid = f2u(tp.w);
-                    carried_r1 = o.w, carried_r2 = d.w;
-                }
-            }
-        }
-        float    t, u, v;
-        uint32_t gid;
-        STAMP(st, 0, true);
-        uint32_t pair_mask = ~0u;
-        if (C::ORG)
-        {
-            uint32_t tx = 0, ty = 0;
-            (void)local_pixel_to_xy(a.screen, i & ~63u, tx, ty);
-            const float4 b    = lds_bounds[lane < kExhaustiveMax / 2 ? lane : 0u];
-            const bool   over = lane < bvh.fan_pair_count && b.x < (float)(tx + 8u) && b.z >= (float)tx && b.y < (float)(ty + 8u) && b.w >= (float)ty;
-            pair_mask         = (uint32_t)__ballot(over);
-        }
-        __builtin_amdgcn_s_setprio(0);
-#if !defined(CAP_CLOSEST_V1)
-        if constexpr (LDS && !C::ORG)
-        {
-            if (bvh.tri_count > 32u)
-                exhaustive_closest_marked<true>(bvh, rec_tab, r, active, t, u, v, gid);
-            else
-                exhaustive_closest_marked<false>(bvh, rec_tab, r, active, t, u, v, gid);
-        }
-        else
-#endif
-            exhaustive_closest<C::ORG, !LDS>(bvh, rec_tab, r, t, u, v, gid, lds_org, pair_mask);
-        __builtin_amdgcn_s_setprio(3);
-        STAMP(st, 1, true);
-        const ShadePre pre = shade_prefetch<C>(a, lds_frames, active, pid, carried_r1, carried_r2, lds_first);
-        if (FIRST && slot == a.aov_slot)
-        {
-            float4 g = make_float4(0.f, 0.f, u2f(kInvalidId), u2f(kInvalidId));
-            if (gid != kInvalidId)
-            {
-                const uint4 id = a.scene.tri_ids[gid];
-                g              = make_float4(u, v, u2f(id.x), u2f(id.y));
-            }
-            a.planes.aov_geo[i] = g;
-        }
-        if constexpr (EXT)
-        {
-            if (a.inline_nee)
-            {
-                v3 acc = mk3(0.f, 0.f, 0.f);
-                if (!FIRST && active)
-                {
-                    const float4 q = a.in.acc[i];
-                    acc            = mk3(q.x, q.y, q.z);
-                }
-                shade_vertex_ext<FIRST, true>(a, shade_tab, pre, klass, pid, make_float4(u, v, u2f(gid), t), thr, r.d, n_shaded, &bvh, acc, xtabs);
-            }
-            else
-                shade_vertex_ext<FIRST>(a, shade_tab, pre, klass, pid, make_float4(u, v, u2f(gid), t), thr, r.d, n_shaded, nullptr, mk3(0.f, 0.f, 0.f), xtabs);
-        }
-        else
-        {
-            shade_vertex<C>(a, shade_tab, pre, klass, pid, make_float4(u, v, u2f(gid), t), thr, n_shaded, st, probe, &n_probed, ring_head, &ring_n);
-            if (C::PROBE && ring_n >= 64u) trace_ring(64u);
-        }
-        STAMP(st, 4, false);
-    }
-    if (!FIRST && !EXT && !FB) st.flush();
-#ifdef CAP_STAMPS
-    if (!FIRST && !EXT && !FB && (threadIdx.x & 63u) == 0 && wave_global_id() < 16384)
-    {
-        g_wave_times[2 * wave_global_id() + 0] = st.t_begin;
-        g_wave_times[2 * wave_global_id() + 1] = __builtin_amdgcn_s_memrealtime();
-    }
-#endif
-    if (C::PROBE && ring_n != 0u) trace_ring(ring_n);
-    flush_stats(a.out.count + (size_t)my_class * kCounterStride, n_shaded, n_probed);
+    using C            = TraceShadeCfg<FIRST, EXT, FB, LDS, TAME, CODE>;
+    constexpr bool TAB = false;
+#include "small_scene_body.h"
+}
+template <bool FIRST, bool CODE>
+__global__ __launch_bounds__(kBlock, (TraceShadeCfg<FIRST, false, false, true, true, CODE, kChunkLean>::kBlocksPerCu)) void k_trace_shade_tab(BvhDev bvh, ShadeArgs a)
+{
+    using C            = TraceShadeCfg<FIRST, false, false, true, true, CODE, kChunkLean>;
+    constexpr bool EXT = false, FB = false, LDS = true, TAB = kChunkLean;
+#include "small_scene_body.h"
 }
 
 #ifdef CAP_STAMPS
@@ -393,7 +211,53 @@
     hipLaunchKernelGGL(k_shade_forms_selftest, dim3(4096), dim3(kBlock), 0, stream, out_device, which);
 }
 
-enum : uint32_t { TS_FIRST = 1, TS_EXT = 2, TS_FB = 4, TS_LDS = 8, TS_TAME = 16, TS_CODE = 32 };
+__global__ __launch_bounds__(kBlock) void k_sample_terms(const float2* bluenoise, const FrameConst* frames, uint32_t n_slots, uint32_t num_bounces, float4* table)
+{
+    const uint32_t tid = blockIdx.x * kBlock + threadIdx.x, row = tid >> 12, at = tid & 4095u;
+    if (row >= n_slots * num_bounces) return;
+    const uint32_t b = row / n_slots, sl = row - b * n_slots;
+    const uint32_t count = frames[sl].frame_count * 25u + b;
+    float          r1, r2;
+    bluenoise_at(bluenoise, bluenoise_base(at & 63u, at >> 6), bluenoise_offset(count), bluenoise_shift(count), r1, r2);
+    const HemiTerms h = hemisphere_terms(r1, r2);
+    table[tid]        = make_float4(h.ca, h.cb, h.cos_theta, 0.0f);
+}
+
+void launch_sample_terms(hipStream_t stream, const float2* bluenoise, const FrameConst* frames, uint32_t n_slots, uint32_t num_bounces, float4* table)
+{
+    const uint32_t rows = n_slots * num_bounces;
+    if (!rows) return;
+    hipLaunchKernelGGL(k_sample_terms, dim3(rows * (4096u / kBlock)), dim3(kBlock), 0, stream, bluenoise, frames, n_slots, num_bounces, table);
+}
+
+__global__ __launch_bounds__(kBlock) void k_sample_terms_selftest(const float2* bluenoise, const FrameConst* frames, uint32_t n_slots, uint32_t num_bounces,
+                                                                  const float4* table, unsigned long long* out)
+{
+    const uint32_t tid = blockIdx.x * kBlock + threadIdx.x, row = tid >> 12, at = tid & 4095u;
+    if (row >= n_slots * num_bounces) return;
+    const uint32_t b = row / n_slots, sl = row - b * n_slots;
+    float          r1, r2;
+    bluenoise4x4(bluenoise, at & 63u, at >> 6, frames[sl].frame_count * 25u + b, r1, r2);
+    const HemiTerms h = hemisphere_terms(r1, r2);
+    const float4    q = table[tid];
+    const bool      bad = f2u(q.x) != f2u(h.ca) || f2u(q.y) != f2u(h.cb) || f2u(q.z) != f2u(h.cos_theta) || f2u(q.w) != 0u;
+    const unsigned long long mb = __ballot(bad), mn = __ballot(true);
+    if ((threadIdx.x & 63u) == 0u)
+    {
+        if (mb) atomicAdd(&out[0], (unsigned long long)__popcll(mb));
+        atomicAdd(&out[1], (unsigned long long)__popcll(mn));
+    }
+}
+
+void launch_sample_terms_selftest(hipStream_t stream, const float2* bluenoise, const FrameConst* frames, uint32_t n_slots, uint32_t num_bounces,
+                                  const float4* table, unsigned long long* out_device)
+{
+    const uint32_t rows = n_slots * num_bounces;
+    if (!rows) return;
+    hipLaunchKernelGGL(k_sample_terms_selftest, dim3(rows * (4096u / kBlock)), dim3(kBlock), 0, stream, bluenoise, frames, n_slots, num_bounces, table, out_device);
+}
+
+enum : uint32_t { TS_FIRST = 1, TS_EXT = 2, TS_FB = 4, TS_LDS = 8, TS_TAME = 16, TS_CODE = 32, TS_TAB = 64 };
 struct TraceShadeKernel
 {
     uint32_t is;
@@ -402,15 +266,22 @@
 template <uint32_t IS>
 constexpr TraceShadeKernel trace_shade_kernel()
 {
-    return {IS, k_trace_shade<(IS & TS_FIRST) != 0, (IS & TS_EXT) != 0, (IS & TS_FB) != 0, (IS & TS_LDS) != 0, (IS & TS_TAME) != 0, (IS & TS_CODE) != 0>};
-}
-constexpr TraceShadeKernel kTraceShadeKernels[13] = {
+    if constexpr ((IS & TS_TAB) != 0)
+    {
+        static_assert((IS & ~(TS_FIRST | TS_CODE)) == (TS_LDS | TS_TAME | TS_TAB), "TAB: the lean kernels");
+        return {IS, k_trace_shade_tab<(IS & TS_FIRST) != 0, (IS & TS_CODE) != 0>};
+    }
+    else
+        return {IS, k_trace_shade<(IS & TS_FIRST) != 0, (IS & TS_EXT) != 0, (IS & TS_FB) != 0, (IS & TS_LDS) != 0, (IS & TS_TAME) != 0, (IS & TS_CODE) != 0>};
+}
+constexpr TraceShadeKernel kTraceShadeKernels[16] = {
     trace_shade_kernel<TS_FIRST | TS_LDS | TS_TAME | TS_CODE>(),
     trace_shade_kernel<TS_FIRST | TS_EXT | TS_LDS>(), trace_shade_kernel<TS_FIRST | TS_EXT>(),
     trace_shade_kernel<TS_FIRST | TS_LDS | TS_TAME>(), trace_shade_kernel<TS_FIRST | TS_LDS>(), trace_shade_kernel<TS_FIRST>(),
     trace_shade_kernel<TS_EXT | TS_LDS>(), trace_shade_kernel<TS_EXT>(),
     trace_shade_kernel<TS_FB | TS_LDS>(), trace_shade_kernel<TS_FB>(),
     trace_shade_kernel<TS_LDS | TS_TAME>(), trace_shade_kernel<TS_LDS>(), trace_shade_kernel<0>(),
+    trace_shade_kernel<TS_FIRST | TS_LDS | TS_TAME | TS_CODE | TS_TAB>(), trace_shade_kernel<TS_FIRST | TS_LDS | TS_TAME | TS_TAB>(), trace_shade_kernel<TS_LDS | TS_TAME | TS_TAB>(),
 };
 
 static bool tame_kernels(const BvhDev& bvh, const SceneDev& scene)
@@ -422,6 +293,7 @@
 #endif
 }
 bool trace_shade_has_code_form(const BvhDev& bvh, const SceneDev& scene) { return tame_kernels(bvh, scene); }
+bool trace_shade_has_table_form(const BvhDev& bvh, const SceneDev& scene) { return kChunkLean && tame_kernels(bvh, scene); }
 
 uint32_t launch_trace_shade(const LaunchCfg& cfg, const BvhDev& bvh, const ShadeArgs& args, bool ext, bool feedback)
 {
@@ -431,10 +303,12 @@
     const bool tame  = !ext && !fb && tame_kernels(bvh, args.scene);
     const bool code  = first && args.code_in_color != 0u;
     assert(!code || tame);
-    const uint32_t is = (first ? TS_FIRST : 0u) | (ext ? TS_EXT : 0u) | (fb ? TS_FB : 0u) | (lds ? TS_LDS : 0u) | (tame ? TS_TAME : 0u) | (code ? TS_CODE : 0u);
+    const bool tab = args.sample_terms != nullptr;
+    assert(!tab || (tame && kChunkLean));
+    const uint32_t is = (first ? TS_FIRST : 0u) | (ext ? TS_EXT : 0u) | (fb ? TS_FB : 0u) | (lds ? TS_LDS : 0u) | (tame ? TS_TAME : 0u) | (code ? TS_CODE : 0u) | (tab ? TS_TAB : 0u);
     const uint32_t gx = queue_grid(cfg, first ? args.screen.pixels_padded * args.n_slots : args.max_count);
     const TraceShadeKernel* k = kTraceShadeKernels;
-    while (k->is != is && k + 1 < kTraceShadeKernels + 13) ++k;
+    while (k->is != is && k + 1 < kTraceShadeKernels + 16) ++k;
     assert(k->is == is);
     hipLaunchKernelGGL(k->kernel, dim3(gx), dim3(kBlock), 0, cfg.stream, bvh, args);
 #if defined(CAP_CLOSEST_V1)
diff --git a/capsaicin_amd/csrc/small_scene_body.h b/capsaicin_amd/csrc/small_scene_body.h
--- /dev/null
+++ b/capsaicin_amd/csrc/small_scene_body.h
@@ -0,0 +1,192 @@
+    const uint32_t Ppad     = a.screen.pixels_padded;
+    const uint32_t cps      = Ppad >> 6;
+    const uint32_t chunks   = FIRST ? cps * a.n_slots : (a.in.class_capacity >> 6) * kQueueClasses;
+    uint32_t       n_shaded = 0, n_probed = 0;
+    __shared__ FrameConst lds_frames[kMaxFrameSlots];
+    __shared__ float4     lds_shade[LDS ? kShadeRec * kExhaustiveMax : 1];
+    __shared__ float4     lds_rec[LDS ? 4 * kExhaustiveMax : 1];
+    __shared__ float4     lds_probe[C::PROBE ? 2 * kMaxFrameSlots : 1];
+    __shared__ float      lds_pscore[C::PROBE ? kExhaustiveMax / 2 : 1];
+    __shared__ SlotSample lds_first[(C::LEAN && FIRST && !TAB) ? kMaxFrameSlots : 1];
+    __shared__ uint32_t   lds_probe_k;
+    __shared__ float4     lds_ring[(C::PROBE && !FIRST) ? (kBlock / 64) * kWaveRing : 1];
+    __shared__ float4     lds_org[C::ORG ? kExhaustiveMax : 1];
+    __shared__ float4     lds_bounds[C::ORG ? kExhaustiveMax / 2 : 1];
+    __shared__ float      lds_mat[C::XT ? 12 * kExhaustiveMax : 1];
+    __shared__ float      lds_lcdf[C::XT ? kExtLightsMax : 1];
+    __shared__ float4     lds_lrec[C::XT ? 4 * kExtLightsMax : 1];
+    const bool            ext_tabs = C::XT && a.scene.material_count <= kExhaustiveMax && a.scene.light_count <= kExtLightsMax;
+    if (LDS)
+    {
+        stage_scene_records(bvh, a, lds_shade, lds_rec);
+        if (C::XT && ext_tabs) stage_ext_tables(a, lds_mat, lds_lcdf, lds_lrec);
+        if (C::ORG) stage_camera_pairs(bvh, a, lds_org, lds_bounds);
+    }
+    if (C::PROBE && a.inline_probe) stage_probe_rows(bvh, a, lds_pscore, lds_probe_k, lds_probe);
+    if constexpr (C::LEAN)
+        stage_frames_samples<FIRST, TAB>(a, lds_frames, lds_first);
+    else
+        stage_frames(a, lds_frames);
+    ProbeArgs probe;
+    if (C::PROBE && a.inline_probe) probe.rows = lds_probe, probe.pairs = bvh.fan_pairs, probe.k = lds_probe_k;
+    uint32_t ring_head = 0, ring_n = 0;
+    if (C::PROBE && !FIRST && a.inline_probe && a.wave_ring)
+    {
+        probe.ring_org = lds_ring + (threadIdx.x >> 6) * kWaveRing;
+        probe.ring_con = a.shadow.contrib_pid + (size_t)wave_global_id() * kWaveRing;
+    }
+    auto trace_ring = [&](uint32_t count) {
+        wave_handoff();
+        const uint32_t lane_ = threadIdx.x & 63u;
+        const bool     on    = lane_ < count;
+        const uint32_t pos   = (ring_head + lane_) & (kWaveRing - 1u);
+        float4         o     = make_float4(0.f, 0.f, 0.f, 0.f);
+        if (on) o = probe.ring_org[pos];
+        const uint32_t spid = f2u(o.w);
+        const bool     good = on && (spid >> kPidShift) < a.n_slots && (spid & kPidMask) < Ppad;
+        const FrameConst& fc = lds_frames[good ? (spid >> kPidShift) : 0u];
+        const Ray  sr = make_ray(mk3(o.x, o.y, o.z), mk3(fc.light_dir[0], fc.light_dir[1], fc.light_dir[2]), kRayEps, good ? kRayFar : kRayEps);
+        float4* const target = a.bounce == 0 ? a.planes.direct : a.planes.color;
+        const size_t  idx    = good ? (size_t)(spid >> kPidShift) * Ppad + (spid & kPidMask) : 0;
+        float4        c = make_float4(0.f, 0.f, 0.f, 0.f), cur = c;
+        if (good) c = probe.ring_con[pos], cur = target[idx];
+        const bool occluded = exhaustive_any<false>(bvh, sr);
+        if (good && !occluded) target[idx] = make_float4(cur.x + c.x, cur.y + c.y, cur.z + c.z, cur.w);
+        ring_head = (ring_head + count) & (kWaveRing - 1u);
+        ring_n -= count;
+    };
+    const float4* shade_tab = LDS ? lds_shade : a.scene.shade_tris;
+    const float4* rec_tab   = LDS ? lds_rec : bvh.tris_by_id;
+    ExtTables     xtabs;
+    if (C::XT && ext_tabs) xtabs.materials = reinterpret_cast<const MaterialDev*>(lds_mat), xtabs.light_cdf = lds_lcdf, xtabs.light_rec = lds_lrec;
+    Stamps st;
+    st.start();
+    const uint32_t my_class = wave_global_id() % kQueueClasses;
+    const uint32_t lane     = threadIdx.x & 63u;
+    uint32_t       n_class  = 0;
+    if (!FIRST)
+    {
+        n_class = a.in.count[my_class * kCounterStride];
+        n_class = n_class < a.in.class_capacity ? n_class : a.in.class_capacity;
+    }
+    uint32_t grab = grab_issue(a.work, my_class);
+    while (true)
+    {
+        const uint32_t j = grab_value(grab);
+        uint32_t       i, pid = 0, slot = 0;
+        const uint32_t klass = my_class;
+        bool           active;
+        v3             thr = mk3(1.0f, 1.0f, 1.0f);
+        Ray            r   = make_ray(mk3(0.f, 0.f, 0.f), mk3(0.f, 0.f, 1.f), 0.0f, 0.0f);
+        float          carried_r1 = 0.f, carried_r2 = 0.f;
+        if (FIRST)
+        {
+            const uint32_t chunk = class_chunk(j, my_class);
+            if (chunk >= chunks) break;
+            grab   = grab_issue(a.work, my_class);
+            slot   = chunk / cps;
+            i      = (chunk - slot * cps) * 64 + lane;
+            active = true;
+            pid    = (slot << kPidShift) | i;
+            uint32_t x, y;
+            if (local_pixel_to_xy(a.screen, i, x, y))
+                r = make_ray(mk3(a.cam.position[0], a.cam.position[1], a.cam.position[2]),
+                             primary_dir(a.cam, a.screen, lds_frames[slot], x, y), 0.0f, kPrimaryFar);
+        }
+        else
+        {
+            if (j * 64u >= n_class) break;
+            active = j * 64u + lane < n_class;
+            if constexpr (C::LEAN)
+            {
+                const uint32_t local = j * 64u + lane;
+                i                    = my_class * a.in.class_capacity + (local < n_class ? local : n_class - 1u);
+                const float4 o = a.in.org_tmin[i], d = a.in.dir_tmax[i], tp = a.in.thr_pid[i];
+                grab = grab_issue(a.work, my_class);
+                r    = make_ray(mk3(o.x, o.y, o.z), mk3(d.x, d.y, d.z), kRayEps, kRayFar);
+                thr  = mk3(tp.x, tp.y, tp.z), pid = f2u(tp.w);
+                if (!TAB) carried_r1 = o.w, carried_r2 = d.w;
+            }
+            else
+            {
+                i      = my_class * a.in.class_capacity + j * 64u + lane;
+                float4 o = make_float4(0.f, 0.f, 0.f, 0.f), d = make_float4(0.f, 0.f, 1.f, 0.f), tp = make_float4(1.f, 1.f, 1.f, 0.f);
+                if (active) o = a.in.org_tmin[i], d = a.in.dir_tmax[i], tp = a.in.thr_pid[i];
+                grab = grab_issue(a.work, my_class);
+                if (active)
+                {
+                    r   = make_ray(mk3(o.x, o.y, o.z), mk3(d.x, d.y, d.z), kRayEps, kRayFar);
+                    thr = mk3(tp.x, tp.y, tp.z), pid = f2u(tp.w);
+                    carried_r1 = o.w, carried_r2 = d.w;
+                }
+            }
+        }
+        float    t, u, v;
+        uint32_t gid;
+        STAMP(st, 0, true);
+        uint32_t pair_mask = ~0u;
+        if (C::ORG)
+        {
+            uint32_t tx = 0, ty = 0;
+            (void)local_pixel_to_xy(a.screen, i & ~63u, tx, ty);
+            const float4 b    = lds_bounds[lane < kExhaustiveMax / 2 ? lane : 0u];
+            const bool   over = lane < bvh.fan_pair_count && b.x < (float)(tx + 8u) && b.z >= (float)tx && b.y < (float)(ty + 8u) && b.w >= (float)ty;
+            pair_mask         = (uint32_t)__ballot(over);
+        }
+        __builtin_amdgcn_s_setprio(0);
+#if !defined(CAP_CLOSEST_V1)
+        if constexpr (LDS && !C::ORG)
+        {
+            if (bvh.tri_count > 32u)
+                exhaustive_closest_marked<true>(bvh, rec_tab, r, active, t, u, v, gid);
+            else
+                exhaustive_closest_marked<false>(bvh, rec_tab, r, active, t, u, v, gid);
+        }
+        else
+#endif
+            exhaustive_closest<C::ORG, !LDS>(bvh, rec_tab, r, t, u, v, gid, lds_org, pair_mask);
+        __builtin_amdgcn_s_setprio(3);
+        STAMP(st, 1, true);
+        const ShadePre pre = shade_prefetch<C>(a, lds_frames, active, pid, carried_r1, carried_r2, lds_first);
+        if (FIRST && slot == a.aov_slot)
+        {
+            float4 g = make_float4(0.f, 0.f, u2f(kInvalidId), u2f(kInvalidId));
+            if (gid != kInvalidId)
+            {
+                const uint4 id = a.scene.tri_ids[gid];
+                g              = make_float4(u, v, u2f(id.x), u2f(id.y));
+            }
+            a.planes.aov_geo[i] = g;
+        }
+        if constexpr (EXT)
+        {
+            if (a.inline_nee)
+            {
+                v3 acc = mk3(0.f, 0.f, 0.f);
+                if (!FIRST && active)
+                {
+                    const float4 q = a.in.acc[i];
+                    acc            = mk3(q.x, q.y, q.z);
+                }
+                shade_vertex_ext<FIRST, true>(a, shade_tab, pre, klass, pid, make_float4(u, v, u2f(gid), t), thr, r.d, n_shaded, &bvh, acc, xtabs);
+            }
+            else
+                shade_vertex_ext<FIRST>(a, shade_tab, pre, klass, pid, make_float4(u, v, u2f(gid), t), thr, r.d, n_shaded, nullptr, mk3(0.f, 0.f, 0.f), xtabs);
+        }
+        else
+        {
+            shade_vertex<C>(a, shade_tab, pre, klass, pid, make_float4(u, v, u2f(gid), t), thr, n_shaded, st, probe, &n_probed, ring_head, &ring_n);
+            if (C::PROBE && ring_n >= 64u) trace_ring(64u);
+        }
+        STAMP(st, 4, false);
+    }
+    if (!FIRST && !EXT && !FB) st.flush();
+#ifdef CAP_STAMPS
+    if (!FIRST && !EXT && !FB && (threadIdx.x & 63u) == 0 && wave_global_id() < 16384)
+    {
+        g_wave_times[2 * wave_global_id() + 0] = st.t_begin;
+        g_wave_times[2 * wave_global_id() + 1] = __builtin_amdgcn_s_memrealtime();
+    }
+#endif
+    if (C::PROBE && ring_n != 0u) trace_ring(ring_n);
+    flush_stats(a.out.count + (size_t)my_class * kCounterStride, n_shaded, n_probed);
diff --git a/include/capsaicin_hip.h b/include/capsaicin_hip.h
--- a/include/capsaicin_hip.h
+++ b/include/capsaicin_hip.h
@@ -180,6 +180,8 @@
     CAP_DEBUG_SHADE_TAME           = 13,
     CAP_DEBUG_CAMERA_CULL          = 14,
     CAP_DEBUG_MARK_FORM            = 15,
+    CAP_DEBUG_SAMPLE_TABLE          = 16,
+    CAP_DEBUG_SELFTEST_SAMPLE_TABLE = 17,
     CAP_DEBUG_SWITCH_BASE         = 64
 };
 int cap_debug_set(CapContext* ctx, uint32_t key, uint64_t value);
```

Result: faster. 58260 Mrays/s (median of 6 runs) (+3.4%).
